# OpenDrift/opendrift

Measured on AMD Instinct MI355X. Metric: particle-steps/sec (RK4, 3D interp), higher is better.
Workload: dtype f64; 1 GPU; C3: OceanDrift 3D, synthetic ROMS-shaped z-level grid 1024x1024x12 (u,v,w,K), RK4 + vertical_mixing(60 s) + vertical_advection; particles_per_gpu=10000000, particles_total=10000000, stage_math=fast, spin_up_steps=200, block_every=0, inputs=resident in HBM, parallelism=particle-sharded x1, field block broadcast once per time level

## Files before the change

include/odrift.h:

```cpp
#ifndef ODRIFT_H
#define ODRIFT_H
#include <stdint.h>

#ifdef __cplusplus
extern "C" {
#endif

typedef struct odr_ctx odr_ctx;
typedef struct odr_particles odr_particles;

typedef enum {
  ODR_OK = 0,
  ODR_ERR_INVALID = -1,
  ODR_ERR_HIP = -2,
  ODR_ERR_CAPACITY = -3,
  ODR_ERR_STATE = -4
} odr_status;

enum {
  ODR_VAR_X_SEA_WATER_VELOCITY = 0,
  ODR_VAR_Y_SEA_WATER_VELOCITY = 1,
  ODR_VAR_X_WIND = 2,
  ODR_VAR_Y_WIND = 3,
  ODR_VAR_UPWARD_SEA_WATER_VELOCITY = 4,
// ... 61 lines not shown
                                       double *z, int32_t *id, int32_t *status);
int odr_particles_upload(odr_ctx *ctx, odr_particles *p, const double *lon, const double *lat,
                         const double *z, const int32_t *moving, const float *wind_drift_factor,
                         const float *current_drift_factor, const float *terminal_velocity);
int odr_particles_download_f32(odr_ctx *ctx, odr_particles *p, const char *name, float *host);
int odr_particles_device_ptr(odr_ctx *ctx, odr_particles *p, const char *name, void **dptr);

int odr_source_constant(odr_ctx *ctx, int nvars, const int32_t *var_ids, const double *values,
                        int32_t *source_id);
int odr_source_analytic(odr_ctx *ctx, int kind, const double *params, int nparams,
                        int32_t *source_id);
int odr_source_landmask(odr_ctx *ctx, int32_t nx, int32_t ny, double lon0, double lat0, double dlon, double dlat,
                        const uint8_t *cells, int32_t *source_id);
int odr_source_grid(odr_ctx *ctx, const odr_proj_desc *proj, const double *domain6,
                    int lon_mode, int mod360_x, int nz, const double *z, int32_t *source_id);
int odr_source_grid_curvilinear(odr_ctx *ctx, const double *lon, const double *lat, int ny, int nx,
                                const double *domain6, int lon_mode, int nz, const double *z,
                                int32_t *source_id);
int odr_source_lonlat2xy(odr_ctx *ctx, int32_t source_id, int64_t n, const double *lon, const double *lat,
                         double *x, double *y);
int odr_block_upload(odr_ctx *ctx, int32_t source_id, int32_t slot, double t_epoch, int nvars,
                     const int32_t *var_ids, const float *const *data, const int32_t *var_nz,
                     int ny, int nx, const double *xy8);
int odr_block_upload_device(odr_ctx *ctx, int32_t source_id, int32_t slot, double t_epoch,
                            int nvars, const int32_t *var_ids, const void *const *dev_data,
                            const int32_t *var_nz, int ny, int nx, const double *xy8);
int odr_block_upload_async(odr_ctx *ctx, int32_t source_id, int32_t slot, double t_epoch, int nvars,
                           const int32_t *var_ids, const void *const *data, const int32_t *var_nz,
                           int ny, int nx, const double *xy8);
int odr_block_commit(odr_ctx *ctx, int32_t source_id, int32_t slot);
int odr_block_set_content_ids(odr_ctx *ctx, int32_t source_id, int32_t slot, int nvars, const int32_t *var_ids,
                              const uint64_t *ids);
int odr_host_register(odr_ctx *ctx, void *ptr, uint64_t bytes);
int odr_host_unregister(odr_ctx *ctx, void *ptr);
int odr_block_drop(odr_ctx *ctx, int32_t source_id, int32_t slot);
int odr_particles_truncate_z(odr_ctx *ctx, odr_particles *p, double truncate_depth);
int odr_particles_restore_z(odr_ctx *ctx, odr_particles *p);
int odr_source_release(odr_ctx *ctx, int32_t source_id);
int odr_source_time_coverage(odr_ctx *ctx, int32_t source_id, double t_start_epoch, double t_end_epoch,
                             int always_valid);
int odr_source_set_members(odr_ctx *ctx, int32_t source_id, int32_t var, int32_t members);
int odr_particles_set_rank_offset(odr_ctx *ctx, odr_particles *p, int64_t offset);
int odr_env_bind(odr_ctx *ctx, int32_t var_id, int nsources, const int32_t *source_ids,
                 float fallback);

int odr_env_sample(odr_ctx *ctx, odr_particles *p, int nvars, const int32_t *var_ids,
                   double t_epoch, float *const *out_host);
int odr_env_download(odr_ctx *ctx, odr_particles *p, int32_t var_id, float *out_host);
int odr_env_upload(odr_ctx *ctx, odr_particles *p, int32_t var_id, const float *host);
enum { ODR_NOISE_NORMAL = 0, ODR_NOISE_UNIFORM = 1 };
int odr_env_add_noise(odr_ctx *ctx, odr_particles *p, int32_t var_x, int32_t var_y, double std, int distribution,
                      int rng_mode, const double *host_nx, const double *host_ny, uint64_t step);
int odr_advect_set_noise(odr_ctx *ctx, odr_particles *p, double std_normal, double std_uniform, int rng_mode,
                         const double *host_main, const double *host_stage, int nstage, uint64_t step);
enum { ODR_STAGE_EXACT = 0, ODR_STAGE_FAST = 1 };
int odr_ctx_set_stage_math(odr_ctx *ctx, int mode);
int odr_advect(odr_ctx *ctx, odr_particles *p, int scheme, double t_epoch, double dt, double factor);
typedef struct {
  int32_t seafloor_action;
  int32_t retired_code;
  double age_dt;
  double max_age_seconds;
  int32_t missing_code;
  int32_t main_noise;
  int32_t vmix;
  int32_t vmix_at_surface;
  int32_t vmix_vadv;
  int32_t pad;
  double vmix_dt_mix;
  uint64_t vmix_step;
} odr_step_extras;
int odr_env_coast_advect(odr_ctx *ctx, odr_particles *p, int nvars, const int32_t *var_ids, double t_epoch,
                         int coastline_action, int stranded_code, int seeded_on_land_code,
                         int store_previous, int scheme, double dt, double factor,
                         const odr_step_extras *extras , int64_t *n_on_land);
int odr_update_positions(odr_ctx *ctx, odr_particles *p, const double *x_vel, const double *y_vel,
                         int velocities_are_float32, double dt);

enum { ODR_FACTOR_SCALAR = 0, ODR_FACTOR_ICE_CURRENT = 1, ODR_FACTOR_ICE_STOKES = 2, ODR_FACTOR_ICE_DRIFT = 3 };
int odr_set_element_factor(odr_ctx *ctx, odr_particles *p, int kind);
int odr_advect_sea_ice(odr_ctx *ctx, odr_particles *p, double dt, double factor);
int odr_advect_wind(odr_ctx *ctx, odr_particles *p, double dt, double wind_drift_depth,
                    int relative_wind, double factor);
int odr_stokes_drift(odr_ctx *ctx, odr_particles *p, double dt, int profile, int hs_mode,
                     int tp_mode, double factor);
int odr_particles_set_property(odr_ctx *ctx, odr_particles *p, int slot, int64_t offset, int64_t count,
                               const float *host);
int odr_particles_get_property(odr_ctx *ctx, odr_particles *p, int slot, float *host);
int odr_particles_snapshot_property(odr_ctx *ctx, odr_particles *p, int slot);
enum { ODR_SPLIT_LANE = 1 };
int odr_leeway_set_missing_code(odr_ctx *ctx, int32_t code);
int odr_env_coast_leeway(odr_ctx *ctx, odr_particles *p, int nvars, const int32_t *var_ids, double t_epoch, int coast_action,
                         int stranded_code, int seeded_on_land_code, int store_previous, double dt, double capsize_fraction,
                         double std_current, double std_wind, uint64_t step, int64_t *n_on_land);
int odr_leeway_capsize(odr_ctx *ctx, odr_particles *p, double dt, double wind_threshold, double wind_threshold_sigma,
                       int rng_mode, const double *host_uniforms, uint64_t step);
int odr_leeway(odr_ctx *ctx, odr_particles *p, double dt, double capsize_leeway_fraction, int rng_mode,
               const double *host_uniforms, uint64_t step);
int odr_hdiffusion(odr_ctx *ctx, odr_particles *p, double dt, int rng_mode,
                   const double *host_nx, const double *host_ny, uint64_t step);
int odr_movers(odr_ctx *ctx, odr_particles *p, double dt, int which, double wind_drift_depth, int relative_wind,
               double wind_factor, int stokes_profile, int hs_mode, int tp_mode, double stokes_factor, int rng_mode,
               const double *host_nx, const double *host_ny, uint64_t step);
int odr_vmix(odr_ctx *ctx, odr_particles *p, double t_epoch, double dt, double dt_mix,
             int mix_at_surface, int rng_mode, const double *host_uniforms, uint64_t step);
enum { ODR_DIFFUSIVITY_LARGE1994 = 1, ODR_DIFFUSIVITY_SUNDBY1983 = 2 };
int odr_vmix_set_profile_levels(odr_ctx *ctx, int32_t n);
int odr_vmix_wind_profile(odr_ctx *ctx, odr_particles *p, int model, double background_diffusivity, double dt,
                          double dt_mix, int mix_at_surface, int rng_mode, const double *host_uniforms,
                          uint64_t step);
enum { ODR_OIL_DIAMETER = 0, ODR_OIL_DENSITY = 1, ODR_OIL_VISCOSITY = 2, ODR_OIL_FILM_THICKNESS = 3,
       ODR_OIL_DIAMETER_IF_ENTRAINED = 4  };
enum { ODR_DROPLETS_JOHANSEN2015 = 1, ODR_DROPLETS_LI2017 = 2 };
int odr_oil_prepare_mixing(odr_ctx *ctx, odr_particles *p, double dt, double dt_mix, double interfacial_tension,
                           double sea_water_density, int droplet_distribution, int keep_droplet_diameter, int hs_mode,
                           int tp_mode, int temperature_to_kelvin, int rng_mode, const double *host_u_diameter,
                           const double *host_u_entrain, const double *host_u_intrusion, uint64_t step);
int odr_oil_mixing_stats(odr_ctx *ctx, double *mean_zb, double *dv50);
int odr_oil_local_sums(odr_ctx *ctx, odr_particles *p, double interfacial_tension, double sea_water_density,
                       int droplet_distribution, int hs_mode, double *sum_dv50, double *sum_zb);
int odr_oil_set_mixing_stats(odr_ctx *ctx, double mean_zb, double dv50);
int odr_vmix_fuse_vertical_advection(odr_ctx *ctx, int at_surface);
int odr_vertical_advection(odr_ctx *ctx, odr_particles *p, double dt, int at_surface);
int odr_vertical_buoyancy(odr_ctx *ctx, odr_particles *p, double dt);
int odr_store_previous(odr_ctx *ctx, odr_particles *p);
int odr_coastline(odr_ctx *ctx, odr_particles *p, int action, int stranded_code,
                  int seeded_on_land_code ,
                  int64_t *n_on_land);
int odr_coastline_crossing(odr_ctx *ctx, odr_particles *p, int action, int stranded_code, int seeded_on_land_code,
                           double precision_deg, int32_t landmask_source, int64_t *n_on_land);
int odr_deactivate_missing(odr_ctx *ctx, odr_particles *p, int nvars, const int32_t *var_ids,
                           int32_t status_code, int64_t *n_missing);
int odr_increase_age(odr_ctx *ctx, odr_particles *p, double dt, double max_age_seconds, int retired_code);
int odr_seafloor(odr_ctx *ctx, odr_particles *p, int64_t *n_below);
enum { ODR_SEAFLOOR_LIFT = 1, ODR_SEAFLOOR_DEACTIVATE = 2, ODR_SEAFLOOR_PREVIOUS = 3 };
int odr_seafloor_action(odr_ctx *ctx, odr_particles *p, int action, int32_t status_code, int64_t *n_below);
int odr_set_seafloor_action(odr_ctx *ctx, int action, int32_t status_code);
int odr_particles_count_status(odr_ctx *ctx, odr_particles *p, int32_t status_code, int64_t *n);
int odr_particles_remap_status(odr_ctx *ctx, odr_particles *p, int32_t from_code, int32_t to_code);
int odr_deactivate(odr_ctx *ctx, odr_particles *p, const uint8_t *mask_host, int32_t status_code);
int odr_deactivate_outside(odr_ctx *ctx, odr_particles *p, double west, double east, double south, double north,
                           int32_t status_code);
int odr_compact(odr_ctx *ctx, odr_particles *p, int64_t *n_active);
int odr_scan_status(odr_ctx *ctx, odr_particles *p, int64_t *n_kept, uint64_t *status_flags);
int odr_scan_status_begin(odr_ctx *ctx, odr_particles *p);
int odr_scan_status_end(odr_ctx *ctx, odr_particles *p, int64_t *n_kept, uint64_t *status_flags);
int odr_ctx_guard_next_vmix(odr_ctx *ctx, int on);
int odr_compact_apply(odr_ctx *ctx, odr_particles *p, int64_t *n_active);
int odr_sort_particles(odr_ctx *ctx, odr_particles *p, int32_t source_id);
int odr_sort_particles_ex(odr_ctx *ctx, odr_particles *p, int32_t source_id, int keep_environment);
int odr_particles_tile_stats(odr_ctx *ctx, odr_particles *p, uint64_t *out4);
int odr_particles_step_layout_stats(odr_ctx *ctx, odr_particles *p, uint64_t *out2);
int odr_particles_step_onlevel_stats(odr_ctx *ctx, odr_particles *p, uint64_t *out1);
int odr_particles_vmix_layout_stats(odr_ctx *ctx, odr_particles *p, uint64_t *out3);
int odr_reduce_scalars(odr_ctx *ctx, odr_particles *p, double wind_drift_depth, double *out16);
int odr_ctx_set_step_reduce(odr_ctx *ctx, int on, double wind_drift_depth, int relative_wind);
int odr_reduce_local(odr_ctx *ctx, odr_particles *p, double wind_drift_depth, int relative_wind, double *out16);
int odr_reduce_install(odr_ctx *ctx, odr_particles *p, const double *in16);
int odr_reduce_unpin(odr_ctx *ctx);

int odr_ctx_set_position_class(odr_ctx *ctx, int f32);
int odr_source_set_coordinate_dtype(odr_ctx *ctx, int32_t source_id, int x_is_float32, int y_is_float32);

#define ODR_COMM_ID_BYTES 256
int odr_device_count(int32_t *n);
int odr_comm_unique_id(uint8_t *id );
int odr_comm_init(odr_ctx *ctx, const uint8_t *id, int32_t rank, int32_t nranks);
int odr_comm_info(int32_t *rank, int32_t *nranks, uint64_t *id_hash, int32_t *rccl_version, uint64_t *collectives);
int odr_comm_destroy(void);
int odr_allreduce_scalars(odr_ctx *ctx, double *values, int32_t n, int32_t op);
int odr_comm_allgather_begin(odr_ctx *ctx, const double *row, int32_t n, int32_t from_scan);
int odr_comm_allgather_end(odr_ctx *ctx, double *rows );
int odr_comm_broadcast_bytes(odr_ctx *ctx, void *buf, int64_t nbytes, int32_t root);
int odr_comm_barrier(odr_ctx *ctx);
int odr_block_broadcast(odr_ctx *ctx, int32_t source_id, int32_t slot, double t_epoch, int nvars, const int32_t *var_ids,
                        const void *const *data, const int32_t *var_nz, int ny, int nx, const double *xy8, int32_t root);

int odr_timer_begin(odr_ctx *ctx);
int odr_timer_end(odr_ctx *ctx, float *ms);

enum {
  ODR_HIST_LON = 1000, ODR_HIST_LAT, ODR_HIST_Z, ODR_HIST_STATUS, ODR_HIST_MOVING, ODR_HIST_AGE_SECONDS,
  ODR_HIST_WIND_DRIFT_FACTOR, ODR_HIST_CURRENT_DRIFT_FACTOR, ODR_HIST_TERMINAL_VELOCITY,
  ODR_HIST_PROPERTY0 = 2000
};
typedef struct odr_history odr_history;
int odr_history_create(odr_ctx *ctx, int64_t n_trajectories, int32_t n_times, int32_t nvars,
                       const int32_t *var_codes, odr_history **out);
int odr_history_set_id_base(odr_ctx *ctx, odr_history *h, int64_t id_base);
int odr_history_destroy(odr_ctx *ctx, odr_history *h);
enum { ODR_HIST_PROPERTIES_FROM_SNAPSHOT = 2 };
int odr_history_record(odr_ctx *ctx, odr_particles *p, odr_history *h, int32_t time_index, int only_deactivated,
                       int position_from_previous);
int odr_history_flush(odr_ctx *ctx, odr_history *h, int32_t t0, int32_t nt);
int odr_history_wait(odr_ctx *ctx, odr_history *h);
int odr_history_host_ptr(odr_ctx *ctx, odr_history *h, int32_t var_index, float **ptr, int32_t *nt);
int odr_history_reset(odr_ctx *ctx, odr_history *h);
int odr_history_minmax(odr_ctx *ctx, odr_history *h, int32_t var_index, double *minval, double *maxval);

typedef struct odr_sgrid odr_sgrid;
int odr_sgrid_create(odr_ctx *ctx, int32_t ny, int32_t nx, int32_t N, const double *H, const double *zeta_or_null,
                     double Hc, const double *Cs_r, const double *S_or_null, int32_t Vtransform, odr_sgrid **out);
int odr_sgrid_destroy(odr_ctx *ctx, odr_sgrid *g);
int odr_sgrid_download_zrho(odr_ctx *ctx, odr_sgrid *g, double *out );
int odr_sgrid_zslice(odr_ctx *ctx, odr_sgrid *g, const void *field, int is_f64, int on_device, int32_t kmax,
                     const double *Z, int32_t out_slot, void **out_dev32, double *out_host64);

#ifdef __cplusplus
}
#endif
#endif
```

opendrift_amd/_abi.py:

```python
import ctypes as C
import os

HERE = os.path.dirname(os.path.abspath(__file__))
LIB_PATH = os.environ.get('ODR_LIB') or os.path.join(HERE, 'libodrift_hip.so')

NVAR = 26
VARIABLES = {
    'x_sea_water_velocity': 0, 'y_sea_water_velocity': 1, 'x_wind': 2, 'y_wind': 3,
    'upward_sea_water_velocity': 4, 'ocean_vertical_diffusivity': 5,
    'sea_surface_wave_stokes_drift_x_velocity': 6, 'sea_surface_wave_stokes_drift_y_velocity': 7,
    'land_binary_mask': 8, 'sea_floor_depth_below_sea_level': 9, 'sea_surface_height': 10,
    'horizontal_diffusivity': 11, 'sea_surface_wave_significant_height': 12,
    'sea_surface_wave_period_at_variance_spectral_density_maximum': 13,
    'ocean_mixed_layer_thickness': 14,
    'sea_water_temperature': 15, 'sea_water_salinity': 16,
    'sea_ice_area_fraction': 17, 'sea_ice_x_velocity': 18, 'sea_ice_y_velocity': 19,
    'sea_surface_swell_wave_to_direction': 20,
    'sea_surface_swell_wave_peak_period_from_variance_spectral_density': 21,
    'sea_surface_swell_wave_significant_height': 22, 'sea_surface_wind_wave_to_direction': 23,
    'sea_surface_wind_wave_mean_period': 24, 'sea_surface_wind_wave_significant_height': 25,
}
VARIABLE_NAMES = {v: k for k, v in VARIABLES.items()}
PROJ_LATLONG, PROJ_STERE_EQUIT_SPHERE, PROJ_STERE_POLAR = 0, 1, 2
PROJ_MERC, PROJ_LCC = 4, 5
PROJ_TMERC, PROJ_LAEA, PROJ_STERE_OBLIQUE, PROJ_OB_TRAN = 6, 7, 8, 9
SCHEME = {'euler': 0, 'runge-kutta': 1, 'runge-kutta4': 2}
RNG_DEVICE, RNG_HOST = 0, 1
STAGE_MATH = {'exact': 0, 'fast': 1}
COAST = {'none': 0, 'stranding': 1, 'previous': 2}
HIST = {'lon': 1000, 'lat': 1001, 'z': 1002, 'status': 1003, 'moving': 1004, 'age_seconds': 1005,
        'wind_drift_factor': 1006, 'current_drift_factor': 1007, 'terminal_velocity': 1008}
HIST_PROPERTY0 = 2000
COMM_ID_BYTES = 256


class StepExtras(C.Structure):
    _fields_ = [('seafloor_action', C.c_int32), ('retired_code', C.c_int32), ('age_dt', C.c_double),
                ('max_age_seconds', C.c_double), ('missing_code', C.c_int32), ('main_noise', C.c_int32),
                ('vmix', C.c_int32), ('vmix_at_surface', C.c_int32), ('vmix_vadv', C.c_int32), ('pad', C.c_int32),
                ('vmix_dt_mix', C.c_double), ('vmix_step', C.c_uint64)]
ANALYTIC_DOUBLE_GYRE, ANALYTIC_OSCILLATING = 1, 2


class ProjDesc(C.Structure):
    _fields_ = [('kind', C.c_int32), ('a', C.c_double), ('es', C.c_double), ('lat0_deg', C.c_double),
                ('lon0_deg', C.c_double), ('lat_ts_deg', C.c_double), ('k0', C.c_double),
                ('x0', C.c_double), ('y0', C.c_double), ('lat1_deg', C.c_double), ('lat2_deg', C.c_double)]


class OdrError(RuntimeError):
    code = 0


_P = C.POINTER
_dp, _fp, _ip, _i64p = _P(C.c_double), _P(C.c_float), _P(C.c_int32), _P(C.c_int64)
_vp = C.c_void_p

_SIGNATURES = {
    'odr_ctx_create': [C.c_int, C.c_uint64, _P(_vp)],
    'odr_ctx_destroy': [_vp],
    'odr_sync': [_vp],
    'odr_set_stream': [_vp, _vp],
    'odr_particles_create': [_vp, C.c_int64, _P(_vp)],
    'odr_particles_destroy': [_vp, _vp],
    'odr_particles_append': [_vp, _vp, C.c_int64, _dp, _dp, _dp, _ip, _ip, _fp, _fp, _fp],
    'odr_particles_count': [_vp, _vp, _i64p, _i64p],
    'odr_particles_download': [_vp, _vp, _dp, _dp, _dp, _ip, _ip, _ip],
    'odr_particles_download_deactivated': [_vp, _vp, _dp, _dp, _dp, _ip, _ip],
    'odr_particles_upload': [_vp, _vp, _dp, _dp, _dp, _ip, _fp, _fp, _fp],
    'odr_particles_device_ptr': [_vp, _vp, C.c_char_p, _P(_vp)],
    'odr_particles_download_f32': [_vp, _vp, C.c_char_p, _fp],
    'odr_source_constant': [_vp, C.c_int, _ip, _dp, _ip],
    'odr_source_analytic': [_vp, C.c_int, _dp, C.c_int, _ip],
    'odr_source_grid': [_vp, _P(ProjDesc), _dp, C.c_int, C.c_int, C.c_int, _dp, _ip],
    'odr_source_grid_curvilinear': [_vp, _dp, _dp, C.c_int, C.c_int, _dp, C.c_int, C.c_int, _dp, _ip],
    'odr_source_landmask': [_vp, C.c_int32, C.c_int32, C.c_double, C.c_double, C.c_double, C.c_double, _P(C.c_uint8), _ip],
    'odr_source_lonlat2xy': [_vp, C.c_int32, C.c_int64, _dp, _dp, _dp, _dp],
    'odr_block_upload': [_vp, C.c_int32, C.c_int32, C.c_double, C.c_int, _ip, _P(_fp), _ip, C.c_int,
                         C.c_int, _dp],
    'odr_block_upload_device': [_vp, C.c_int32, C.c_int32, C.c_double, C.c_int, _ip, _P(_vp), _ip,
                                C.c_int, C.c_int, _dp],
    'odr_block_upload_async': [_vp, C.c_int32, C.c_int32, C.c_double, C.c_int, _ip, _P(_vp), _ip, C.c_int, C.c_int, _dp],
    'odr_block_commit': [_vp, C.c_int32, C.c_int32],
    'odr_host_register': [_vp, _vp, C.c_uint64],
    'odr_host_unregister': [_vp, _vp],
    'odr_block_drop': [_vp, C.c_int32, C.c_int32],
    'odr_env_bind': [_vp, C.c_int32, C.c_int, _ip, C.c_float],
    'odr_env_sample': [_vp, _vp, C.c_int, _ip, C.c_double, _P(_fp)],
    'odr_env_download': [_vp, _vp, C.c_int32, _fp],
    'odr_env_upload': [_vp, _vp, C.c_int32, _fp],
    'odr_env_add_noise': [_vp, _vp, C.c_int32, C.c_int32, C.c_double, C.c_int, C.c_int, _dp, _dp, C.c_uint64],
    'odr_advect_set_noise': [_vp, _vp, C.c_double, C.c_double, C.c_int, _dp, _dp, C.c_int, C.c_uint64],
    'odr_ctx_set_stage_math': [_vp, C.c_int],
    'odr_advect': [_vp, _vp, C.c_int, C.c_double, C.c_double, C.c_double],
    'odr_env_coast_advect': [_vp, _vp, C.c_int, _ip, C.c_double, C.c_int, C.c_int, C.c_int, C.c_int, C.c_int,
                             C.c_double, C.c_double, _vp, _P(C.c_int64)],
    'odr_update_positions': [_vp, _vp, _dp, _dp, C.c_int, C.c_double],
    'odr_source_set_members': [_vp, C.c_int32, C.c_int32, C.c_int32],
    'odr_particles_set_rank_offset': [_vp, _vp, C.c_int64],
    'odr_block_set_content_ids': [_vp, C.c_int32, C.c_int32, C.c_int, _P(C.c_int32), _P(C.c_uint64)],
    'odr_set_element_factor': [_vp, _vp, C.c_int],
    'odr_advect_sea_ice': [_vp, _vp, C.c_double, C.c_double],
    'odr_advect_wind': [_vp, _vp, C.c_double, C.c_double, C.c_int, C.c_double],
    'odr_stokes_drift': [_vp, _vp, C.c_double, C.c_int, C.c_int, C.c_int, C.c_double],
    'odr_particles_set_property': [_vp, _vp, C.c_int, C.c_int64, C.c_int64, _fp],
    'odr_particles_get_property': [_vp, _vp, C.c_int, _fp],
    'odr_particles_snapshot_property': [_vp, _vp, C.c_int],
    'odr_env_coast_leeway': [_vp, _vp, C.c_int, _ip, C.c_double, C.c_int, C.c_int, C.c_int, C.c_int, C.c_double, C.c_double,
                             C.c_double, C.c_double, C.c_uint64, _i64p],
    'odr_leeway_set_missing_code': [_vp, C.c_int32],
    'odr_leeway_capsize': [_vp, _vp, C.c_double, C.c_double, C.c_double, C.c_int, _dp, C.c_uint64],
    'odr_leeway': [_vp, _vp, C.c_double, C.c_double, C.c_int, _dp, C.c_uint64],
    'odr_hdiffusion': [_vp, _vp, C.c_double, C.c_int, _dp, _dp, C.c_uint64],
    'odr_movers': [_vp, _vp, C.c_double, C.c_int, C.c_double, C.c_int, C.c_double, C.c_int, C.c_int, C.c_int, C.c_double, C.c_int, _dp, _dp,
                   C.c_uint64],
    'odr_vmix': [_vp, _vp, C.c_double, C.c_double, C.c_double, C.c_int, C.c_int, _dp, C.c_uint64],
    'odr_vmix_wind_profile': [_vp, _vp, C.c_int, C.c_double, C.c_double, C.c_double, C.c_int, C.c_int, _dp, C.c_uint64],
    'odr_vmix_fuse_vertical_advection': [_vp, C.c_int],
    'odr_oil_prepare_mixing': [_vp, _vp, C.c_double, C.c_double, C.c_double, C.c_double, C.c_int, C.c_int, C.c_int, C.c_int,
                               C.c_int, C.c_int, _dp, _dp, _dp, C.c_uint64],
    'odr_oil_mixing_stats': [_vp, _dp, _dp],
    'odr_oil_local_sums': [_vp, _vp, C.c_double, C.c_double, C.c_int, C.c_int, _dp, _dp],
    'odr_oil_set_mixing_stats': [_vp, C.c_double, C.c_double],
    'odr_vertical_advection': [_vp, _vp, C.c_double, C.c_int],
    'odr_vertical_buoyancy': [_vp, _vp, C.c_double],
    'odr_store_previous': [_vp, _vp],
    'odr_coastline': [_vp, _vp, C.c_int, C.c_int, C.c_int, _i64p],
    'odr_coastline_crossing': [_vp, _vp, C.c_int, C.c_int, C.c_int, C.c_double, C.c_int32, _i64p],
    'odr_increase_age': [_vp, _vp, C.c_double, C.c_double, C.c_int],
    'odr_source_time_coverage': [_vp, C.c_int32, C.c_double, C.c_double, C.c_int],
    'odr_source_release': [_vp, C.c_int32],
    'odr_particles_truncate_z': [_vp, _vp, C.c_double],
    'odr_particles_restore_z': [_vp, _vp],
    'odr_seafloor': [_vp, _vp, _i64p],
    'odr_seafloor_action': [_vp, _vp, C.c_int, C.c_int32, _i64p],
    'odr_set_seafloor_action': [_vp, C.c_int, C.c_int32],
    'odr_deactivate_missing': [_vp, _vp, C.c_int, _ip, C.c_int32, _i64p],
    'odr_particles_count_status': [_vp, _vp, C.c_int32, _i64p],
    'odr_particles_remap_status': [_vp, _vp, C.c_int32, C.c_int32],
    'odr_deactivate': [_vp, _vp, _P(C.c_uint8), C.c_int32],
    'odr_deactivate_outside': [_vp, _vp, C.c_double, C.c_double, C.c_double, C.c_double, C.c_int32],
    'odr_compact': [_vp, _vp, _i64p],
    'odr_vmix_set_profile_levels': [_vp, C.c_int32],
    'odr_ctx_set_position_class': [_vp, C.c_int],
    'odr_source_set_coordinate_dtype': [_vp, C.c_int32, C.c_int, C.c_int],
    'odr_device_count': [_P(C.c_int32)],
    'odr_comm_unique_id': [_P(C.c_uint8)],
    'odr_comm_init': [_vp, _P(C.c_uint8), C.c_int32, C.c_int32],
    'odr_comm_info': [_P(C.c_int32), _P(C.c_int32), _P(C.c_uint64), _P(C.c_int32), _P(C.c_uint64)],
    'odr_comm_destroy': [],
    'odr_allreduce_scalars': [_vp, _dp, C.c_int32, C.c_int32],
    'odr_comm_allgather_begin': [_vp, _dp, C.c_int32, C.c_int32],
    'odr_comm_allgather_end': [_vp, _dp],
    'odr_comm_broadcast_bytes': [_vp, _vp, C.c_int64, C.c_int32],
    'odr_comm_barrier': [_vp],
    'odr_block_broadcast': [_vp, C.c_int32, C.c_int32, C.c_double, C.c_int, _ip, _P(_vp), _ip, C.c_int, C.c_int, _dp, C.c_int32],
    'odr_scan_status': [_vp, _vp, _i64p, _P(C.c_uint64)],
    'odr_scan_status_begin': [_vp, _vp],
    'odr_scan_status_end': [_vp, _vp, _i64p, _P(C.c_uint64)],
    'odr_ctx_guard_next_vmix': [_vp, C.c_int],
    'odr_compact_apply': [_vp, _vp, _i64p],
    'odr_sort_particles': [_vp, _vp, C.c_int32],
    'odr_sort_particles_ex': [_vp, _vp, C.c_int32, C.c_int],
    'odr_particles_tile_stats': [_vp, _vp, _P(C.c_uint64)],
    'odr_particles_step_layout_stats': [_vp, _vp, _P(C.c_uint64)],
    'odr_particles_step_onlevel_stats': [_vp, _vp, _P(C.c_uint64)],
    'odr_particles_vmix_layout_stats': [_vp, _vp, _P(C.c_uint64)],
    'odr_reduce_scalars': [_vp, _vp, C.c_double, _dp],
    'odr_ctx_set_step_reduce': [_vp, C.c_int, C.c_double, C.c_int],
    'odr_reduce_local': [_vp, _vp, C.c_double, C.c_int, _dp],
    'odr_reduce_install': [_vp, _vp, _dp],
    'odr_reduce_unpin': [_vp],
    'odr_timer_begin': [_vp],
    'odr_timer_end': [_vp, _fp],
    'odr_sgrid_create': [_vp, C.c_int32, C.c_int32, C.c_int32, _dp, _dp, C.c_double, _dp, _dp, C.c_int32, _P(_vp)],
    'odr_sgrid_destroy': [_vp, _vp],
    'odr_sgrid_download_zrho': [_vp, _vp, _dp],
    'odr_sgrid_zslice': [_vp, _vp, _vp, C.c_int, C.c_int, C.c_int32, _dp, C.c_int32, _P(_vp), _dp],
    'odr_history_create': [_vp, C.c_int64, C.c_int32, C.c_int32, _ip, _P(_vp)],
    'odr_history_destroy': [_vp, _vp],
    'odr_history_set_id_base': [_vp, _vp, C.c_int64],
    'odr_history_record': [_vp, _vp, _vp, C.c_int32, C.c_int, C.c_int],
    'odr_history_flush': [_vp, _vp, C.c_int32, C.c_int32],
    'odr_history_wait': [_vp, _vp],
    'odr_history_host_ptr': [_vp, _vp, C.c_int32, _P(_fp), _P(C.c_int32)],
    'odr_history_reset': [_vp, _vp],
    'odr_history_minmax': [_vp, _vp, C.c_int32, _dp, _dp],
}
EXPORTS = sorted(list(_SIGNATURES) + ['odr_last_error', 'odr_version'])

_lib = None


def load():
    global _lib
    if _lib is not None:
        return _lib
    if not os.path.exists(LIB_PATH):
        raise OdrError('libodrift_hip.so is missing: run `python -c "import __graft_entry__ as g; '
                       'g.build()"` (hipcc --offload-arch=gfx950).  There is no CPU fallback.')
    lib = C.CDLL(LIB_PATH)
    for name, args in _SIGNATURES.items():
        fn = getattr(lib, name)
        fn.argtypes = args
        fn.restype = C.c_int
    lib.odr_last_error.restype = C.c_char_p
    lib.odr_last_error.argtypes = []
    lib.odr_version.restype = C.c_char_p
    lib.odr_version.argtypes = []
    _lib = lib
    return lib


NOISE_NORMAL, NOISE_UNIFORM = 0, 1
DIFFUSIVITY = {'windspeed_Large1994': 1, 'windspeed_Sundby1983': 2}
DROPLETS = {'Johansen et al. (2015)': 1, 'Li et al. (2017)': 2}
OIL_PROPERTIES = ['diameter', 'density', 'viscosity', 'oil_film_thickness', 'diameter_if_entrained']


def check(rc):
    if rc != 0:
        msg = load().odr_last_error().decode()
        if rc == -1:
            raise ValueError(msg)
        e = OdrError('odrift error %d: %s' % (rc, msg))
        e.code = rc
        raise e
```

opendrift_amd/csrc/odr_host.h:

```cpp
#pragma once
#include <hip/hip_runtime.h>

#include <algorithm>
#include <cmath>
#include <cstdarg>
#include <cstdio>
#include <cstdlib>
#include <cstring>
#include <string>
#include <vector>

#include "../../include/odrift.h"
#include "odr_kernels.hip.h"

using namespace odr;

#include <chrono>
struct SlowSpan {
  const char *what;
  std::chrono::steady_clock::time_point t0;
  static double limit() { static const double v = getenv("ODR_SLOW_CALLS") ? atof(getenv("ODR_SLOW_CALLS")) : 0.0; return v; }
  explicit SlowSpan(const char *w) : what(w) { if (limit() > 0) t0 = std::chrono::steady_clock::now(); }
  ~SlowSpan() {
    if (limit() > 0) {
      const double ms = std::chrono::duration<double, std::milli>(std::chrono::steady_clock::now() - t0).count();
      if (ms > limit()) fprintf(stderr, "[odr slow] %s: %.3f ms\n", what, ms);
    }
  }
};

int odr_i_fail(int code, const char *fmt, ...);
#define fail odr_i_fail
#define HIPCHK(x)                                                                          \
  do {                                                                                     \
    hipError_t e_ = (x);                                                                   \
    if (e_ != hipSuccess) return fail(ODR_ERR_HIP, "%s: %s", #x, hipGetErrorString(e_));   \
  } while (0)
#define REQUIRE(c, ...) do { if (!(c)) return fail(ODR_ERR_INVALID, __VA_ARGS__); } while (0)

struct Staged { DevBlock blk; float *base; size_t bytes; unsigned long long cid[NVAR]; };
struct Retired { void *ptr; size_t bytes; hipEvent_t ev; };

struct odr_ctx {
  int device;
  unsigned long long seed;
  hipStream_t stream, own_stream;
  DevWorld hw;
  DevWorld *dw;
  unsigned src_gen[MAXSRC] = {0};
  hipEvent_t scan_ev = nullptr;
  bool scan_open = false;
  int guard_next_vmix = 0;
  const odr_particles *guarded_vmix = nullptr;
  int guarded_vadv = -1;
  int vmix_levels = 0;
  unsigned long long *scan_host = nullptr;
  DevWorld *hw_pin[3] = {nullptr, nullptr, nullptr};
  hipEvent_t hw_ev[3] = {nullptr, nullptr, nullptr};
  int hw_turn = 0;
  bool dirty;
  std::vector<void *> block_bufs[MAXSRC][MAXLEVELS];
  size_t block_bytes[MAXSRC][MAXLEVELS];
  unsigned long long block_cid[MAXSRC][MAXLEVELS][NVAR];
  hipStream_t up_stream;
  hipEvent_t up_done, up_dep;
  float *prep[2];
  size_t prep_floats;
  int *dilate_flags;
  int *tile_flags = nullptr;
  size_t tile_flags_n = 0;
  void *bounce[2];
  Staged staged[MAXSRC][MAXLEVELS];
  std::vector<Retired> graveyard;
  std::vector<void *> source_bufs;
  std::vector<void *> registered;
  double *red;
  const odr_particles *noise_owner;
  StageNoise noise;
  double *noise_buf;
  size_t noise_buf_n;
  const odr_particles *oil_owner;
  OilArgs oil;
  double *oil_stat, *oil_cdf, *oil_chunk, *oil_part, *oil_u;
  int *oil_guide;
  int oil_override;
  double oil_stat_host[2];
  size_t oil_part_n, oil_u_n;
  unsigned long long *counter;
  hipEvent_t ev0, ev1;
  int nsrc;
  bool src_free[MAXSRC];
  int stage_math;
  int fuse_vadv;
  int leeway_missing_code;
  int seafloor;
  const odr_particles *red_owner;
  unsigned long long red_epoch;
  double red_wdd;
  int red_rel;
  bool red_extents = true;
  int red_pinned;
  double *red_rec = nullptr; long long red_rec_cap = 0;
  bool red_partial = false;
  int step_reduce_on = 0, step_reduce_rel = 0;
  double step_reduce_wdd = 0.1;
};

struct odr_particles {
  long long cap, n, ndead, dead_cap;
  int ice_kind;
  int *rank;
  unsigned *rank_words, *rank_before, *rank_bsum;
  long long rank_words_n, id_max;
  int rank_on;
  int rank_sharded = 0;
  long long rank_offset = 0;
  double *d64[7];
  double *alt64[7];
  int *i32[3];
  int *alti32[3];
  float *f32[4];
  float *altf32[4];
  float *env[NVAR];
  float *altenv[NVAR];
  float *aux[9];
  float *altaux[9];
  bool profiles_f32 = false;
  unsigned aux_user = 0;
  bool kmember_on = false;
  float *aux_snap[9];
  long long aux_snap_cap[9];
  double *dead64[3];
  int *deadi32[2];
  unsigned *bcount;
  unsigned *wcount;
  unsigned long long wcount_epoch;
  long long wcount_n;
  void *scratch;
  size_t scratch_bytes;
  unsigned long long epoch;
  unsigned long long status_epoch, scan_epoch;
  long long scan_kept;
  float env_cval[NVAR];
  long long env_cn[NVAR];
  bool env_cok[NVAR];
  bool external;
  unsigned *wg_tab, *wg_list;
  unsigned long long *wg_total, *wg_stats;
  long long wg_cap, wg_grid, wg_n, wg_list_cap;
  unsigned long long wg_launches;
  unsigned long long step_launches[3];
  unsigned long long vmix_launches[3];
  double *z_keep;
  long long z_keep_n;
  bool z_truncated;
  int wg_sid;
  bool wg_valid;
  unsigned wg_src_gen;
};

static inline unsigned nblk(long long n) { return (unsigned)((n + BLOCK - 1) / BLOCK); }

static inline PView view(const odr_particles *p) {
  PView v;
  v.n = p->n;
  v.lon = p->d64[0]; v.lat = p->d64[1]; v.z = p->d64[2]; v.plon = p->d64[3]; v.plat = p->d64[4];
  v.slon = p->d64[5]; v.slat = p->d64[6];
  v.id = p->i32[0]; v.status = p->i32[1]; v.moving = p->i32[2];
  v.wdf = p->f32[0]; v.cdf = p->f32[1]; v.tv = p->f32[2]; v.age = p->f32[3];
  for (int k = 0; k < NVAR; ++k) v.env[k] = p->env[k];
  for (int k = 0; k < 9; ++k) v.aux[k] = p->aux[k];
  v.ice = p->ice_kind; v.pad = 0;
  v.rank = p->rank_on && p->rank ? p->rank : nullptr;
  return v;
}

static inline EnvGroupDesc env_bind_out(const EnvGroupDesc &G0, const PView &v) {
  EnvGroupDesc G = G0;
  for (int k = 0; k < MAXG; ++k) G.out_ptr[k] = k < G.nv ? v.env[G.var[k]] : nullptr;
  return G;
}

int flush_world(odr_ctx *c);
int flush_world_init(odr_ctx *c);

static inline bool env_is_const(const odr_particles *p, int v, float val) {
  return p->env[v] && p->env_cok[v] && p->env_cn[v] >= p->n && p->env_cval[v] == val;
}
static inline int ensure_env(odr_ctx *c, odr_particles *p, int var) {
  if (!p->env[var]) {
    HIPCHK(hipMalloc((void **)&p->env[var], sizeof(float) * (size_t)p->cap));
    HIPCHK(hipMemsetAsync(p->env[var], 0, sizeof(float) * (size_t)p->cap, c->stream));
  }
  return 0;
}

static inline int scratch(odr_ctx *c, odr_particles *p, size_t bytes, void **out) {
  if (p->scratch_bytes < bytes) {
    SlowSpan sp("scratch: synchronize + hipFree + hipMalloc");
    HIPCHK(hipStreamSynchronize(c->stream));
    if (p->scratch) HIPCHK(hipFree(p->scratch));
    HIPCHK(hipMalloc(&p->scratch, bytes));
    p->scratch_bytes = bytes;
  }
  *out = p->scratch;
  return 0;
}

static inline void host_bracket(const DevSource &s, double t, int &ib, int &ia) {
  int b = 0;
  for (int k = 0; k < s.nlevels; ++k) if (s.slot[s.level_slot[k]].t <= t) b = k;
  ib = s.level_slot[b];
  ia = (b + 1 < s.nlevels && s.slot[ib].t != t) ? s.level_slot[b + 1] : -1;
}

static inline UVTime uv_time(const DevSource &s, double t) {
  int ib, ia;
  host_bracket(s, t, ib, ia);
  UVTime tm;
  tm.b = s.slot[ib].data[VAR_U];
  tm.a = (ia >= 0 && !s.always_valid) ? s.slot[ia].data[VAR_U] : nullptr;
  tm.w = ia >= 0 ? (t - s.slot[ib].t) / (s.slot[ia].t - s.slot[ib].t) : 0.0;
  return tm;
}


static inline bool build_vmix_desc(const odr_ctx *c, double t, VMixDesc &D) {
  memset(&D, 0, sizeof D);
  int ksid = -1, nzp = 1;
  for (int k = 0; k < c->hw.nlist[VAR_KZ]; ++k)
    if (c->hw.src[c->hw.list[VAR_KZ][k]].kind == SRC_GRID) { ksid = c->hw.list[VAR_KZ][k]; break; }
  if (ksid < 0) return false;
  const DevSource &s = c->hw.src[ksid];
  nzp = s.nz > 1 ? s.nz : 1;
  if (nzp <= 1 || s.nlevels < 1) return false;
  const DevBlock &g0 = s.slot[s.level_slot[0]];
  for (int k = 0; k < s.nlevels; ++k) {
    const DevBlock &bk = s.slot[s.level_slot[k]];
    if (s.members[VAR_KZ] > 1 || !bk.small || !bk.data[VAR_KZ] || bk.es[VAR_KZ] != 1 || bk.var_nz[VAR_KZ] != nzp || bk.rec != g0.rec || bk.ny != g0.ny || bk.nx != g0.nx ||
        bk.x0 != g0.x0 || bk.xspan != g0.xspan || bk.y0 != g0.y0 || bk.yspan != g0.yspan)
      return false;
  }
  int ib, ia;
  host_bracket(s, t, ib, ia);
  D.sid = ksid; D.nzp = nzp; D.geo_slot = ib;
  D.kb = s.slot[ib].data[VAR_KZ];
  D.ka = ia >= 0 ? s.slot[ia].data[VAR_KZ] : nullptr;
  D.wgt = ia >= 0 ? (t - s.slot[ib].t) / (s.slot[ia].t - s.slot[ib].t) : 0.0;
  D.Kfb = c->hw.fallback[VAR_KZ];
  return true;
}

constexpr size_t ODR_BOUNCE_BYTES = 8u << 20;
static inline int odr_i_bounce(odr_ctx *c, int which, void **buf) {
  if (!c->bounce[which]) HIPCHK(hipHostMalloc(&c->bounce[which], ODR_BOUNCE_BYTES, hipHostMallocDefault));
  *buf = c->bounce[which];
  return 0;
}
static inline int odr_i_h2d(odr_ctx *c, void *dst, const void *src, size_t bytes, hipStream_t st, int which = 0) {
  void *b;
  int rc = odr_i_bounce(c, which, &b);
  if (rc) return rc;
  for (size_t o = 0; o < bytes; o += ODR_BOUNCE_BYTES) {
    const size_t m = std::min(ODR_BOUNCE_BYTES, bytes - o);
    memcpy(b, (const char *)src + o, m);
    HIPCHK(hipMemcpyAsync((char *)dst + o, b, m, hipMemcpyHostToDevice, st));
    HIPCHK(hipStreamSynchronize(st));
  }
  return 0;
}
static inline int odr_i_d2h(odr_ctx *c, void *dst, const void *src, size_t bytes, hipStream_t st, int which = 0) {
  void *b;
  int rc = odr_i_bounce(c, which, &b);
  if (rc) return rc;
  for (size_t o = 0; o < bytes; o += ODR_BOUNCE_BYTES) {
    const size_t m = std::min(ODR_BOUNCE_BYTES, bytes - o);
    HIPCHK(hipMemcpyAsync(b, (const char *)src + o, m, hipMemcpyDeviceToHost, st));
    HIPCHK(hipStreamSynchronize(st));
    memcpy((char *)dst + o, b, m);
  }
  return 0;
}
#define H2D(dst, src, bytes) do { int rc_ = odr_i_h2d(c, (dst), (src), (bytes), c->stream); if (rc_) return rc_; } while (0)
#define D2H(dst, src, bytes) do { int rc_ = odr_i_d2h(c, (dst), (src), (bytes), c->stream); if (rc_) return rc_; } while (0)

static inline bool source_has_members(const DevSource &s) {
  for (int v = 0; v < NVAR; ++v) if (s.members[v] > 1) return true;
  return false;
}
static inline bool any_members(const odr_ctx *c) {
  for (int k = 0; k < c->nsrc; ++k) if (c->hw.src[k].kind == SRC_GRID && source_has_members(c->hw.src[k])) return true;
  return false;
}
static inline int odr_proj_template(const odr::DevProj &p) {
  if (p.kind == odr::PROJ_STERE_POLAR) return p.es != 0 ? odr::PROJ_STERE_POLAR : odr::PROJ_STERE_EQUIT_SPHERE;
  if (p.kind >= odr::PROJ_TMERC) return odr::PROJ_EXT;
  return p.kind;
}
int odr_i_ensure_ranks(odr_ctx *c, odr_particles *p);

bool odr_i_build_env_group(const odr_ctx *c, const int *grp, int ng, double t, EnvGroupDesc &G);
bool odr_i_comm_on();
int odr_i_comm_rank();
int odr_i_comm_bcast_floats(float *dev, size_t count, int root, hipStream_t st);
void odr_i_phase_dump();
bool odr_i_uv_fast_source(const odr_ctx *c, int &sid, double t_lo, double t_hi);

bool odr_i_gyre_source(const odr_ctx *c, int var, int &sid);
int odr_i_env_sample(odr_ctx *c, odr_particles *p, int nvars, const int32_t *var_ids, double t, float *const *out_host,
                     bool record_positions);
int odr_i_red_finish(odr_ctx *c, odr_particles *p);
int odr_i_red_records(odr_ctx *c, odr_particles *p, double **rec);
int odr_i_reduce(odr_ctx *c, odr_particles *p, double wdd, int relwind, bool wind_args_matter = true, bool extents = true, bool partial_ok = false);
int odr_i_read_counter(odr_ctx *c, int64_t *out);
int odr_i_env_noise(odr_ctx *c, odr_particles *p, int vx, int vy, double std, int distribution, int rng_mode,
                    const double *dev_nx, const double *dev_ny, unsigned long long step);
#define build_env_group odr_i_build_env_group
#define uv_fast_source odr_i_uv_fast_source
#define gyre_source odr_i_gyre_source
#define env_sample_impl odr_i_env_sample
#define reduce odr_i_reduce
#define read_counter odr_i_read_counter
```

opendrift_amd/csrc/odr_kernels.hip.h:

```cpp
#pragma once
#include <hip/hip_runtime.h>
#include <rocrand/rocrand_kernel.h>
#include "odr_field.hip.h"

namespace odr {

#ifndef ODR_BLOCK
#define ODR_BLOCK 256
#endif
constexpr int BLOCK = ODR_BLOCK;
#ifndef ODR_POLAR_WAVES
#define ODR_POLAR_WAVES 3
#endif
#ifndef ODR_POLAR_STEP_WAVES
#define ODR_POLAR_STEP_WAVES 2
#endif
#define ODR_STEP_WAVES(PROJ) ((PROJ) == PROJ_LATLONG ? ODR_LATLONG_WAVES : ((PROJ) == PROJ_EXT ? 1 : ODR_POLAR_STEP_WAVES))
#ifndef ODR_LATLONG_WAVES
#define ODR_LATLONG_WAVES 1
#endif
#define ODR_WAVES(PROJ) ((PROJ) == PROJ_LATLONG ? ODR_LATLONG_WAVES : ((PROJ) == PROJ_EXT ? 1 : ODR_POLAR_WAVES))

__device__ __forceinline__ long long pid() {
  const unsigned nb = gridDim.x, b = blockIdx.x, per = nb >> 3, rem = nb & 7u, x = b & 7u, j = b >> 3;
// ... 397 lines not shown
    if (TL) {
      a00 = ld_off<F4>(ka, o00 + 16u * q); a01 = ld_off<F4>(ka, o01 + 16u * q);
      a10 = ld_off<F4>(ka, o10 + 16u * q); a11 = ld_off<F4>(ka, o11 + 16u * q);
    }
    if (VM::STATIC && q > 0) __builtin_amdgcn_sched_barrier(0);
    if (q == 0) hook();
    double v[4];
    v[0] = (double)bilw(b00.x, b01.x, b10.x, b11.x, w00, w01, w10, w11);
    v[1] = (double)bilw(b00.y, b01.y, b10.y, b11.y, w00, w01, w10, w11);
    v[2] = (double)bilw(b00.z, b01.z, b10.z, b11.z, w00, w01, w10, w11);
    v[3] = (double)bilw(b00.w, b01.w, b10.w, b11.w, w00, w01, w10, w11);
    if (TL) {
      double w[4];
      w[0] = (double)bilw(a00.x, a01.x, a10.x, a11.x, w00, w01, w10, w11);
      w[1] = (double)bilw(a00.y, a01.y, a10.y, a11.y, w00, w01, w10, w11);
      w[2] = (double)bilw(a00.z, a01.z, a10.z, a11.z, w00, w01, w10, w11);
      w[3] = (double)bilw(a00.w, a01.w, a10.w, a11.w, w00, w01, w10, w11);
#pragma unroll
      for (int j = 0; j < 4; ++j) v[j] = __dadd_rn(__dmul_rn(v[j], 1 - wgt), __dmul_rn(w[j], wgt));
    }
#pragma unroll
    for (int j = 0; j < 4; ++j) Kp[(4 * q + j) * BLOCK + tid] = (cov && isfinite(v[j])) ? v[j] : Kfb;
  }
}

struct VMixArgs {
  double dt, dt_mix_cfg;
  int mix_at_surface, rng_mode, sfl, pad;
  const double *huni;
  unsigned long long seed, step;
};
struct MixRng { MixKey key; uint4 q; bool primed; };
template <class VM = VMixRT>
__device__ __forceinline__ MixRng mix_rng_begin(const VMixArgs &A, int id) {
  MixRng R;
  R.key = mix_key(A.seed, A.step, id);
  R.q = make_uint4(0u, 0u, 0u, 0u);
  R.primed = false;
  if (VM::rng_mode(A.rng_mode) == 0) {
    R.q = mix_block(R.key, 0u);
    R.primed = true;
  }
  return R;
}
template <int NQ, class VM = VMixRT>
__device__ __forceinline__ double vmix_col_walk(const DevSource &s, int nzp, const double *Kp, const double *gsh, int tid,
                                                const VMixArgs &A, long long i, long long n, int id, double z, int &moving,
                                                float Zmin, float tv, int &sf_flags, const MixRng *pre) {
  constexpr int NL = 4 * NQ;
  static_assert(!VM::STATIC || NL >= 3, "a static configuration has the three-level window inside the profile");
  const double dt = A.dt;
  const int mix_at_surface = VM::mix_at_surface(A.mix_at_surface), rng_mode = VM::rng_mode(A.rng_mode), sfl = A.sfl;
  double zm[NL - 1];
#pragma unroll
  for (int k = 0; k < NL - 1; ++k) zm[k] = k < nzp - 1 ? s.zmid[k] : __builtin_inf();
  const bool uniform_z = VM::uniform_z(s.vg_uniform != 0);
  const double gd0 = s.vg_d[0], gi0 = s.vg_id[0], gd1 = s.vg_d[1], gi1 = s.vg_id[1], gd2 = s.vg_d[2], gi2 = s.vg_id[2];
  const double sgn = dt > 0 ? 1.0 : (dt < 0 ? -1.0 : 0.0);
  const double dt_mix = A.dt_mix_cfg * sgn;
  const int ntimes = VM::ntimes(abs((int)(dt / dt_mix)));
  const double r = 1.0 / 3, ir = 1.0 / r;
  double wstep = __dmul_rn(__dmul_rn((double)tv, dt_mix), (double)moving);
  const MixKey st = mix_key(A.seed, A.step, id);
  uint4 u4 = make_uint4(0u, 0u, 0u, 0u);
  bool primed = false;
  if (pre) { u4 = pre->q; primed = pre->primed; }
  auto level_terms = [&](auto edges, int zl, double &dk_dt, double &sg) {
    constexpr int E = decltype(edges)::value;
    const double Kz = Kp[zl * BLOCK + tid];
    double gK;
    if ((E & 1) && zl == 0) gK = div_cr(Kp[BLOCK + tid] - Kz, gd0, gi0);
    else if ((E & 2) && zl == nzp - 1) gK = div_cr(Kz - Kp[(nzp - 2) * BLOCK + tid], gd1, gi1);
    else if (uniform_z) gK = div_cr(Kp[(zl + 1) * BLOCK + tid] - Kp[(zl - 1) * BLOCK + tid], gd2, gi2);
    else
      gK = __dadd_rn(__dadd_rn(__dmul_rn(gsh[zl], Kp[(zl - 1) * BLOCK + tid]), __dmul_rn(gsh[NL + zl], Kz)),
                     __dmul_rn(gsh[2 * NL + zl], Kp[(zl + 1) * BLOCK + tid]));
    double dK = -gK;
    if (fabs(dK) < 1e-10) dK = 0;
    dk_dt = __dmul_rn(dK, dt_mix);
    sg = sqrt(div_cr(__dmul_rn(__dmul_rn(Kz, fabs(dt_mix)), 2.0), r, ir));
  };
  using AnyLevel = std::integral_constant<int, 3>;
  int lv0;
  {
    const double d0 = -z;
    int zs = 0;
#pragma unroll
    for (int k = 0; k < NL - 1; ++k) zs += ((k & 1) ? d0 >= zm[k] : d0 > zm[k]) ? 1 : 0;
    lv0 = zs < 1 ? 1 : (zs > nzp - 2 ? nzp - 2 : zs);
    if (nzp < 3) lv0 = 1;
  }
  double c_dk[3], c_sg[3];
#pragma unroll
  for (int q = 0; q < 3; ++q) {
    const int zl = lv0 - 1 + q;
    c_dk[q] = 0; c_sg[q] = 0;
    if constexpr (VM::STATIC) {
      if (q == 0) level_terms(std::integral_constant<int, 1>(), zl, c_dk[q], c_sg[q]);
      else if (q == 1) level_terms(std::integral_constant<int, 0>(), zl, c_dk[q], c_sg[q]);
      else level_terms(std::integral_constant<int, 2>(), zl, c_dk[q], c_sg[q]);
    } else if (zl >= 0 && zl < nzp) level_terms(AnyLevel(), zl, c_dk[q], c_sg[q]);
  }
  double wb[4];
#pragma unroll
  for (int j = 0; j < 4; ++j) {
    const int k = lv0 - 2 + j;
    double b = k < 0 ? -1.0 : __builtin_inf();
    if (k >= 0 && k < nzp - 1) {
      b = gsh[3 * NL + k];
      if ((k & 1) && b > 0) b = __longlong_as_double(__double_as_longlong(b) - 1);
    }
    wb[j] = b;
  }
  for (int it0 = 0; it0 < ntimes; it0 += 5) {
  if (rng_mode == 0 && !(primed && it0 == 0)) u4 = mix_block(st, (unsigned)it0 / 5u);
#pragma unroll
  for (int k5 = 0; k5 < 5; ++k5) {
    const int it = it0 + k5;
    if (it >= ntimes) break;
    const bool surface = z == 0;
    const double d = -z;
    int q = (d > wb[1] ? 1 : 0) + (d > wb[2] ? 1 : 0);
    int zi = lv0 - 1 + q;
    if (!(d > wb[0]) || d > wb[3]) {
      zi = 0;
#pragma unroll
      for (int k = 0; k < NL - 1; ++k) zi += ((k & 1) ? d >= zm[k] : d > zm[k]) ? 1 : 0;
      q = zi - lv0 + 1;
    }
    double dKdt = q == 0 ? c_dk[0] : (q == 1 ? c_dk[1] : c_dk[2]);
    double sig = q == 0 ? c_sg[0] : (q == 1 ? c_sg[1] : c_sg[2]);
    if (q < 0 || q > 2) level_terms(AnyLevel(), zi, dKdt, sig);
    double R;
    if (rng_mode == 1) R = __dsub_rn(__dmul_rn(2.0, A.huni[(size_t)it * n + i]), 1.0);
    else R = mix_R_of(mix_word(u4, (unsigned)k5));
    z = __dsub_rn(z, __dmul_rn((double)moving, __dsub_rn(dKdt, __dmul_rn(R, sig))));
    if (z >= 0) z = -z;
    if (z < (double)Zmin && moving == 1) z = __dsub_rn((double)__fmul_rn(2.f, Zmin), z);
    z = __dadd_rn(z, wstep);
    if (!mix_at_surface && surface) z = 0.0;
    if (z > 0) z = 0.0;
    if (z < (double)Zmin) {
      const int act = VM::sf_action(sfl & 255);
      if (act == 3) sf_flags |= 2;
      else if (act) {
        z = (double)Zmin;
        if (act == 2) { sf_flags |= 1; moving = 0; wstep = 0.0; }
      }
    }
  }
  }
  return z;
}

__device__ __forceinline__ float pick_slot(const float (&a)[MAXG], int j) {
  float r = a[0];
#pragma unroll
  for (int k = 1; k < MAXG; ++k) {
    float v = a[k];
    asm volatile("" : "+v"(v));
    r = j == k ? v : r;
  }
  return r;
}

#ifdef ODR_TU_MISC
template <int NV>
struct GroupVars { int v[NV]; };

template <int NV>
__global__ __launch_bounds__(BLOCK) void k_env_group(const DevWorld *__restrict__ W, PView p,
                                                     GroupVars<NV> gv, double t, int record_prev) {
  long long i = (long long)blockIdx.x * BLOCK + threadIdx.x;
  if (i >= p.n) return;
  int vars[NV];
#pragma unroll
  for (int k = 0; k < NV; ++k) vars[k] = gv.v[k];
  double lon = p.lon[i], lat = p.lat[i], z = p.z[i];
  float out[NV];
  env_group<NV>(*W, vars, lon, lat, z, t, out, p.rank ? p.rank[i] : 0, W->f32pos & 1);
#pragma unroll
  for (int k = 0; k < NV; ++k) p.env[vars[k]][i] = out[k];
  if (record_prev) { p.slon[i] = lon; p.slat[i] = lat; }
}

template <int PROJ>
__global__ __launch_bounds__(BLOCK, ODR_WAVES(PROJ)) void k_env_grid(const DevWorld *__restrict__ W, PView p, EnvGroupDesc G,
                                                    int record_prev) {
  long long i = pid();
  if (i >= p.n) return;
  double lon = p.lon[i], lat = p.lat[i], z = p.z[i];
  int f32idx = 0;
  if (W->f32pos & 1) {
    lon = lon_f32class(W->src[G.sid].lon_mode, lon);
    if (PROJ == PROJ_LATLONG) f32idx = W->src[G.sid].xy_f32;
  }
  float out[MAXG];
  env_group_fast<PROJ>(*W, G, lon, lat, z, out, f32idx);
#pragma unroll
  for (int k = 0; k < MAXG; ++k)
    if (k < G.nv) G.out_ptr[k][i] = out[k];
  if (record_prev) { p.slon[i] = lon; p.slat[i] = lat; }
}

__global__ __launch_bounds__(BLOCK) void k_fill_f32(float *a, long long n, float v) {
  long long i = (long long)blockIdx.x * BLOCK + threadIdx.x;
  if (i < n) a[i] = v;
}

__global__ __launch_bounds__(BLOCK) void k_record_prev(PView p, int which) {
  long long i = (long long)blockIdx.x * BLOCK + threadIdx.x;
  if (i >= p.n) return;
  if (which == 0) { p.slon[i] = p.lon[i]; p.slat[i] = p.lat[i]; }
  else { p.plon[i] = p.lon[i]; p.plat[i] = p.lat[i]; }
}

#endif
#ifdef ODR_TU_STEP
__device__ __forceinline__ float rk4_mix(float k1, float k2, float k3, float k4) {
  float s = __fadd_rn(k1, __fmul_rn(2.0f, k2));
  s = __fadd_rn(s, __fmul_rn(2.0f, k3));
  s = __fadd_rn(s, k4);
  return div_cr_f32(s, 6.0f, 1.0f / 6.0f);
}

template <int SCHEME, bool NOISE>
__global__ __launch_bounds__(BLOCK) void k_advect(const DevWorld *__restrict__ W, PView p, double t,
                                                  double dt, float factor, StageNoise N) {
  long long i = (long long)blockIdx.x * BLOCK + threadIdx.x;
  if (i >= p.n) return;
  const int uv[2] = {VAR_U, VAR_V};
  double lon = p.lon[i], lat = p.lat[i], z = p.z[i];
  float u1 = p.env[VAR_U][i], v1 = p.env[VAR_V][i];
  float f = __fmul_rn(current_factor(p, i, factor), p.cdf[i]);
  int moving = p.moving[i];
  const int rk = p.rank ? p.rank[i] : 0;
  float fu, fv;
  GeodStart o = geod_start(lat, lon);
  if (SCHEME == 0) {
    fu = __fmul_rn(f, u1);
    fv = __fmul_rn(f, v1);
  } else {
    float dtf = (float)dt;
    double lon2, lat2;
    float k2[2];
    stage_pos_rt(N.sm, o, u1, v1, dtf, lon2, lat2);
    env_group<2>(*W, uv, lon2, lat2, z, t + dt / 2, k2, rk);
    const int id = NOISE ? p.id[i] : 0;
    if (NOISE) add_current_noise(N, 1, i, p.n, id, k2[0], k2[1]);
    if (SCHEME == 1) {
      fu = __fmul_rn(f, k2[0]);
      fv = __fmul_rn(f, k2[1]);
    } else {
      float k3[2], k4[2];
      stage_pos_rt(N.sm, o, k2[0], k2[1], dtf, lon2, lat2);
      env_group<2>(*W, uv, lon2, lat2, z, t + dt / 2, k3, rk);
      if (NOISE) add_current_noise(N, 2, i, p.n, id, k3[0], k3[1]);
      stage_pos_rt(N.sm, o, k3[0], k3[1], dtf, lon2, lat2);
      env_group<2>(*W, uv, lon2, lat2, z, t + dt, k4, rk);
      if (NOISE) add_current_noise(N, 3, i, p.n, id, k4[0], k4[1]);
      fu = __fmul_rn(rk4_mix(u1, k2[0], k3[0], k4[0]), f);
      fv = __fmul_rn(rk4_mix(v1, k2[1], k3[1], k4[1]), f);
    }
  }
  move_f32_from(o, lon, lat, fu, fv, moving, dt);
  p.lon[i] = lon;
  p.lat[i] = lat;
}

template <int PROJ, bool IS3D, int SM, class LD>
__device__ __forceinline__ void uv_stage_or_global(const DevSource &s, const DevBlock &geo, const UVTime &tm, const LD &ld, double lon,
                                                   double lat, double z, const ZBracket &zb, float fbu, float fbv, float &uo,
                                                   float &vo, const ProjStart &ps, UVKeep<IS3D> &K, bool keep) {
  if (!uv_stage<PROJ, IS3D, SM>(s, geo, tm, ld, lon, lat, z, zb, fbu, fbv, uo, vo, ps, K, keep)) {
    if constexpr (sizeof(LD) != sizeof(LdGlobal)) uv_stage<PROJ, IS3D, SM>(s, geo, tm, uv_global(tm), lon, lat, z, zb, fbu, fbv, uo, vo, ps, K, keep);
  }
}
template <int SCHEME, int PROJ, bool IS3D, bool NOISE, int SM = 0, bool PARK = false, class LD = LdGlobal>
__device__ __forceinline__ void advect_grid_body(const DevSource &s, const DevBlock &geo, double &lon, double &lat,
                                                 double z, float u1, float v1, float f, int moving, double dt,
                                                 const UVTime &th, const UVTime &tf, const LD &lh, const LD &lf, float fbu, float fbv,
                                                 const StageNoise &N, long long i, long long n, int id, UVKeep<IS3D> &K,
                                                 ZBracket zb_pre = ZBracket(), bool have_pre = false,
                                                 double *park = nullptr ODR_PT_PARAM, const ProjStart ps_pre = ProjStart()) {
  float fu, fv;
  const bool keep_f = tf.b == th.b && tf.a == th.a;
  GeodStart o0 = geod_start(lat, lon);
  lds_f64 *slot = (lds_f64 *)park;
  if constexpr (PARK) { geod_park(o0, slot); if (SM == 1 && SCHEME == 2) slot[14 * BLOCK] = (double)f; }
  auto O = [&]() { if constexpr (PARK) return geod_unpark(slot[12 * BLOCK], slot[13 * BLOCK], slot); else return o0; };
#define ODR_O O()
#define ODR_STAGE_POS(U_, V_) do { if constexpr (PARK && SM == 1) stage_pos_parked(slot, U_, V_, dtf, lon2, lat2); \
                                   else stage_pos<SM>(ODR_O, U_, V_, dtf, lon2, lat2); } while (0)
  if (SCHEME == 0) {
    fu = __fmul_rn(f, u1);
    fv = __fmul_rn(f, v1);
  } else {
    ZBracket zb;
    zb.iz0 = 0; zb.same = 0; zb.wa = 1;
    if (IS3D) { if (have_pre) zb = zb_pre; else zb = zbracket(s, z); }
    float dtf = (float)dt;
    double lon2, lat2;
    float u2, v2;
    ProjStart ps;
    if (PROJ == PROJ_STERE_POLAR || (ODR_PROJ_ROTATES(PROJ) && s.proj.kind == PROJ_STERE_POLAR && s.proj.es != 0)) {
      if (ps_pre.ok) ps = ps_pre;
      else {
        double lw = lon;
        if (s.lon_mode == 1) lw = np_mod(lw + 180.0, 360.0) - 180.0;
        else if (s.lon_mode == 2) lw = np_mod(lw, 360.0);
        ps = proj_start(s.proj, lw, lat);
      }
    }
    ODR_STAGE_POS(u1, v1);
    ODR_PT_USE(lon2); ODR_PT_USE(lat2); ODR_PT(4);
    uv_stage_or_global<PROJ, IS3D, SM>(s, geo, th, lh, lon2, lat2, z, zb, fbu, fbv, u2, v2, ps, K, true);
    if (NOISE) add_current_noise(N, 1, i, n, id, u2, v2);
    ODR_PT_USE(u2); ODR_PT_USE(v2); ODR_PT(5);
    if (SCHEME == 1) {
      fu = __fmul_rn(f, u2);
      fv = __fmul_rn(f, v2);
    } else {
      float u3, v3, u4, v4;
      ODR_STAGE_POS(u2, v2);
      uv_stage_or_global<PROJ, IS3D, SM>(s, geo, th, lh, lon2, lat2, z, zb, fbu, fbv, u3, v3, ps, K, true);
      if (NOISE) add_current_noise(N, 2, i, n, id, u3, v3);
      ODR_PT_USE(u3); ODR_PT_USE(v3); ODR_PT(6);
      ODR_STAGE_POS(u3, v3);
      uv_stage_or_global<PROJ, IS3D, SM>(s, geo, tf, lf, lon2, lat2, z, zb, fbu, fbv, u4, v4, ps, K, keep_f);
      if (NOISE) add_current_noise(N, 3, i, n, id, u4, v4);
      ODR_PT_USE(u4); ODR_PT_USE(v4); ODR_PT(7);
      float fl = f;
      if constexpr (PARK && SM == 1) fl = (float)slot[14 * BLOCK];
      fu = __fmul_rn(rk4_mix(u1, u2, u3, u4), fl);
      fv = __fmul_rn(rk4_mix(v1, v2, v3, v4), fl);
    }
  }
  move_f32_from(ODR_O, lon, lat, fu, fv, moving, dt);
#undef ODR_O
#undef ODR_STAGE_POS
}

template <int SCHEME, int PROJ, bool IS3D, bool NOISE, int SM = 0>
__global__ __launch_bounds__(BLOCK, ODR_STEP_WAVES(PROJ)) void k_advect_grid(const DevWorld *__restrict__ W, int sid, int geo_slot,
                                                       PView p, double dt, float factor, UVTime th,
                                                       UVTime tf, StageNoise N) {
  long long i = pid();
  if (i >= p.n) return;
  const DevSource &s = W->src[sid];
  const DevBlock &geo = s.slot[geo_slot];
  double lon = p.lon[i], lat = p.lat[i];
  UVKeep<IS3D> K;
  K.valid = false; K.n00 = K.n11 = K.kb = 0;
  advect_grid_body<SCHEME, PROJ, IS3D, NOISE, SM>(s, geo, lon, lat, p.z[i], p.env[VAR_U][i], p.env[VAR_V][i],
                                              __fmul_rn(current_factor(p, i, factor), p.cdf[i]), p.moving[i], dt, th, tf, uv_global(th), uv_global(tf),
                                              W->fallback[VAR_U], W->fallback[VAR_V], N, i, p.n, NOISE ? p.id[i] : 0, K);
  p.lon[i] = lon;
  p.lat[i] = lat;
}

#endif
enum { R_NACT = 0, R_LONMIN, R_LONMAX, R_LATMIN, R_LATMAX, R_ZMIN, R_ZMAX, R_DMAX, R_STOKESMAX,
       R_WSPEEDMAX, R_WDFMAX, R_NSURF, R_HSMAX, R_TPMAX, R_RELWSPEEDMAX, R_MLDMAX, R_N };

__device__ __forceinline__ void atomic_max_d(double *addr, double v) {
  unsigned long long *a = (unsigned long long *)addr, old = *a, assumed;
  do {
    assumed = old;
    if (__longlong_as_double((long long)assumed) >= v) break;
    old = atomicCAS(a, assumed, (unsigned long long)__double_as_longlong(v));
  } while (assumed != old);
}

__device__ __forceinline__ double wave_max(double v) {
#pragma unroll
  for (int o = 32; o > 0; o >>= 1) v = fmax(v, __shfl_xor(v, o, 64));
  return v;
}
__device__ __forceinline__ double wave_sum(double v) {
#pragma unroll
  for (int o = 32; o > 0; o >>= 1) v += __shfl_xor(v, o, 64);
  return v;
}
#ifdef ODR_TU_STEP
struct StepDesc {
  int coast_action, stranded_code, seeded_code, land_slot;
  int store_previous, geo_slot_uv;
  int seafloor, depth_slot;
  float age_dt, max_age;
  int retired_code, missing_code;
  int nmiss_grp, nmiss_rest;
  int miss_grp[4], miss_rest[4];
  int main_noise;
  int ssh_slot;
  int red_on, red_rel;
  int red_hd, red_sx, red_xw, red_pad;
  double red_wdd, red_iwdd;
  double *red;
  unsigned *wcount;
  unsigned long long *sflags;
};

#ifndef ODR_PARK_WAVES
#define ODR_PARK_WAVES 4
#endif
#ifndef ODR_PARK_WAVES_FAST3D
#define ODR_PARK_WAVES_FAST3D 5
#endif
#define ODR_PARK_WAVES_OF(PROJ, IS3D, SM) (((PROJ) == PROJ_LATLONG && (IS3D) && (SM) == 1) ? ODR_PARK_WAVES_FAST3D : ODR_PARK_WAVES)
#define ODR_STEP_PARKS(SCHEME, PROJ) ((SCHEME) > 0 && ((PROJ) == PROJ_LATLONG || (PROJ) == PROJ_CURVILINEAR))
template <int SCHEME, int PROJ, bool IS3D, bool NOISE, int SM = 0, class LY = LayoutRT>
__global__ __launch_bounds__(BLOCK, ODR_STEP_PARKS(SCHEME, PROJ) ? ODR_PARK_WAVES_OF(PROJ, IS3D, SM) : ODR_STEP_WAVES(PROJ)) void k_step_grid(const DevWorld *__restrict__ W, PView p, EnvGroupDesc G,
                                                     StepDesc S, double dt, float factor, UVTime th, UVTime tf,
                                                     unsigned long long *n_hit, StageNoise N) {
  long long i = pid();
  bool hit = false;
  ODR_PT_DECL;
  ODR_PT(0);
  constexpr bool PARK = ODR_STEP_PARKS(SCHEME, PROJ);
  __shared__ double s_park[PARK ? GEOD_PARK * BLOCK : 1];
  __shared__ double s_zt[IS3D ? 3 * ZT_STRIDE : 1];
  const double *zt = nullptr;
  double lon_e = 0, lat_e = 0, z_e = 0;
  if (i < p.n) { lon_e = p.lon[i]; lat_e = p.lat[i]; z_e = p.z[i]; }
  if (IS3D) { zt_stage(W->src[G.sid], s_zt); zt = s_zt; }
  unsigned r_bits = 0;
  if (i < p.n) {
    double lon = lon_e, lat = lat_e;
    const double z = z_e;
    constexpr bool STATE_LATE = ODR_STEP_PARKS(SCHEME, PROJ) && IS3D;
    int moving = 0, st = 0;
    float age0 = 0.f, cdf0 = 0.f, ssh0 = 0.f;
    auto load_state = [&]() {
      moving = p.moving[i];
      st = p.status[i];
      age0 = p.age[i]; cdf0 = p.cdf[i];
      ssh0 = S.seafloor && p.env[VAR_SSH] ? p.env[VAR_SSH][i] : 0.f;
    };
    if constexpr (!STATE_LATE) load_state();
    constexpr bool RED = !IS3D;
    const float wdf0 = (RED && S.red_on && S.red_xw > -2) ? p.wdf[i] : 0.f;
    ODR_PT_USE(lon); ODR_PT_USE(lat); ODR_PT_USE(z); ODR_PT(1);
    float out[MAXG];
    ZBracket zb_env;
    zb_env.iz0 = 0; zb_env.same = 0; zb_env.wa = 1;
    EnvExport X;
    X.valid = false; X.n00 = X.n11 = 0; X.iz0 = 0;
    X.combine = IS3D && SM == 1;
    ProjStart ps0;
    if constexpr (PROJ == PROJ_STERE_POLAR && SCHEME != 0) {
      const DevSource &s0 = W->src[G.sid];
      double lw = lon;
      if (s0.lon_mode == 1) lw = np_mod(lw + 180.0, 360.0) - 180.0;
      else if (s0.lon_mode == 2) lw = np_mod(lw, 360.0);
      ps0 = proj_start(s0.proj, lw, lat);
    }
    env_group_fast<PROJ, true, IS3D, LY>(*W, G, lon, lat, z, out, zt, zb_env, &X ODR_PT_ARG, 0, ps0, th.a);
    UVKeep<IS3D> K = uv_keep_from_sm<IS3D, SM, LY>(G, X, th, zb_env, W->src[G.sid].nz, true);
    if constexpr (STATE_LATE) load_state();
    ODR_PT_USE(out[0]); ODR_PT_USE(out[1]); ODR_PT_USE(out[2]); ODR_PT_USE(out[3]); ODR_PT_USE(out[4]); ODR_PT(2);
    const int id = NOISE ? p.id[i] : 0;
    if (NOISE && S.main_noise) add_current_noise(N, 0, i, p.n, id, out[0], out[1]);
#pragma unroll
    for (int k = 0; k < MAXG; ++k)
      if (k < LY::nv_of(G)) G.out_ptr[k][i] = out[k];
    p.slon[i] = lon;
    p.slat[i] = lat;
    float l_hd = 0.f, l_sx = 0.f, l_sy = 0.f, l_xw = 0.f, l_yw = 0.f;
    if (RED && S.red_on) {
      if (S.red_hd > -2) l_hd = p.env[VAR_HDIFF][i];
      if (S.red_sx > -2) { l_sx = p.env[VAR_SX][i]; l_sy = p.env[VAR_SY][i]; }
      if (S.red_xw > -2) { l_xw = p.env[VAR_XWIND][i]; l_yw = p.env[VAR_YWIND][i]; }
    }
    double zz = z;
    if (S.missing_code) {
      bool miss = false;
#pragma unroll
      for (int k = 0; k < 4; ++k) {
        if (k < S.nmiss_grp) { const float e = pick_slot(out, S.miss_grp[k]); miss |= e != e; }
        if (k < S.nmiss_rest) { const float e = p.env[S.miss_rest[k]][i]; miss |= e != e; }
      }
      if (miss) {
        if (st == 0) p.status[i] = st = S.missing_code;
        p.moving[i] = moving = 0;
      }
    }
    if (S.coast_action) {
      float land;
      if constexpr (LY::STATIC) land = out[LY::land_slot];
      else land = S.land_slot == 2 ? out[2] : p.env[VAR_LAND][i];
      if (land == 1.0f) {
        hit = true;
        if (S.coast_action == 1) {
          if (z <= 0) {
            if (st == 0) p.status[i] = st = S.stranded_code;
            p.moving[i] = moving = 0;
          }
        } else {
          if (S.seeded_code > 0 && age0 == 0.0f) {
            if (st == 0) p.status[i] = st = S.seeded_code;
            p.moving[i] = moving = 0;
          }
          lon = p.plon[i];
          lat = p.plat[i];
          ps0.ok = 0;
          p.env[VAR_LAND][i] = 0.0f;
        }
      }
    }
    if (S.seafloor) {
      float floorz;
      if constexpr (LY::STATIC) {
        static_assert(LY::depth_slot >= 0 && LY::ssh_slot < 0, "a static layout holds the depth and not the ssh");
        floorz = -__fadd_rn(out[LY::depth_slot], ssh0);
      } else {
        const float dep = S.depth_slot == 2 ? out[2] : (S.depth_slot == 3 ? out[3] : p.env[VAR_DEPTH][i]);
        floorz = -__fadd_rn(dep, S.ssh_slot >= 0 ? pick_slot(out, S.ssh_slot) : ssh0);
      }
      if (zz < (double)floorz) { zz = (double)floorz; p.z[i] = zz; }
    }
    if (S.age_dt != 0.0f) {
      const float a = __fadd_rn(age0, S.age_dt);
      p.age[i] = a;
      if (S.max_age > 0 && a >= S.max_age) {
        if (st == 0) p.status[i] = st = S.retired_code;
        p.moving[i] = moving = 0;
      }
    }
    const bool skip = st != 0;
    if constexpr (IS3D && SM == 1) { if (zz != z) K.valid = false; }
    if (S.store_previous) { p.plon[i] = lon; p.plat[i] = lat; }
    ODR_PT(3);
    if (!skip) {
      const DevSource &s = W->src[G.sid];
      advect_grid_body<SCHEME, PROJ, IS3D, NOISE, SM, PARK>(s, s.slot[S.geo_slot_uv], lon, lat, zz, out[0], out[1],
                                                        __fmul_rn(current_factor(p, i, factor), cdf0), moving, dt, th, tf, uv_global(th), uv_global(tf),
                                                        W->fallback[VAR_U], W->fallback[VAR_V], N, i, p.n, id, K, zb_env, IS3D && zz == z, PARK ? s_park + threadIdx.x : nullptr ODR_PT_ARG, ps0);
    }
    ODR_PT_USE(lon); ODR_PT_USE(lat); ODR_PT(8);
    if (RED && S.red_on && !skip) {
      if (S.red_hd > -2) r_bits |= (l_hd > 0.f ? 1u : 0u) | (l_hd == 0.f ? 2u : 0u);
      if (S.red_sx > -2) { const float st_sum = __fadd_rn(l_sx, l_sy); r_bits |= (st_sum > 0.f ? 4u : 0u) | (st_sum == 0.f ? 8u : 0u); }
      if (S.red_xw > -2) {
        const double wdd = fabs(S.red_wdd);
        if (zz >= -wdd) {
          double wdf = wdf0;
          if (S.red_wdd != 0) {
            wdf = div_cr(wdf * (wdd + zz), wdd, S.red_iwdd);
            if (zz > 0) wdf = wdf0;
          }
          float xa = l_xw, ya = l_yw;
          if (S.red_rel) { xa = __fsub_rn(xa, out[0]); ya = __fsub_rn(ya, out[1]); }
          const float rws = speed_f32(xa, ya);
          r_bits |= 16u | (wdf > 0 ? 32u : 0u) | (wdf == 0 ? 64u : 0u) | (rws > 0.f ? 128u : 0u) | (rws == 0.f ? 256u : 0u);
        }
      }
    }
    {
      long long i2 = i;
      asm volatile("" : "+v"(i2));
      p.lon[i2] = lon;
      p.lat[i2] = lat;
    }
#ifdef ODR_PHASE_TIMING
    pt_[9] = __builtin_readcyclecounter();
    if ((threadIdx.x & 63) == 0 && (blockIdx.x & 127) == 5) {
      for (int k = 0; k < 9; ++k) atomicAdd(&g_phase[k], pt_[k + 1] > pt_[k] && pt_[k] ? pt_[k + 1] - pt_[k] : 0ull);
      for (int k = 10; k < 17; ++k) atomicAdd(&g_phase[k], pt_[k + 1] > pt_[k] && pt_[k] ? pt_[k + 1] - pt_[k] : 0ull);
      atomicAdd(&g_phase[31], 1ull);
    }
#endif
  }
  if (S.coast_action) {
    unsigned long long b = __ballot(hit);
    if ((threadIdx.x & 63) == 0 && b) atomicAdd(n_hit, (unsigned long long)__popcll(b));
  }
  if (!IS3D && S.red_on) {
    const unsigned long long b1 = __ballot(r_bits & 1u), b2 = __ballot(r_bits & 2u), b4 = __ballot(r_bits & 4u), b8 = __ballot(r_bits & 8u);
    const unsigned long long bs = __ballot(r_bits & 16u), b32 = __ballot(r_bits & 32u), b64 = __ballot(r_bits & 64u);
    const unsigned long long b128 = __ballot(r_bits & 128u), b256 = __ballot(r_bits & 256u);
    const unsigned lane = threadIdx.x & 63u;
    if (lane < 6u) {
      const double ninf = -__builtin_inf();
      auto sgn = [&](unsigned long long pos, unsigned long long zero) { return pos ? 1.0 : (zero ? 0.0 : ninf); };
      const double v = lane == 0 ? sgn(b1, b2) : lane == 1 ? sgn(b4, b8) : lane == 2 ? ninf
                     : lane == 3 ? sgn(b128, b256) : lane == 4 ? sgn(b32, b64) : (double)__popcll(bs);
      S.red[((size_t)blockIdx.x * (BLOCK / 64) + (threadIdx.x >> 6)) * 6 + lane] = v;
    }
  }
  if (S.wcount) {
    int s2 = 1;
    long long i3 = i;
    asm volatile("" : "+v"(i3));
    if (i3 < p.n) s2 = p.status[i3];
    const unsigned long long kb = __ballot(s2 == 0);
    if (__ballot(s2 >= 100 && s2 < 164)) {
      if (s2 >= 100 && s2 < 164) atomicOr(S.sflags, 1ull << (s2 - 100));
    }
    if ((threadIdx.x & 63) == 0 && i3 < p.n) S.wcount[i3 >> 6] = (unsigned)__popcll(kb);
  }
}

#endif
#ifdef ODR_TU_MISC
__global__ __launch_bounds__(BLOCK) void k_env_gyre(const DevWorld *__restrict__ W, int sid, PView p, double snw,
                                                    int with_land, int record_prev) {
  long long i = (long long)blockIdx.x * BLOCK + threadIdx.x;
  if (i >= p.n) return;
  const DevSource &s = W->src[sid];
  const double lon = (W->f32pos & 1) ? lon_f32class(s.lon_mode, p.lon[i]) : p.lon[i], lat = p.lat[i];
  float u, v;
  const bool covered = gyre_sample(s, lon, lat, p.z[i], snw, W->fallback[VAR_U], W->fallback[VAR_V], u, v);
  p.env[VAR_U][i] = u;
  p.env[VAR_V][i] = v;
  if (with_land) p.env[VAR_LAND][i] = covered ? 0.0f : W->fallback[VAR_LAND];
  if (record_prev) { p.slon[i] = lon; p.slat[i] = lat; }
}

#endif
#ifdef ODR_TU_STEP
template <int SCHEME, bool NOISE>
__global__ __launch_bounds__(BLOCK) void k_advect_gyre(const DevWorld *__restrict__ W, int sid, PView p, double dt,
                                                       float factor, double snw_half, double snw_full, StageNoise N) {
  long long i = (long long)blockIdx.x * BLOCK + threadIdx.x;
  if (i >= p.n) return;
  const DevSource &s = W->src[sid];
  const float fbu = W->fallback[VAR_U], fbv = W->fallback[VAR_V];
  double lon = p.lon[i], lat = p.lat[i];
  const double z = p.z[i];
  const float u1 = p.env[VAR_U][i], v1 = p.env[VAR_V][i];
  const float f = __fmul_rn(current_factor(p, i, factor), p.cdf[i]);
  float fu, fv;
  GeodStart o = geod_start(lat, lon);
  if (SCHEME == 0) {
    fu = __fmul_rn(f, u1);
    fv = __fmul_rn(f, v1);
  } else {
    const float dtf = (float)dt;
    double lon2, lat2;
    float u2, v2;
    stage_pos_rt(N.sm, o, u1, v1, dtf, lon2, lat2);
    gyre_sample(s, lon2, lat2, z, snw_half, fbu, fbv, u2, v2);
    const int id = NOISE ? p.id[i] : 0;
    if (NOISE) add_current_noise(N, 1, i, p.n, id, u2, v2);
    if (SCHEME == 1) {
      fu = __fmul_rn(f, u2);
      fv = __fmul_rn(f, v2);
    } else {
      float u3, v3, u4, v4;
      stage_pos_rt(N.sm, o, u2, v2, dtf, lon2, lat2);
      gyre_sample(s, lon2, lat2, z, snw_half, fbu, fbv, u3, v3);
      if (NOISE) add_current_noise(N, 2, i, p.n, id, u3, v3);
      stage_pos_rt(N.sm, o, u3, v3, dtf, lon2, lat2);
      gyre_sample(s, lon2, lat2, z, snw_full, fbu, fbv, u4, v4);
      if (NOISE) add_current_noise(N, 3, i, p.n, id, u4, v4);
      fu = __fmul_rn(rk4_mix(u1, u2, u3, u4), f);
      fv = __fmul_rn(rk4_mix(v1, v2, v3, v4), f);
    }
  }
  move_f32_from(o, lon, lat, fu, fv, p.moving[i], dt);
  p.lon[i] = lon;
  p.lat[i] = lat;
}

#endif
#ifdef ODR_TU_MISC
__global__ __launch_bounds__(BLOCK) void k_update_positions(PView p, const double *u, const double *v,
                                                            int is_f32, double dt) {
  long long i = (long long)blockIdx.x * BLOCK + threadIdx.x;
  if (i >= p.n) return;
  double lon = p.lon[i], lat = p.lat[i];
  if (is_f32) move_f32(lon, lat, (float)u[i], (float)v[i], p.moving[i], dt);
  else move_f64(lon, lat, u[i], v[i], p.moving[i], dt);
  p.lon[i] = lon;
  p.lat[i] = lat;
}

#endif
#ifdef ODR_TU_MISC
template <bool EXT>
__global__ __launch_bounds__(BLOCK) void k_reduce(PView p, double wind_drift_depth, int relative_wind,
                                                  double *red) {
  const double ninf = -__builtin_inf();
  double v[R_N];
#pragma unroll
  for (int k = 0; k < R_N; ++k) v[k] = ninf;
  v[R_NACT] = 0;
  v[R_NSURF] = 0;
  const double wdd = fabs(wind_drift_depth);
  const bool has_hd = p.env[VAR_HDIFF] != nullptr, has_st = p.env[VAR_SX] && p.env[VAR_SY], has_hs = p.env[VAR_HS] != nullptr;
  const bool has_tp = p.env[VAR_TP] != nullptr, has_mld = p.env[VAR_MLD] != nullptr, has_w = p.env[VAR_XWIND] && p.env[VAR_YWIND];
  const bool rel = relative_wind && p.env[VAR_U] && p.env[VAR_V];
  const long long stride = (long long)gridDim.x * BLOCK;
  for (long long i0 = (long long)blockIdx.x * BLOCK + threadIdx.x; i0 < p.n; i0 += 2 * stride) {
    int st[2]; double z[2], lo[2], la[2]; float hd[2], sx[2], sy[2], hs[2], tp[2], mld[2], xw[2], yw[2], wdf0[2], cu[2], cv[2];
#pragma unroll
    for (int u = 0; u < 2; ++u) {
      const long long i = i0 + u * stride;
      const bool in = i < p.n;
      const long long j = in ? i : i0;
      st[u] = in ? p.status[j] : 1;
      z[u] = p.z[j];
      if (EXT) { lo[u] = p.lon[j]; la[u] = p.lat[j]; }
      hd[u] = has_hd ? p.env[VAR_HDIFF][j] : 0.f;
      sx[u] = has_st ? p.env[VAR_SX][j] : 0.f; sy[u] = has_st ? p.env[VAR_SY][j] : 0.f;
      hs[u] = has_hs ? p.env[VAR_HS][j] : 0.f; tp[u] = has_tp ? p.env[VAR_TP][j] : 0.f; mld[u] = has_mld ? p.env[VAR_MLD][j] : 0.f;
      xw[u] = has_w ? p.env[VAR_XWIND][j] : 0.f; yw[u] = has_w ? p.env[VAR_YWIND][j] : 0.f; wdf0[u] = has_w ? p.wdf[j] : 0.f;
      cu[u] = rel ? p.env[VAR_U][j] : 0.f; cv[u] = rel ? p.env[VAR_V][j] : 0.f;
    }
#pragma unroll
    for (int u = 0; u < 2; ++u) {
      if (st[u] != 0) continue;
      v[R_NACT] += 1;
      if (EXT) {
        v[R_LONMIN] = fmax(v[R_LONMIN], -lo[u]); v[R_LONMAX] = fmax(v[R_LONMAX], lo[u]);
        v[R_LATMIN] = fmax(v[R_LATMIN], -la[u]); v[R_LATMAX] = fmax(v[R_LATMAX], la[u]);
        v[R_ZMIN] = fmax(v[R_ZMIN], -z[u]); v[R_ZMAX] = fmax(v[R_ZMAX], z[u]);
      }
      if (has_hd) v[R_DMAX] = fmax(v[R_DMAX], (double)hd[u]);
      if (has_st) v[R_STOKESMAX] = fmax(v[R_STOKESMAX], (double)__fadd_rn(sx[u], sy[u]));
      if (has_hs) v[R_HSMAX] = fmax(v[R_HSMAX], (double)hs[u]);
      if (has_tp) v[R_TPMAX] = fmax(v[R_TPMAX], (double)tp[u]);
      if (has_mld) v[R_MLDMAX] = fmax(v[R_MLDMAX], (double)mld[u]);
      if (has_w) {
// ... 334 lines not shown
  {
    bool cov = false;
    double xi = 0, yi = 0, wgt = 0;
    int ib = 0, ia = -1;
    const size_t moff = (kmembers > 1 && p.aux[AUX_KMEMBER]) ? (size_t)((int)p.aux[AUX_KMEMBER][i]) * (size_t)nz_full : 0;
    if (src) {
      double lon = p.slon[i], lat = p.slat[i], x, y;
      if (src->lon_mode == 1) lon = np_mod(lon + 180.0, 360.0) - 180.0;
      else if (src->lon_mode == 2) lon = np_mod(lon, 360.0);
      proj_fwd_rt(src->proj, lon, lat, x, y);
      cov = x >= src->xmin && x <= src->xmax && y >= src->ymin && y <= src->ymax;
      if (src->mod360_x) x = np_mod(x, 360.0);
      bracket(*src, t, ib, ia);
      const DevBlock &bb = src->slot[ib];
      const int f32idx = ((W->f32pos & 2) && src->proj.kind == PROJ_LATLONG) ? src->xy_f32 : 0;
      xi = (f32idx & 1) ? index_f32(x, bb.x0, bb.xspan, bb.nx - 1) : __dmul_rn(div_cr(x - bb.x0, bb.xspan, bb.ixspan), (double)(bb.nx - 1));
      yi = (f32idx & 2) ? index_f32(y, bb.y0, bb.yspan, bb.ny - 1) : __dmul_rn(div_cr(y - bb.y0, bb.yspan, bb.iyspan), (double)(bb.ny - 1));
      if (ia >= 0) wgt = __ddiv_rn(t - bb.t, src->slot[ia].t - bb.t);
    }
    if (src && cov && src->slot[ib].es[VAR_KZ] == 1 && NZMAX > 1) {
      const DevBlock &bb = src->slot[ib];
      const int ny = bb.ny, nx = bb.nx;
      const Axis ay = axis_fp(yi, ny), ax = axis_fp(xi, nx);
      const int y0 = ay.i0, y1 = ay.i1, x0 = ax.i0, x1 = ax.i1;
      const double ty = ay.t, tx = ax.t, wy0 = 1 - ty, wx0 = 1 - tx;
      const size_t rec = (size_t)bb.rec;
      size_t o00 = ((size_t)y0 * nx + x0) * rec, o01 = ((size_t)y0 * nx + x1) * rec;
      size_t o10 = ((size_t)y1 * nx + x0) * rec, o11 = ((size_t)y1 * nx + x1) * rec;
      float c00[NZMAX], c01[NZMAX], c10[NZMAX], c11[NZMAX];
      const float *d = bb.data[VAR_KZ] + moff;
      kcolumn(d + o00, nzp, c00); kcolumn(d + o01, nzp, c01);
      kcolumn(d + o10, nzp, c10); kcolumn(d + o11, nzp, c11);
#pragma unroll
      for (int k = 0; k < NZMAX; ++k)
        if (k < nzp) Kp[k * BLOCK + tid] = (double)bil4(c00[k], c01[k], c10[k], c11[k], wy0, ty, wx0, tx);
      if (ia >= 0) {
        const float *da = src->slot[ia].data[VAR_KZ] + moff;
        kcolumn(da + o00, nzp, c00); kcolumn(da + o01, nzp, c01);
        kcolumn(da + o10, nzp, c10); kcolumn(da + o11, nzp, c11);
#pragma unroll
        for (int k = 0; k < NZMAX; ++k)
          if (k < nzp) {
            double v1 = (double)bil4(c00[k], c01[k], c10[k], c11[k], wy0, ty, wx0, tx);
            Kp[k * BLOCK + tid] = __dadd_rn(__dmul_rn(Kp[k * BLOCK + tid], 1 - wgt), __dmul_rn(v1, wgt));
          }
      }
      for (int k = 0; k < nzp; ++k)
        if (!isfinite(Kp[k * BLOCK + tid])) Kp[k * BLOCK + tid] = Kfb;
    } else {
      for (int k = 0; k < nzp; ++k) {
        double val = Kfb;
        if (src && cov) {
          const DevBlock &bb = src->slot[ib];
          const size_t ns = (size_t)bb.rec;
          double v0 = bilinear_f32(bb.data[VAR_KZ] + (moff + (size_t)k) * bb.es[VAR_KZ], bb.ny, bb.nx, ns, yi, xi), vv;
          if (ia >= 0) {
            const DevBlock &ba = src->slot[ia];
            double v1 = bilinear_f32(ba.data[VAR_KZ] + (moff + (size_t)k) * ba.es[VAR_KZ], ba.ny, ba.nx, ns, yi, xi);
            vv = __dadd_rn(__dmul_rn(v0, 1 - wgt), __dmul_rn(v1, wgt));
          } else vv = v0;
          if (isfinite(vv)) val = vv;
        }
        Kp[k * BLOCK + tid] = val;
      }
    }
  }
  const bool uniform_z = src ? src->vg_uniform != 0 : true;
  const double sgn = dt > 0 ? 1.0 : (dt < 0 ? -1.0 : 0.0);
  const double dt_mix = dt_mix_cfg * sgn;
  const int ntimes = abs((int)(dt / dt_mix));
  const double r = 1.0 / 3, ir = 1.0 / r;
  double z = p.z[i];
  int moving = p.moving[i];
  int sf_flags = 0;
  const float Zmin = __fmul_rn(-1.f, __fadd_rn(p.env[VAR_DEPTH][i], p.env[VAR_SSH][i]));
  double wstep = __dmul_rn(__dmul_rn((double)p.tv[i], dt_mix), (double)moving);
  const MixKey st = mix_key(seed, step, rng_mode == 0 ? p.id[i] : 0);
  uint4 u4 = make_uint4(0u, 0u, 0u, 0u);
  OilLane oil;
  if (OIL) oil.init(p, i, oa);
  int zi_cur = -1;
  double sig = 0, dKdt = 0;
  for (int it = 0; it < ntimes; ++it) {
    const bool surface = z == 0;
    if (OIL)
      wstep = __dmul_rn(__dmul_rn(oil.terminal_velocity(), dt_mix), (double)moving);
    const double d = -z;
    int zi = 0;
#pragma unroll
    for (int k = 0; k < (NZMAX > 1 ? NZMAX - 1 : MAXNZ - 1); ++k)
      if (k < nzp - 1) {
        const double mid = src->zmid[k];
        zi += ((k & 1) ? d >= mid : d > mid) ? 1 : 0;
      }
    if (zi != zi_cur) {
      zi_cur = zi;
      const double Kz = Kp[zi * BLOCK + tid];
      double gK = 0;
      if (nzp >= 2) {
        if (zi == 0) gK = div_cr(Kp[BLOCK + tid] - Kz, src->vg_d[0], src->vg_id[0]);
        else if (zi == nzp - 1) {
          if (nzp == nz_full) gK = div_cr(Kz - Kp[(nzp - 2) * BLOCK + tid], src->vg_d[1], src->vg_id[1]);
          else gK = __ddiv_rn(Kz - Kp[(nzp - 2) * BLOCK + tid], src->z[nzp - 1] - src->z[nzp - 2]);
        } else if (uniform_z)
          gK = div_cr(Kp[(zi + 1) * BLOCK + tid] - Kp[(zi - 1) * BLOCK + tid], src->vg_d[2], src->vg_id[2]);
        else
          gK = __dadd_rn(__dadd_rn(__dmul_rn(gsh[zi], Kp[(zi - 1) * BLOCK + tid]), __dmul_rn(gsh[nzp + zi], Kz)),
                         __dmul_rn(gsh[2 * nzp + zi], Kp[(zi + 1) * BLOCK + tid]));
      }
      double dK = -gK;
      if (fabs(dK) < 1e-10) dK = 0;
      dKdt = __dmul_rn(dK, dt_mix);
      sig = sqrt(div_cr(__dmul_rn(__dmul_rn(Kz, fabs(dt_mix)), 2.0), r, ir));
    }
    double u01;
    if (rng_mode == 1) u01 = huni[(size_t)it * p.n + i];
    else u01 = mix_uniform(st, u4, it);
    double R = __dsub_rn(__dmul_rn(2.0, u01), 1.0);
    z = __dsub_rn(z, __dmul_rn((double)moving, __dsub_rn(dKdt, __dmul_rn(R, sig))));
    if (z >= 0) z = -z;
    if (z < (double)Zmin && moving == 1) z = __dsub_rn((double)__fmul_rn(2.f, Zmin), z);
    z = __dadd_rn(z, wstep);
    if (!mix_at_surface && surface) z = 0.0;
    if (z > 0) z = 0.0;
    if (OIL && z >= 0) z = oil.surface_wave_mixing(z, p, i, it, oa, seed, step);
    if (z < (double)Zmin) {
      const int act = sfl & 255;
      if (act == 3) sf_flags |= 2;
      else if (act) {
        z = (double)Zmin;
        if (act == 2) { sf_flags |= 1; moving = 0; wstep = 0.0; }
      }
    }
  }
  if (sf_flags & 1) {
    if (p.status[i] == 0) p.status[i] = sfl >> 8;
    p.moving[i] = 0;
  }
  if (sf_flags & 2) { p.lon[i] = p.plon[i]; p.lat[i] = p.plat[i]; }
  if (vadv >= 0 && (vadv ? z <= 0 : z < 0)) {
    double zz = __dadd_rn(z, __dmul_rn(__dmul_rn((double)moving, (double)p.env[VAR_W][i]), dt));
    z = zz < 0 ? zz : 0.0;
  }
  if (OIL) {
    p.tv[i] = (float)oil.W;
    p.aux[OIL_DIAMETER][i] = oil.d;
  }
  p.z[i] = z;
}

#ifndef ODR_VMIX_WAVES
#define ODR_VMIX_WAVES 6
#endif
struct VMixState { double slon, slat, z0; int moving, id; float dep, ssh, tv; };
__device__ __forceinline__ VMixState vmix_load_state(const PView &p, long long i) {
  VMixState S;
  S.slon = p.slon[i]; S.slat = p.slat[i]; S.z0 = p.z[i];
  S.moving = p.moving[i]; S.id = p.id[i];
  S.dep = p.env[VAR_DEPTH][i]; S.ssh = p.env[VAR_SSH][i]; S.tv = p.tv[i];
  return S;
}
template <int NQ, bool TL, class VM>
__device__ __forceinline__ void vmix_col_particle(const DevSource &s, const PView &p, const VMixDesc &D, const VMixArgs &A,
                                                  int vadv, long long i, double *Kp, const double *gsh, int tid, const VMixState &S) {
  const int nzp = VM::nzp(D.nzp, 4 * NQ), sfl = A.sfl;
  const double dt = A.dt;
  const double slon = S.slon, slat = S.slat, z0 = S.z0;
  int moving = S.moving;
  const float dep0 = S.dep, ssh0 = S.ssh, tv0 = S.tv;
  const int id0 = S.id;
  MixRng R0;
  R0.key = mix_key(A.seed, A.step, id0); R0.q = make_uint4(0u, 0u, 0u, 0u); R0.primed = false;
  vmix_col_fill<NQ, TL, VM>(s, D, slon, slat, Kp, tid, [&]() { R0 = mix_rng_begin<VM>(A, id0); });
  int sf_flags = 0;
  const float Zmin = __fmul_rn(-1.f, __fadd_rn(dep0, ssh0));
  double z = vmix_col_walk<NQ, VM>(s, nzp, Kp, gsh, tid, A, i, p.n, id0, z0, moving, Zmin, tv0, sf_flags, &R0);
  if (sf_flags & 1) {
    if (p.status[i] == 0) p.status[i] = sfl >> 8;
    p.moving[i] = 0;
  }
  if (sf_flags & 2) { p.lon[i] = p.plon[i]; p.lat[i] = p.plat[i]; }
  vadv = VM::vadv(vadv);
  if (vadv >= 0 && (vadv ? z <= 0 : z < 0)) {
    const float w0 = p.env[VAR_W][i];
    double zz = __dadd_rn(z, __dmul_rn(__dmul_rn((double)moving, (double)w0), dt));
    z = zz < 0 ? zz : 0.0;
  }
  p.z[i] = z;
}
template <int NQ, bool TL, class VM = VMixRT>
__global__ __launch_bounds__(BLOCK, ODR_VMIX_WAVES) void k_vmix_col(const DevWorld *__restrict__ W, PView p, VMixDesc D,
                                                    double dt, double dt_mix_cfg, int mix_at_surface,
                                                    int rng_mode, const double *__restrict__ huni,
                                                    unsigned long long seed, unsigned long long step,
                                                    int vadv, int sfl) {
  constexpr int NL = 4 * NQ;
  extern __shared__ __attribute__((aligned(16))) char smem[];
  const int tid = threadIdx.x;
  const DevSource &s = W->src[D.sid];
  const int nzp = VM::nzp(D.nzp, NL);
  double *Kp = (double *)smem;
  double *gsh = Kp + (size_t)NL * BLOCK;
  if (D.guard && *D.guard == 0ull) return;
  const long long i = pid();
  const bool valid = i < p.n;
  const VMixState S = vmix_load_state(p, valid ? i : 0);
  if (tid < nzp) {
    gsh[tid] = s.vg_a[tid]; gsh[NL + tid] = s.vg_b[tid]; gsh[2 * NL + tid] = s.vg_c[tid];
    gsh[3 * NL + tid] = s.zmid[tid];
  }
  __syncthreads();
  if (!valid) return;
  VMixArgs A;
  A.dt = dt; A.dt_mix_cfg = dt_mix_cfg; A.mix_at_surface = mix_at_surface; A.rng_mode = rng_mode; A.sfl = sfl; A.pad = 0;
  A.huni = huni; A.seed = seed; A.step = step;
  vmix_col_particle<NQ, TL, VM>(s, p, D, A, vadv, i, Kp, gsh, tid, S);
}

#ifndef ODR_VWIN_WAVES
#define ODR_VWIN_WAVES 5
#endif
template <bool TL>
__device__ __forceinline__ double vmix_layer(float b00, float b01, float b10, float b11, float a00, float a01, float a10, float a11,
                                             double w00, double w01, double w10, double w11, double wgt, bool cov, double Kfb) {
  double v = (double)bilw(b00, b01, b10, b11, w00, w01, w10, w11);
  if (TL) {
    const double w = (double)bilw(a00, a01, a10, a11, w00, w01, w10, w11);
    v = __dadd_rn(__dmul_rn(v, 1 - wgt), __dmul_rn(w, wgt));
  }
  return (cov && isfinite(v)) ? v : Kfb;
}
struct VMixGrad { double gd0, gi0, gd1, gi1, gd2, gi2, dt_mix; bool uniform_z; };
__device__ __forceinline__ void vmix_terms(const VMixGrad &G, const double *gsh, int nzp, int zl, double Kl, double Kz, double Kh,
                                           double &dk_dt, double &sg) {
  const double r = 1.0 / 3, ir = 1.0 / r;
  double gK;
  if (zl == 0) gK = div_cr(Kh - Kz, G.gd0, G.gi0);
  else if (zl == nzp - 1) gK = div_cr(Kz - Kl, G.gd1, G.gi1);
  else if (G.uniform_z) gK = div_cr(Kh - Kl, G.gd2, G.gi2);
  else gK = __dadd_rn(__dadd_rn(__dmul_rn(gsh[zl], Kl), __dmul_rn(gsh[nzp + zl], Kz)), __dmul_rn(gsh[2 * nzp + zl], Kh));
  double dK = -gK;
  if (fabs(dK) < 1e-10) dK = 0;
  dk_dt = __dmul_rn(dK, G.dt_mix);
  sg = sqrt(div_cr(__dmul_rn(__dmul_rn(Kz, fabs(G.dt_mix)), 2.0), r, ir));
}
template <bool TL>
__global__ __launch_bounds__(BLOCK, ODR_VWIN_WAVES) void k_vmix_win(const DevWorld *__restrict__ W, PView p, VMixDesc D,
                                                    double dt, double dt_mix_cfg, int mix_at_surface,
                                                    int rng_mode, const double *__restrict__ huni,
                                                    unsigned long long seed, unsigned long long step,
                                                    int vadv, int sfl) {
  extern __shared__ __attribute__((aligned(16))) char smem[];
  if (D.guard && *D.guard == 0ull) return;
  const int tid = threadIdx.x;
  const DevSource &s = W->src[D.sid];
  const int nzp = D.nzp;
  double *fw = (double *)smem;
  unsigned *fo = (unsigned *)(fw + 4 * BLOCK);
  double *gsh = (double *)(fo + 4 * BLOCK);
  if (tid < nzp) {
    gsh[tid] = s.vg_a[tid]; gsh[nzp + tid] = s.vg_b[tid]; gsh[2 * nzp + tid] = s.vg_c[tid];
    gsh[3 * nzp + tid] = tid < nzp - 1 ? s.zmid[tid] : __builtin_inf();
  }
  __syncthreads();
  const long long i = pid();
  if (i >= p.n) return;
  const double slon = p.slon[i], slat = p.slat[i], z0 = p.z[i];
  int moving = p.moving[i];
  const float dep0 = p.env[VAR_DEPTH][i], ssh0 = p.env[VAR_SSH][i], tv0 = p.tv[i];
  const int id0 = rng_mode == 0 ? p.id[i] : 0;
  const float w0 = vadv >= 0 ? p.env[VAR_W][i] : 0.f;
  const MixKey key = mix_key(seed, step, id0);
  uint4 u4 = make_uint4(0u, 0u, 0u, 0u);
  const bool primed = rng_mode == 0;
  VMixGrad G;
  G.uniform_z = s.vg_uniform != 0;
  G.gd0 = s.vg_d[0]; G.gi0 = s.vg_id[0]; G.gd1 = s.vg_d[1]; G.gi1 = s.vg_id[1]; G.gd2 = s.vg_d[2]; G.gi2 = s.vg_id[2];
  const double sgn = dt > 0 ? 1.0 : (dt < 0 ? -1.0 : 0.0);
  const double dt_mix = dt_mix_cfg * sgn;
  G.dt_mix = dt_mix;
  const int ntimes = abs((int)(dt / dt_mix));
  double wstep = __dmul_rn(__dmul_rn((double)tv0, dt_mix), (double)moving);
  const float Zmin = __fmul_rn(-1.f, __fadd_rn(dep0, ssh0));
  const double Kfb = (double)D.Kfb, wgt = D.wgt;
  const float *kb = D.kb, *ka = TL ? D.ka : D.kb;
  auto level_of = [&](double d) {
    int zs = 0;
    for (int k = 0; k < nzp - 1; ++k) {
      const double b = gsh[3 * nzp + k];
      zs += ((k & 1) ? d >= b : d > b) ? 1 : 0;
    }
    return zs;
  };
  auto centre_of = [&](int zs) { return zs < 1 ? 1 : (zs > nzp - 2 ? nzp - 2 : zs); };
  double c_dk[3], c_sg[3], wb[4];
  auto load_window = [&](int lv0, unsigned o00, unsigned o01, unsigned o10, unsigned o11, double w00, double w01, double w10,
                         double w11, bool cov, bool first) {
    const unsigned lq = (unsigned)(lv0 - 1) * 4u, l1 = (unsigned)(lv0 >= 2 ? lv0 - 2 : 0) * 4u;
    const F4 b00 = ld_off<F4>(kb, o00 + lq), b01 = ld_off<F4>(kb, o01 + lq), b10 = ld_off<F4>(kb, o10 + lq), b11 = ld_off<F4>(kb, o11 + lq);
    const float c00 = ld_off<float>(kb, o00 + l1), c01 = ld_off<float>(kb, o01 + l1), c10 = ld_off<float>(kb, o10 + l1), c11 = ld_off<float>(kb, o11 + l1);
    const F4 a00 = ld_off<F4>(ka, o00 + lq), a01 = ld_off<F4>(ka, o01 + lq), a10 = ld_off<F4>(ka, o10 + lq), a11 = ld_off<F4>(ka, o11 + lq);
    const float e00 = ld_off<float>(ka, o00 + l1), e01 = ld_off<float>(ka, o01 + l1), e10 = ld_off<float>(ka, o10 + l1), e11 = ld_off<float>(ka, o11 + l1);
    if (first && primed) u4 = mix_block(key, 0u);
    double Kw[5];
    Kw[0] = vmix_layer<TL>(c00, c01, c10, c11, e00, e01, e10, e11, w00, w01, w10, w11, wgt, cov, Kfb);
    Kw[1] = vmix_layer<TL>(b00.x, b01.x, b10.x, b11.x, a00.x, a01.x, a10.x, a11.x, w00, w01, w10, w11, wgt, cov, Kfb);
    Kw[2] = vmix_layer<TL>(b00.y, b01.y, b10.y, b11.y, a00.y, a01.y, a10.y, a11.y, w00, w01, w10, w11, wgt, cov, Kfb);
    Kw[3] = vmix_layer<TL>(b00.z, b01.z, b10.z, b11.z, a00.z, a01.z, a10.z, a11.z, w00, w01, w10, w11, wgt, cov, Kfb);
    Kw[4] = vmix_layer<TL>(b00.w, b01.w, b10.w, b11.w, a00.w, a01.w, a10.w, a11.w, w00, w01, w10, w11, wgt, cov, Kfb);
#pragma unroll
    for (int q = 0; q < 3; ++q) {
      const int zl = lv0 - 1 + q;
      c_dk[q] = 0; c_sg[q] = 0;
      if (zl >= 0 && zl < nzp) vmix_terms(G, gsh, nzp, zl, Kw[q], Kw[q + 1], Kw[q + 2], c_dk[q], c_sg[q]);
    }
#pragma unroll
    for (int j = 0; j < 4; ++j) {
      const int k = lv0 - 2 + j;
      double b = k < 0 ? -1.0 : __builtin_inf();
      if (k >= 0 && k < nzp - 1) {
        b = gsh[3 * nzp + k];
        if ((k & 1) && b > 0) b = __longlong_as_double(__double_as_longlong(b) - 1);
      }
      wb[j] = b;
    }
  };
  double z = z0;
  int sf_flags = 0, it = 0;
  auto substep = [&](int lv0, unsigned x) -> bool {
    const bool surface = z == 0;
    const double d = -z;
    int q = (d > wb[1] ? 1 : 0) + (d > wb[2] ? 1 : 0);
    if (!(d > wb[0]) || d > wb[3]) {
      if (d != d && lv0 == 1) q = 0;
      else return false;
    }
    const double dKdt = q == 0 ? c_dk[0] : (q == 1 ? c_dk[1] : c_dk[2]);
    const double sig = q == 0 ? c_sg[0] : (q == 1 ? c_sg[1] : c_sg[2]);
    double R;
    if (rng_mode == 1) R = __dsub_rn(__dmul_rn(2.0, huni[(size_t)it * p.n + i]), 1.0);
    else R = mix_R_of(x);
    z = __dsub_rn(z, __dmul_rn((double)moving, __dsub_rn(dKdt, __dmul_rn(R, sig))));
    if (z >= 0) z = -z;
    if (z < (double)Zmin && moving == 1) z = __dsub_rn((double)__fmul_rn(2.f, Zmin), z);
    z = __dadd_rn(z, wstep);
    if (!mix_at_surface && surface) z = 0.0;
    if (z > 0) z = 0.0;
    if (z < (double)Zmin) {
      const int act = sfl & 255;
      if (act == 3) sf_flags |= 2;
      else if (act) {
        z = (double)Zmin;
        if (act == 2) { sf_flags |= 1; moving = 0; wstep = 0.0; }
      }
    }
    return true;
  };
  bool cov;
  {
    double lon = slon, x, y;
    if (s.lon_mode == 1) lon = np_mod(lon + 180.0, 360.0) - 180.0;
    else if (s.lon_mode == 2) lon = np_mod(lon, 360.0);
    proj_fwd_rt(s.proj, lon, slat, x, y);
// ... 1301 lines not shown
```

opendrift_amd/csrc/odr_mix.hip:

```cpp
#define ODR_TU_MIX 1
#include "odr_host.h"

template <class VM>
static bool vmix_layout_matches(const DevSource &s, const VMixDesc &D, int nq, double dt, double dt_mix, int mix_at_surface,
                                int rng_mode, int sfl, int vadv) {
  const bool uz = s.vg_uniform != 0;
  const int ntimes = abs((int)(dt / (dt_mix * (dt > 0 ? 1.0 : (dt < 0 ? -1.0 : 0.0)))));
  return VM::proj_kind(s.proj.kind) == s.proj.kind && VM::lon_mode(s.lon_mode) == s.lon_mode &&
         VM::mod360_x(s.mod360_x) == s.mod360_x && VM::nzp(D.nzp, 4 * nq) == D.nzp && VM::uniform_z(uz) == uz &&
         VM::rng_mode(rng_mode) == rng_mode && VM::mix_at_surface(mix_at_surface) == mix_at_surface &&
         VM::sf_action(sfl & 255) == (sfl & 255) && VM::vadv(vadv) == vadv && VM::ntimes(ntimes) == ntimes;
}

int odr_vmix(odr_ctx *c, odr_particles *p, double t, double dt, double dt_mix, int mix_at_surface, int rng_mode,
             const double *huni, uint64_t step) {
  const bool guarded = c->guard_next_vmix != 0;
  c->guard_next_vmix = 0;
  const bool oil = c->oil_owner == p;
  const bool f32prof = p->profiles_f32;
  const int cut = c->vmix_levels;
  VMixDesc D;
  const bool fast = !oil && !f32prof && cut <= 0 && !getenv("ODR_NO_FAST_PATH") && build_vmix_desc(c, t, D);
  if (guarded && (rng_mode == ODR_RNG_HOST || !fast)) return 1;
  const int vadv = c->fuse_vadv;
  c->fuse_vadv = -1;
  c->oil_owner = nullptr;
  c->vmix_levels = 0;
  c->guarded_vmix = nullptr;
  p->status_epoch++;
  p->epoch++;
  REQUIRE(dt_mix > 0 && dt != 0, "bad time steps");
  if (!p->env[VAR_DEPTH]) return fail(ODR_ERR_STATE, "sea_floor_depth_below_sea_level has not been sampled");
  int rc = ensure_env(c, p, VAR_SSH);
  if (rc) return rc;
  if ((rc = flush_world(c))) return rc;
  if (p->n == 0) return 0;
  int nzp = 1;
  for (int k = 0; k < c->hw.nlist[VAR_KZ]; ++k) {
    const DevSource &s = c->hw.src[c->hw.list[VAR_KZ][k]];
    if (s.kind == SRC_GRID) { nzp = s.nz > 1 ? s.nz : 1; break; }
  }
  double *du = nullptr;
  if (rng_mode == ODR_RNG_HOST) {
    REQUIRE(huni, "host uniforms required in ODR_RNG_HOST mode");
    int ntimes = abs((int)(dt / (dt_mix * (dt > 0 ? 1 : -1))));
    void *s;
    size_t n = (size_t)ntimes * (size_t)p->n;
    if ((rc = scratch(c, p, sizeof(double) * n, &s))) return rc;
    du = (double *)s;
    H2D(du, huni, sizeof(double) * n);
    HIPCHK(hipStreamSynchronize(c->stream));
  }
  size_t lds = sizeof(double) * ((size_t)nzp * BLOCK + 3 * (size_t)nzp);
  dim3 g(nblk(p->n)), b(BLOCK);
  PView v = view(p);
  unsigned long long st = (unsigned long long)step;
  if (vadv >= 0 && !p->env[VAR_W]) return fail(ODR_ERR_STATE, "upward_sea_water_velocity has not been sampled");
  struct F32ProfileClass {
    odr_ctx *c;
    bool on;
    ~F32ProfileClass() { if (on) { c->hw.f32pos &= ~2; c->dirty = true; } }
  } f32bit{c, false};
  if (f32prof) { c->hw.f32pos |= 2; c->dirty = true; f32bit.on = true; if ((rc = flush_world(c))) return rc; }
  if (cut > 0) {
    REQUIRE(cut >= 2 && cut <= 255, "odr_vmix_set_profile_levels: 2 .. 255 levels");
    if (cut < nzp) nzp = cut;
  }
  const int sfl_cut = c->seafloor | ((cut > 0 ? nzp : 0) << 16);
  if (fast) {
    if (guarded) { D.guard = c->counter + 4; c->guarded_vmix = p; c->guarded_vadv = vadv; }
    const int nq = (nzp + 3) / 4;
    const bool tl = D.ka != nullptr;
    const char *wenv = getenv("ODR_VMIX_WINDOW");
    const bool win = nzp >= 3 && nzp <= BLOCK && (wenv ? atoi(wenv) != 0 : nzp > 12);
    const bool spec = !win && (nq == 2 || nq == 3) &&
                      vmix_layout_matches<VMixC3>(c->hw.src[D.sid], D, nq, dt, dt_mix, mix_at_surface, rng_mode, c->seafloor, vadv) &&
                      !getenv("ODR_NO_VMIX_SPEC");
    p->vmix_launches[win ? 2 : spec ? 1 : 0]++;
#define VMIX_COL(NQ, VM)                                                                                          \
  do {                                                                                                            \
    size_t l2 = sizeof(double) * ((size_t)(4 * NQ) * BLOCK + 4 * (size_t)(4 * NQ));                               \
    if (tl) hipLaunchKernelGGL((k_vmix_col<NQ, true, VM>), g, b, l2, c->stream, c->dw, v, D, dt, dt_mix,          \
                               mix_at_surface, rng_mode, du, c->seed, st, vadv, c->seafloor);                                  \
    else hipLaunchKernelGGL((k_vmix_col<NQ, false, VM>), g, b, l2, c->stream, c->dw, v, D, dt, dt_mix,            \
                            mix_at_surface, rng_mode, du, c->seed, st, vadv, c->seafloor);                                     \
  } while (0)
    if (win) {
      const size_t lw = (sizeof(double) + sizeof(unsigned)) * 4 * BLOCK + sizeof(double) * 4 * (size_t)nzp;
      if (tl) hipLaunchKernelGGL((k_vmix_win<true>), g, b, lw, c->stream, c->dw, v, D, dt, dt_mix, mix_at_surface, rng_mode, du,
                                 c->seed, st, vadv, c->seafloor);
      else hipLaunchKernelGGL((k_vmix_win<false>), g, b, lw, c->stream, c->dw, v, D, dt, dt_mix, mix_at_surface, rng_mode, du,
                              c->seed, st, vadv, c->seafloor);
    }
    else if (spec && nq == 2) VMIX_COL(2, VMixC3);
    else if (spec) VMIX_COL(3, VMixC3);
    else if (nq <= 1) VMIX_COL(1, VMixRT);
    else if (nq == 2) VMIX_COL(2, VMixRT);
    else if (nq == 3) VMIX_COL(3, VMixRT);
    else if (nq == 4) VMIX_COL(4, VMixRT);
    else if (nq <= 6) VMIX_COL(6, VMixRT);
    else if (nq <= 8) VMIX_COL(8, VMixRT);
    else if (nq <= 12) VMIX_COL(12, VMixRT);
    else VMIX_COL(16, VMixRT);
#undef VMIX_COL
  } else if (oil) {
    if (nzp <= 16) hipLaunchKernelGGL((k_vmix<16, true>), g, b, lds, c->stream, c->dw, v, t, dt, dt_mix, mix_at_surface, rng_mode, du, c->seed, st, vadv, sfl_cut, c->oil);
    else if (nzp <= 32) hipLaunchKernelGGL((k_vmix<32, true>), g, b, lds, c->stream, c->dw, v, t, dt, dt_mix, mix_at_surface, rng_mode, du, c->seed, st, vadv, sfl_cut, c->oil);
    else hipLaunchKernelGGL((k_vmix<1, true>), g, b, lds, c->stream, c->dw, v, t, dt, dt_mix, mix_at_surface, rng_mode, du, c->seed, st, vadv, sfl_cut, c->oil);
  } else if (nzp <= 16) hipLaunchKernelGGL(k_vmix<16>, g, b, lds, c->stream, c->dw, v, t, dt, dt_mix, mix_at_surface, rng_mode, du, c->seed, st, vadv, sfl_cut);
  else if (nzp <= 32) hipLaunchKernelGGL(k_vmix<32>, g, b, lds, c->stream, c->dw, v, t, dt, dt_mix, mix_at_surface, rng_mode, du, c->seed, st, vadv, sfl_cut);
  else hipLaunchKernelGGL(k_vmix<1>, g, b, lds, c->stream, c->dw, v, t, dt, dt_mix, mix_at_surface, rng_mode, du, c->seed, st, vadv, sfl_cut);
  if (!fast) p->vmix_launches[2]++;
  HIPCHK(hipGetLastError());
  return 0;
}

int odr_particles_vmix_layout_stats(odr_ctx *c, odr_particles *p, uint64_t *out3) {
  REQUIRE(c && p && out3, "NULL argument");
  for (int k = 0; k < 3; ++k) out3[k] = p->vmix_launches[k];
  return 0;
}

int odr_vmix_set_profile_levels(odr_ctx *c, int32_t n) {
  REQUIRE(n == 0 || (n >= 2 && n <= 255), "bad level count %d", n);
  c->vmix_levels = n;
  return 0;
}

int odr_vmix_wind_profile(odr_ctx *c, odr_particles *p, int model, double background_diffusivity, double dt,
                          double dt_mix, int mix_at_surface, int rng_mode, const double *huni, uint64_t step) {
  c->guard_next_vmix = 0;
  p->status_epoch++;
  p->epoch++;
  REQUIRE(model == ODR_DIFFUSIVITY_LARGE1994 || model == ODR_DIFFUSIVITY_SUNDBY1983, "Unknown diffusivity model: %d", model);
  REQUIRE(dt_mix > 0 && dt != 0, "bad time steps");
  if (!p->env[VAR_DEPTH]) return fail(ODR_ERR_STATE, "sea_floor_depth_below_sea_level has not been sampled");
  int rc;
  for (int v : {VAR_SSH, VAR_XWIND, VAR_YWIND, VAR_MLD})
    if ((rc = ensure_env(c, p, v))) return rc;
  if ((rc = flush_world(c))) return rc;
  if (p->n == 0) return 0;
  p->epoch++;
  if ((rc = reduce(c, p, 0.0, 0, false, false))) return rc;
  double *du = nullptr;
  if (rng_mode == ODR_RNG_HOST) {
    REQUIRE(huni, "host uniforms required in ODR_RNG_HOST mode");
    int ntimes = abs((int)(dt / (dt_mix * (dt > 0 ? 1 : -1))));
    void *s;
    size_t n = (size_t)ntimes * (size_t)p->n;
    if ((rc = scratch(c, p, sizeof(double) * n, &s))) return rc;
    du = (double *)s;
    H2D(du, huni, sizeof(double) * n);
    HIPCHK(hipStreamSynchronize(c->stream));
  }
  int vadv = c->fuse_vadv;
  c->fuse_vadv = -1;
  if (vadv >= 0 && !p->env[VAR_W]) return fail(ODR_ERR_STATE, "upward_sea_water_velocity has not been sampled");
  dim3 g(nblk(p->n)), b(BLOCK);
  const bool oil = c->oil_owner == p;
  c->oil_owner = nullptr;
  if (oil && model == ODR_DIFFUSIVITY_LARGE1994)
    hipLaunchKernelGGL((k_vmix_wind<DIFF_LARGE1994, true>), g, b, 0, c->stream, view(p), c->red, background_diffusivity, dt, dt_mix,
                       mix_at_surface, rng_mode, du, c->seed, (unsigned long long)step, vadv, c->seafloor, c->oil);
  else if (oil)
    hipLaunchKernelGGL((k_vmix_wind<DIFF_SUNDBY1983, true>), g, b, 0, c->stream, view(p), c->red, background_diffusivity, dt, dt_mix,
                       mix_at_surface, rng_mode, du, c->seed, (unsigned long long)step, vadv, c->seafloor, c->oil);
  else if (model == ODR_DIFFUSIVITY_LARGE1994)
    hipLaunchKernelGGL(k_vmix_wind<DIFF_LARGE1994>, g, b, 0, c->stream, view(p), c->red, background_diffusivity, dt, dt_mix,
                       mix_at_surface, rng_mode, du, c->seed, (unsigned long long)step, vadv, c->seafloor);
  else
    hipLaunchKernelGGL(k_vmix_wind<DIFF_SUNDBY1983>, g, b, 0, c->stream, view(p), c->red, background_diffusivity, dt, dt_mix,
                       mix_at_surface, rng_mode, du, c->seed, (unsigned long long)step, vadv, c->seafloor);
  HIPCHK(hipGetLastError());
  p->epoch++;
  return 0;
}

int odr_oil_prepare_mixing(odr_ctx *c, odr_particles *p, double dt, double dt_mix, double interfacial_tension,
                           double sea_water_density, int droplet_distribution, int keep_droplet_diameter, int hs_mode,
                           int tp_mode, int temperature_to_kelvin, int rng_mode, const double *host_u_diameter,
                           const double *host_u_entrain, const double *host_u_intrusion, uint64_t step) {
  c->oil_owner = nullptr;
  REQUIRE(dt_mix > 0 && dt != 0, "bad time steps");
  REQUIRE(droplet_distribution == ODR_DROPLETS_JOHANSEN2015 || droplet_distribution == ODR_DROPLETS_LI2017,
          "no wave entrainment droplet size distribution specified");
  REQUIRE(interfacial_tension > 0 && sea_water_density > 0, "bad oil / water constants");
  REQUIRE(hs_mode >= 0 && hs_mode <= 2 && tp_mode >= 0 && tp_mode <= 3, "bad wave options");
  for (int k : {OIL_DIAMETER, OIL_DENSITY, OIL_VISCOSITY, OIL_FILM})
    if (!p->aux[k]) return fail(ODR_ERR_STATE, "oil property slot %d has not been set", k);
  for (int v : {VAR_XWIND, VAR_YWIND, VAR_TEMP, VAR_SALT})
    if (!p->env[v]) return fail(ODR_ERR_STATE, "wind, sea_water_temperature and sea_water_salinity must have been sampled");
  if ((hs_mode == 0 && !p->env[VAR_HS]) || (tp_mode == 0 && !p->env[VAR_TP])) return fail(ODR_ERR_STATE, "Hs/Tp not sampled");
  if (!p->aux[OIL_DIAMETER_IF_ENTRAINED]) {
    HIPCHK(hipMalloc((void **)&p->aux[OIL_DIAMETER_IF_ENTRAINED], sizeof(float) * (size_t)p->cap));
    HIPCHK(hipMemsetAsync(p->aux[OIL_DIAMETER_IF_ENTRAINED], 0, sizeof(float) * (size_t)p->cap, c->stream));
  }
  if (!c->oil_stat) {
    HIPCHK(hipMalloc((void **)&c->oil_stat, sizeof(double) * OIL_STAT_N));
    HIPCHK(hipMalloc((void **)&c->oil_cdf, sizeof(double) * OIL_NSPEC));
    HIPCHK(hipMalloc((void **)&c->oil_chunk, sizeof(double) * OIL_SPEC_BLOCKS));
    HIPCHK(hipMalloc((void **)&c->oil_guide, sizeof(int) * (OIL_GUIDE + 1)));
  }
  if (p->n == 0) return 0;
  const int ntimes = abs((int)(dt / (dt_mix * (dt > 0 ? 1 : -1))));
  REQUIRE(rng_mode == ODR_RNG_HOST || ntimes <= OIL_MAX_SUBSTEPS_DEVICE_RNG, "more than %d mixing sub-steps per step", OIL_MAX_SUBSTEPS_DEVICE_RNG);
  const unsigned nb = nblk(p->n);
  if (c->oil_part_n < 2 * (size_t)nb) {
    HIPCHK(hipStreamSynchronize(c->stream));
    if (c->oil_part) HIPCHK(hipFree(c->oil_part));
    HIPCHK(hipMalloc((void **)&c->oil_part, sizeof(double) * 2 * (size_t)nb));
    c->oil_part_n = 2 * (size_t)nb;
  }
  OilArgs &a = c->oil;
  memset(&a, 0, sizeof a);
  a.keep_diameter = keep_droplet_diameter ? 1 : 0;
  a.hs_mode = hs_mode; a.tp_mode = tp_mode; a.to_kelvin = temperature_to_kelvin ? 1 : 0;
  a.droplets = droplet_distribution; a.rng_mode = rng_mode;
  a.sigma_ow = interfacial_tension; a.rho_w = sea_water_density; a.dt_mix_cfg = dt_mix;
  a.stat = c->oil_stat;
  const double *du_d = nullptr;
  if (rng_mode == ODR_RNG_HOST) {
    REQUIRE(host_u_diameter && host_u_entrain && host_u_intrusion, "host uniforms required in ODR_RNG_HOST mode");
    const size_t per = (size_t)ntimes * (size_t)p->n, need = 2 * per + (size_t)p->n;
    if (c->oil_u_n < need) {
      HIPCHK(hipStreamSynchronize(c->stream));
      if (c->oil_u) HIPCHK(hipFree(c->oil_u));
      HIPCHK(hipMalloc((void **)&c->oil_u, sizeof(double) * need));
      c->oil_u_n = need;
    }
    H2D(c->oil_u, host_u_entrain, sizeof(double) * per);
// ... 73 lines not shown
```

opendrift_amd/csrc/odr_step.hip:

```cpp
#define ODR_TU_STEP 1
#include <chrono>
#include "odr_step_launch.h"

int odr_advect_set_noise(odr_ctx *c, odr_particles *p, double std_normal, double std_uniform, int rng_mode,
                         const double *host_main, const double *host_stage, int nstage, uint64_t step) {
  c->noise_owner = nullptr;
  REQUIRE(std_normal >= 0 && std_uniform >= 0, "uncertainties must not be negative");
  REQUIRE(rng_mode == ODR_RNG_DEVICE || rng_mode == ODR_RNG_HOST, "bad rng mode");
  if (!(std_normal > 0) && !(std_uniform > 0)) return 0;
  StageNoise &N = c->noise;
  memset(&N, 0, sizeof N);
  N.on = 1; N.rng_mode = rng_mode; N.std_n = std_normal; N.std_u = std_uniform;
  N.ncomp = 2 * ((std_normal > 0) + (std_uniform > 0));
  N.seed = c->seed; N.step = (unsigned long long)step;
  if (rng_mode == ODR_RNG_HOST && p->n > 0) {
    REQUIRE(nstage >= 0 && nstage <= 3 && (nstage == 0 || host_stage), "host draws of the stage calls required in ODR_RNG_HOST mode");
    const size_t per = (size_t)N.ncomp * (size_t)p->n, need = per * (size_t)(nstage + (host_main ? 1 : 0));
    if (c->noise_buf_n < need) {
      HIPCHK(hipStreamSynchronize(c->stream));
      if (c->noise_buf) HIPCHK(hipFree(c->noise_buf));
      HIPCHK(hipMalloc((void **)&c->noise_buf, sizeof(double) * need));
      c->noise_buf_n = need;
    }
    double *d = c->noise_buf;
// ... 50 lines not shown

int odr_advect(odr_ctx *c, odr_particles *p, int scheme, double t, double dt, double factor) {
  const StageNoise N = take_noise(c, p);
  return advect_impl(c, p, scheme, t, dt, factor, N);
}

static int mix_after(odr_ctx *c, odr_particles *p, double t, double dt, const odr_step_extras *ex) {
  c->fuse_vadv = ex->vmix_vadv;
  return odr_vmix(c, p, t, dt, ex->vmix_dt_mix, ex->vmix_at_surface, ODR_RNG_DEVICE, nullptr, ex->vmix_step);
}

int odr_env_coast_advect(odr_ctx *c, odr_particles *p, int nvars, const int32_t *var_ids, double t,
                         int coast_action, int stranded_code, int seeded_on_land_code, int store_previous,
                         int scheme, double dt, double factor, const odr_step_extras *extras, int64_t *n_on_land) {
  p->status_epoch++;
  p->epoch++;
  const StageNoise N = take_noise(c, p);
  const bool main_noise = N.on && extras && extras->main_noise;
  REQUIRE(nvars > 0 && nvars <= NVAR && var_ids, "bad variable list");
  REQUIRE(scheme >= 0 && scheme <= 2, "Drift scheme not recognised: %d", scheme);
  REQUIRE(coast_action >= 0 && coast_action <= 2, "bad coastline action");
  HIPCHK(hipSetDevice(c->device));
  if (n_on_land) *n_on_land = 0;
  int rc;
  bool has_u = false, has_v = false, has_land = false;
  for (int k = 0; k < nvars; ++k) {
    REQUIRE(var_ids[k] >= 0 && var_ids[k] < NVAR, "bad variable id %d", var_ids[k]);
    has_u |= var_ids[k] == VAR_U; has_v |= var_ids[k] == VAR_V; has_land |= var_ids[k] == VAR_LAND;
  }
  REQUIRE(has_u && has_v, "the variable list must hold x/y_sea_water_velocity");
  if (coast_action && !has_land && !p->env[VAR_LAND]) return fail(ODR_ERR_STATE, "land_binary_mask has not been sampled");
  static const double slow_ms = getenv("ODR_SLOW_CALLS") ? atof(getenv("ODR_SLOW_CALLS")) : 0.0;
  const auto t_call = std::chrono::steady_clock::now();
  double t_mark[4] = {0, 0, 0, 0};
  auto mark = [&](int k) { if (slow_ms > 0) t_mark[k] = std::chrono::duration<double, std::milli>(std::chrono::steady_clock::now() - t_call).count(); };
  struct SlowReport {
    const double &lim; const double *m;
    ~SlowReport() { if (lim > 0 && (m[3] > lim || m[2] > lim)) fprintf(stderr, "odr_env_coast_advect: world flushed at %.3f ms, group built at %.3f, other variables sampled at %.3f, launched at %.3f\n", m[0], m[1], m[2], m[3]); }
  } slow_report{slow_ms, t_mark};
  if ((rc = flush_world(c))) return rc;
  mark(0);
  int grp[NVAR], ng = 0, rest[NVAR], nrest = 0;
  auto same_list = [&](int a, int b) {
    if (c->hw.nlist[a] != c->hw.nlist[b]) return false;
    for (int k = 0; k < c->hw.nlist[a]; ++k) if (c->hw.list[a][k] != c->hw.list[b][k]) return false;
    return true;
  };
  bool land_in_group = has_land && same_list(VAR_LAND, VAR_U);
  bool has_depth = false;
  for (int k = 0; k < nvars; ++k) has_depth |= var_ids[k] == VAR_DEPTH;
  const bool want_floor = extras && extras->seafloor_action == 1;
  const bool want_mix = extras && extras->vmix;
  if (want_mix) REQUIRE(extras->vmix_dt_mix > 0 && dt != 0, "bad mixing time step");
  if (want_floor && !has_depth && !p->env[VAR_DEPTH]) return fail(ODR_ERR_STATE, "sea_floor_depth_below_sea_level has not been sampled");
  const bool depth_in_group = (want_floor || want_mix) && has_depth && same_list(VAR_DEPTH, VAR_U);
  grp[ng++] = VAR_U; grp[ng++] = VAR_V;
  if (land_in_group) grp[ng++] = VAR_LAND;
  const int depth_slot = depth_in_group ? ng : -1;
  if (depth_in_group) grp[ng++] = VAR_DEPTH;
  bool seen[NVAR] = {false};
  seen[VAR_U] = seen[VAR_V] = true;
  if (land_in_group) seen[VAR_LAND] = true;
  if (depth_in_group) seen[VAR_DEPTH] = true;
  for (int k = 0; k < nvars; ++k) {
    int v = var_ids[k];
    if (seen[v]) continue;
    seen[v] = true;
    if (same_list(v, VAR_U)) grp[ng++] = v; else rest[nrest++] = v;
  }
  int miss_grp[NVAR], nmg = 0, miss_rest[NVAR], nmr = 0;
  if (extras && extras->missing_code) {
    for (int k = 0; k < ng; ++k) if (std::isnan(c->hw.fallback[grp[k]])) miss_grp[nmg++] = k;
    for (int k = 0; k < nrest; ++k) if (std::isnan(c->hw.fallback[rest[k]])) miss_rest[nmr++] = rest[k];
  }
  EnvGroupDesc G;
  int sid = -1;
  bool fuse = p->n > 0 && !c->hw.f32pos && !getenv("ODR_NO_FAST_PATH") && same_list(VAR_V, VAR_U) && ng <= MAXG && nmg <= 4 && nmr <= 4 &&
              uv_fast_source(c, sid, t < t + dt ? t : t + dt, t < t + dt ? t + dt : t) &&
              build_env_group(c, grp, ng, t, G) && G.sid == sid && G.burst;
  mark(1);
  if (main_noise && N.rng_mode == ODR_RNG_HOST && !N.main) return fail(ODR_ERR_INVALID, "no host draws for the main sample");
  if (!fuse) {
    if ((rc = odr_env_sample(c, p, nvars, var_ids, t, nullptr))) return rc;
    if (main_noise) {
      const size_t n = (size_t)p->n;
      if (N.std_n > 0 && (rc = odr_i_env_noise(c, p, VAR_U, VAR_V, N.std_n, ODR_NOISE_NORMAL, N.rng_mode, N.main, N.main ? N.main + n : nullptr, N.step)))
        return rc;
      const double *um = N.main ? N.main + (N.std_n > 0 ? 2 * n : 0) : nullptr;
      if (N.std_u > 0 && (rc = odr_i_env_noise(c, p, VAR_U, VAR_V, N.std_u, ODR_NOISE_UNIFORM, N.rng_mode, um, um ? um + n : nullptr, N.step)))
        return rc;
    }
    if (extras && extras->missing_code && (rc = odr_deactivate_missing(c, p, nvars, var_ids, extras->missing_code, nullptr)))
      return rc;
    if ((rc = odr_coastline(c, p, coast_action, stranded_code, seeded_on_land_code, n_on_land))) return rc;
    if (want_floor && (rc = odr_seafloor(c, p, nullptr))) return rc;
    if (extras && extras->age_dt != 0 &&
        (rc = odr_increase_age(c, p, extras->age_dt, extras->max_age_seconds, extras->retired_code)))
      return rc;
    if (store_previous && (rc = odr_store_previous(c, p))) return rc;
    if ((rc = advect_impl(c, p, scheme, t, dt, factor, N))) return rc;
    return want_mix ? mix_after(c, p, t, dt, extras) : 0;
  }
  p->profiles_f32 = false;
  for (int k = 0; k < ng; ++k) { if ((rc = ensure_env(c, p, grp[k]))) return rc; p->env_cok[grp[k]] = false; }
  if (coast_action == 2) p->env_cok[VAR_LAND] = false;
  if (nrest && (rc = env_sample_impl(c, p, nrest, rest, t, nullptr, false))) return rc;
  mark(2);
  StepDesc S;
  memset(&S, 0, sizeof S);
  S.coast_action = coast_action; S.stranded_code = stranded_code; S.seeded_code = seeded_on_land_code;
  S.land_slot = land_in_group ? 2 : -1;
  S.store_previous = store_previous;
  S.seafloor = want_floor ? 1 : 0;
  S.depth_slot = depth_slot;
  S.age_dt = extras ? (float)extras->age_dt : 0.0f;
  S.max_age = extras ? (float)extras->max_age_seconds : 0.0f;
  S.retired_code = extras ? extras->retired_code : 0;
  S.missing_code = extras ? extras->missing_code : 0;
  S.nmiss_grp = nmg; S.nmiss_rest = nmr;
  for (int k = 0; k < nmg && k < 4; ++k) S.miss_grp[k] = miss_grp[k];
  for (int k = 0; k < nmr && k < 4; ++k) S.miss_rest[k] = miss_rest[k];
  if (want_floor && (rc = ensure_env(c, p, VAR_SSH))) return rc;
  const bool count_in_launch = p->wcount && !p->external && !getenv("ODR_NO_STEP_COUNT");
  if (coast_action || count_in_launch)
    HIPCHK(hipMemsetAsync(c->counter, 0, sizeof(unsigned long long) * (count_in_launch ? 4 : 1), c->stream));
  S.main_noise = main_noise ? 1 : 0;
  S.ssh_slot = -1;
  for (int k = 0; k < G.nv; ++k) if (G.var[k] == VAR_SSH) S.ssh_slot = k;
  if (odr_i_step_tile(c, p, G, S, scheme, t, dt, factor, N)) {
    HIPCHK(hipGetLastError());
    if ((rc = coast_action ? read_counter(c, n_on_land) : 0)) return rc;
    return want_mix ? mix_after(c, p, t, dt, extras) : 0;
  }
  bool red_in_launch = c->step_reduce_on && !p->external && !(c->red_pinned && c->red_owner == p) && !getenv("ODR_NO_STEP_REDUCE") &&
                       !(c->hw.src[G.sid].slot[c->hw.src[G.sid].level_slot[0]].var_nz[VAR_U] > 1);
  if (red_in_launch) {
    auto slot_of = [&](int var) { for (int k = 0; k < G.nv; ++k) if (G.var[k] == var) return k; return p->env[var] ? -1 : -2; };
    auto pair_of = [&](int vx, int vy, int &out) {
      const int a = slot_of(vx), b = slot_of(vy);
      if (a >= 0 && b == a + 1) { out = a; return true; }
      if (a == -1 && b == -1) { out = -1; return true; }
      if (a == -2 || b == -2) { out = -2; return a < 0 && b < 0; }
      return false;
    };
    S.red_hd = slot_of(VAR_HDIFF);
    red_in_launch = pair_of(VAR_SX, VAR_SY, S.red_sx) && pair_of(VAR_XWIND, VAR_YWIND, S.red_xw) && (S.red_xw == -2 || p->f32[0]);
    if (red_in_launch) {
      S.red_on = 1; S.red_rel = c->step_reduce_rel; S.red_wdd = c->step_reduce_wdd;
      S.red_iwdd = c->step_reduce_wdd != 0 ? 1.0 / fabs(c->step_reduce_wdd) : 0.0;
      if ((rc = odr_i_red_records(c, p, &S.red))) return rc;
    }
  }
  if (count_in_launch) { S.wcount = p->wcount; S.sflags = c->counter + 2; }
  if (N.on && (scheme > 0 || main_noise)) {
    if (scheme > 0 && N.rng_mode == ODR_RNG_HOST && !N.stage) return fail(ODR_ERR_INVALID, "no host draws for the Runge-Kutta stage calls");
    if (N.sm == ODR_STAGE_FAST && scheme > 0) odr_i_step_fast_noise(c, p, G, S, scheme, t, dt, factor, N);
    else odr_i_step_noise(c, p, G, S, scheme, t, dt, factor, N);
  } else if (N.sm == ODR_STAGE_FAST && scheme > 0) odr_i_step_fast(c, p, G, S, scheme, t, dt, factor, N);
  else step_dispatch<false>(c, p, G, S, scheme, t, dt, factor, N);
  HIPCHK(hipGetLastError());
  if (red_in_launch) {
    if ((rc = odr_i_red_finish(c, p))) return rc;
    c->red_owner = p; c->red_epoch = p->epoch; c->red_wdd = c->step_reduce_wdd; c->red_rel = c->step_reduce_rel;
    c->red_extents = false; c->red_partial = true;
  }
  mark(3);
  if (count_in_launch) { p->wcount_epoch = p->status_epoch; p->wcount_n = p->n; }
  if ((rc = coast_action ? read_counter(c, n_on_land) : 0)) return rc;
  return want_mix ? mix_after(c, p, t, dt, extras) : 0;
}

int odr_particles_step_layout_stats(odr_ctx *c, odr_particles *p, uint64_t *out2) {
  REQUIRE(c && p && out2, "NULL argument");
  out2[0] = p->step_launches[0]; out2[1] = p->step_launches[1];
  return 0;
}

int odr_particles_step_onlevel_stats(odr_ctx *c, odr_particles *p, uint64_t *out1) {
  REQUIRE(c && p && out1, "NULL argument");
  out1[0] = p->step_launches[2];
  return 0;
}
```

opendrift_amd/csrc/odr_step_fast.hip:

```cpp
#define ODR_TU_STEP 1
#include "odr_step_launch.h"

bool odr_i_advect_fast(odr_ctx *c, odr_particles *p, int scheme, double t, double dt, double factor, const StageNoise &N) {
  return advect_dispatch<false, 1>(c, p, scheme, t, dt, factor, N);
}
void odr_i_step_fast(odr_ctx *c, odr_particles *p, const EnvGroupDesc &G, const StepDesc &S, int scheme, double t, double dt,
                     double factor, const StageNoise &N) {
  step_dispatch<false, 1>(c, p, G, S, scheme, t, dt, factor, N);
}
ODR_DEFINE_PHASE_DUMP(odr_i_phase_dump_fast, "fast stage math")
```

opendrift_amd/csrc/odr_step_launch.h:

```cpp
#pragma once
#include "odr_host.h"

template <int SCHEME, bool NOISE, int SM = 0>
static void launch_advect_grid(odr_ctx *c, odr_particles *p, int sid, double t, double dt, double factor, const StageNoise &N) {
  const DevSource &s = c->hw.src[sid];
  UVTime th = uv_time(s, t + dt / 2), tf = uv_time(s, t + dt);
  int geo = s.level_slot[0];
  bool is3d = s.slot[geo].var_nz[VAR_U] > 1;
  dim3 g(nblk(p->n)), b(BLOCK);
  PView v = view(p);
  float f = (float)factor;
#define ODR_LAUNCH(PROJ, D3) hipLaunchKernelGGL((k_advect_grid<SCHEME, PROJ, D3, NOISE, SM>), g, b, 0, c->stream, c->dw, sid, geo, v, dt, f, th, tf, N)
  switch (odr_proj_template(s.proj)) {
    case PROJ_LATLONG: if (is3d) ODR_LAUNCH(PROJ_LATLONG, true); else ODR_LAUNCH(PROJ_LATLONG, false); break;
    case PROJ_STERE_POLAR: if (is3d) ODR_LAUNCH(PROJ_STERE_POLAR, true); else ODR_LAUNCH(PROJ_STERE_POLAR, false); break;
    case PROJ_CURVILINEAR: if (is3d) ODR_LAUNCH(PROJ_CURVILINEAR, true); else ODR_LAUNCH(PROJ_CURVILINEAR, false); break;
    case PROJ_EXT: if (is3d) ODR_LAUNCH(PROJ_EXT, true); else ODR_LAUNCH(PROJ_EXT, false); break;
    default: if (is3d) ODR_LAUNCH(PROJ_STERE_EQUIT_SPHERE, true); else ODR_LAUNCH(PROJ_STERE_EQUIT_SPHERE, false); break;
  }
#undef ODR_LAUNCH
}

template <bool NOISE, int SM = 0>
static bool advect_dispatch(odr_ctx *c, odr_particles *p, int scheme, double t, double dt, double factor, const StageNoise &N) {
  dim3 g(nblk(p->n)), b(BLOCK);
  PView v = view(p);
  int sid = -1, gsid = -1;
  const bool gyre = !getenv("ODR_NO_FAST_PATH") && scheme > 0 && gyre_source(c, VAR_U, gsid) && c->hw.nlist[VAR_V] == 1 &&
                    c->hw.list[VAR_V][0] == gsid &&
                    (c->hw.src[gsid].always_valid || (fmin(t, t + dt) >= c->hw.src[gsid].tmin && fmax(t, t + dt) <= c->hw.src[gsid].tmax));
  const bool grid = scheme > 0 && !gyre && uv_fast_source(c, sid, t < t + dt ? t : t + dt, t < t + dt ? t + dt : t) && !getenv("ODR_NO_FAST_PATH");
  if constexpr (SM != 0) {
    if (!grid) return false;
    if (scheme == 1) launch_advect_grid<1, NOISE, SM>(c, p, sid, t, dt, factor, N);
    else launch_advect_grid<2, NOISE, SM>(c, p, sid, t, dt, factor, N);
    return true;
  } else {
    if (scheme == 0) hipLaunchKernelGGL((k_advect<0, false>), g, b, 0, c->stream, c->dw, v, t, dt, (float)factor, N);
    else if (gyre) {
      const DevSource &gs = c->hw.src[gsid];
      const double sh = sin(gs.params[2] * (t + dt / 2 - gs.params[3])), sf = sin(gs.params[2] * (t + dt - gs.params[3]));
      if (scheme == 1) hipLaunchKernelGGL((k_advect_gyre<1, NOISE>), g, b, 0, c->stream, c->dw, gsid, v, dt, (float)factor, sh, sf, N);
      else hipLaunchKernelGGL((k_advect_gyre<2, NOISE>), g, b, 0, c->stream, c->dw, gsid, v, dt, (float)factor, sh, sf, N);
    } else if (grid) {
      if (scheme == 1) launch_advect_grid<1, NOISE, 0>(c, p, sid, t, dt, factor, N);
      else launch_advect_grid<2, NOISE, 0>(c, p, sid, t, dt, factor, N);
    } else if (scheme == 1) hipLaunchKernelGGL((k_advect<1, NOISE>), g, b, 0, c->stream, c->dw, v, t, dt, (float)factor, N);
    else hipLaunchKernelGGL((k_advect<2, NOISE>), g, b, 0, c->stream, c->dw, v, t, dt, (float)factor, N);
    return true;
  }
}

template <class LY>
static bool layout_matches(const EnvGroupDesc &G, const StepDesc &S) {
  return G.burst && G.nv == LY::nv && G.bs[0] == LY::kA && G.bs[1] == LY::kB && G.bs[2] == LY::kC && G.bs[3] == LY::kD &&
         G.bs[4] == LY::kL && G.var[0] == VAR_U && G.var[1] == VAR_V && G.ps_mode[0] == LY::mA && G.ps_mode[1] == LY::mB &&
         G.ps_mode[2] == LY::mC && G.ps_off[0] == LY::offA && G.ps_static == LY::ps_static && G.temp_mask == 0 &&
         S.land_slot == LY::land_slot && S.depth_slot == LY::depth_slot && S.ssh_slot == LY::ssh_slot;
}
static bool layout_matches_onlevel(const DevSource &s, const EnvGroupDesc &G, const StepDesc &S, double t, double dt,
                                   const UVTime &th) {
  typedef LayoutC3L1 LY;
  if (!(layout_matches<LY>(G, S) && G.ba == nullptr && !G.all_static && th.a != nullptr &&
        th.b == (const float *)((const char *)G.bb + LY::offA)))
    return false;
  int ib, ia;
  host_bracket(s, t + dt / 2, ib, ia);
  return ia >= 0 && th.a == (const float *)((const char *)s.slot[ia].base + LY::offA) && s.slot[ia].small &&
         s.slot[ia].rec == s.slot[ib].rec;
}

template <int SCHEME, bool NOISE, int SM = 0>
static void launch_step_grid(odr_ctx *c, odr_particles *p, const EnvGroupDesc &G0, StepDesc S, double t, double dt,
                             double factor, const StageNoise &N) {
  const EnvGroupDesc G = env_bind_out(G0, view(p));
  const DevSource &s = c->hw.src[G.sid];
  UVTime th = uv_time(s, t + dt / 2), tf = uv_time(s, t + dt);
  S.geo_slot_uv = s.level_slot[0];
  bool is3d = s.slot[S.geo_slot_uv].var_nz[VAR_U] > 1;
  dim3 g(nblk(p->n)), b(BLOCK);
  PView v = view(p);
  float f = (float)factor;
  if constexpr (SCHEME == 2 && !NOISE && SM == 1) {
    if (odr_proj_template(s.proj) == PROJ_LATLONG && is3d && !getenv("ODR_NO_LAYOUT_SPEC")) {
      if (layout_matches<LayoutC3>(G, S)) {
        hipLaunchKernelGGL((k_step_grid<SCHEME, PROJ_LATLONG, true, NOISE, SM, LayoutC3>), g, b, 0, c->stream, c->dw, v, G, S,
                           dt, f, th, tf, c->counter, N);
        p->step_launches[1]++;
        return;
      }
      if (layout_matches_onlevel(s, G, S, t, dt, th)) {
        hipLaunchKernelGGL((k_step_grid<SCHEME, PROJ_LATLONG, true, NOISE, SM, LayoutC3L1>), g, b, 0, c->stream, c->dw, v, G, S,
                           dt, f, th, tf, c->counter, N);
        p->step_launches[0]++;
        p->step_launches[2]++;
        return;
      }
    }
  }
  p->step_launches[0]++;
#define ODR_LAUNCH(PROJ, D3) hipLaunchKernelGGL((k_step_grid<SCHEME, PROJ, D3, NOISE, SM>), g, b, 0, c->stream, c->dw, v, G, S, dt, f, th, tf, c->counter, N)
  switch (odr_proj_template(s.proj)) {
    case PROJ_LATLONG: if (is3d) ODR_LAUNCH(PROJ_LATLONG, true); else ODR_LAUNCH(PROJ_LATLONG, false); break;
    case PROJ_STERE_POLAR: if (is3d) ODR_LAUNCH(PROJ_STERE_POLAR, true); else ODR_LAUNCH(PROJ_STERE_POLAR, false); break;
    case PROJ_CURVILINEAR: if (is3d) ODR_LAUNCH(PROJ_CURVILINEAR, true); else ODR_LAUNCH(PROJ_CURVILINEAR, false); break;
    case PROJ_EXT: if (is3d) ODR_LAUNCH(PROJ_EXT, true); else ODR_LAUNCH(PROJ_EXT, false); break;
    default: if (is3d) ODR_LAUNCH(PROJ_STERE_EQUIT_SPHERE, true); else ODR_LAUNCH(PROJ_STERE_EQUIT_SPHERE, false); break;
  }
#undef ODR_LAUNCH
}

template <bool NOISE, int SM = 0>
static void step_dispatch(odr_ctx *c, odr_particles *p, const EnvGroupDesc &G, const StepDesc &S, int scheme, double t, double dt,
                          double factor, const StageNoise &N) {
  if constexpr (SM == 0) { if (scheme == 0) { launch_step_grid<0, NOISE, 0>(c, p, G, S, t, dt, factor, N); return; } }
  if (scheme == 1) launch_step_grid<1, NOISE, SM>(c, p, G, S, t, dt, factor, N);
  else launch_step_grid<2, NOISE, SM>(c, p, G, S, t, dt, factor, N);
}

bool odr_i_step_tile(odr_ctx *c, odr_particles *p, const EnvGroupDesc &G, StepDesc S, int scheme, double t, double dt,
                     double factor, const StageNoise &N);
#ifdef ODR_PHASE_TIMING
#define ODR_DEFINE_PHASE_DUMP(NAME, LABEL)                                                                                      \
  void NAME() {                                                                                                                 \
    unsigned long long h[32];                                                                                                   \
    if (hipMemcpyFromSymbol(h, HIP_SYMBOL(g_phase), sizeof h) != hipSuccess || !h[31]) return;                                  \
    static const char *nm[9] = {"entry->state loaded", "env sample (gathers+math)", "stores+bookkeeping", "geod origin+stage1 pos", \
                                "stage1 sample", "stage2 pos+sample", "stage3 pos+sample", "rk4 mix+final move", "final stores issue"}; \
    static const char *sub[6] = {"env: front door + coverage", "env: xi, yi", "env: zbracket", "env: footprint + nearest",       \
                                 "env: burst 1 (A, land)", "env: burst 2 (B, C, D)"};                                            \
    double tot = 0;                                                                                                             \
    for (int k = 0; k < 9; ++k) tot += (double)h[k] / (double)h[31];                                                             \
    fprintf(stderr, "k_step_grid phases, %s (cycles per wave, %llu waves, total %.0f):\n", LABEL, h[31], tot);                   \
    for (int k = 0; k < 9; ++k) fprintf(stderr, "  %-28s %9.0f  %5.1f %%\n", nm[k], (double)h[k] / (double)h[31], 100.0 * (double)h[k] / (double)h[31] / tot); \
    for (int k = 0; k < 6; ++k) fprintf(stderr, "      %-28s %9.0f\n", sub[k], (double)h[10 + k] / (double)h[31]);               \
  }
#else
#define ODR_DEFINE_PHASE_DUMP(NAME, LABEL) void NAME() {}
#endif
void odr_i_phase_dump_fast();
bool odr_i_advect_fast(odr_ctx *c, odr_particles *p, int scheme, double t, double dt, double factor, const StageNoise &N);
void odr_i_step_fast(odr_ctx *c, odr_particles *p, const EnvGroupDesc &G, const StepDesc &S, int scheme, double t, double dt,
                     double factor, const StageNoise &N);
bool odr_i_advect_fast_noise(odr_ctx *c, odr_particles *p, int scheme, double t, double dt, double factor, const StageNoise &N);
void odr_i_step_fast_noise(odr_ctx *c, odr_particles *p, const EnvGroupDesc &G, const StepDesc &S, int scheme, double t, double dt,
                           double factor, const StageNoise &N);
void odr_i_advect_noise(odr_ctx *c, odr_particles *p, int scheme, double t, double dt, double factor, const StageNoise &N);
void odr_i_step_noise(odr_ctx *c, odr_particles *p, const EnvGroupDesc &G, const StepDesc &S, int scheme, double t, double dt,
                      double factor, const StageNoise &N);
```

opendrift_amd/device.py:

```python
import ctypes as C
import os

import numpy as np

from . import _abi
from ._abi import VARIABLES, check

_dp, _fp, _ip = C.POINTER(C.c_double), C.POINTER(C.c_float), C.POINTER(C.c_int32)


def _vid(v):
    return v if isinstance(v, (int, np.integer)) else VARIABLES[v]


def _d(a, n=None):
    if a is None:
        return None, None
    a = np.ascontiguousarray(np.broadcast_to(np.asarray(a, dtype=np.float64), (n,)) if n is not None
                             else np.asarray(a, dtype=np.float64))
    return a, a.ctypes.data_as(_dp)


def _f(a, n=None):
    if a is None:
# ... 623 lines not shown
        if distribution not in _abi.DROPLETS:
            raise ValueError('no wave entrainment droplet size distribution specified')
        pd = pe = pi = None
        mode = _abi.RNG_DEVICE
        if uniforms is not None:
            d, pd = _d(np.ascontiguousarray(self._host_order(uniforms['diameter'])))
            e, pe = _d(np.ascontiguousarray(self._host_order(uniforms['entrain'])))
            i, pi = _d(np.ascontiguousarray(self._host_order(uniforms['intrusion'])))
            mode = _abi.RNG_HOST
        check(self.lib.odr_oil_prepare_mixing(self.ctx.h, self.h, float(dt), float(dt_mix), float(interfacial_tension),
                                              float(sea_water_density), _abi.DROPLETS[distribution],
                                              int(bool(keep_droplet_diameter)), int(hs_mode), int(tp_mode),
                                              int(bool(temperature_to_kelvin)), mode, pd, pe, pi, step))

    def oil_global_stats(self, allreduce_sum, interfacial_tension, distribution, sea_water_density, hs_mode=1):
        a, b = C.c_double(), C.c_double()
        check(self.lib.odr_oil_local_sums(self.ctx.h, self.h, float(interfacial_tension), float(sea_water_density),
                                          _abi.DROPLETS[distribution], int(hs_mode), C.byref(a), C.byref(b)))
        g = allreduce_sum([a.value, b.value, float(len(self))])
        if g[2] > 0:
            check(self.lib.odr_oil_set_mixing_stats(self.ctx.h, g[1] / g[2], g[0] / g[2]))

    def oil_mixing_stats(self):
        a, b = C.c_double(), C.c_double()
        check(self.lib.odr_oil_mixing_stats(self.ctx.h, C.byref(a), C.byref(b)))
        return dict(mean_zb=a.value, dV_50=b.value)

    def vmix_oil(self, model, background_diffusivity, dt, dt_mix, interfacial_tension, distribution, sea_water_density=None,
                 t_epoch=0.0, uniforms=None, step=0, mix_at_surface=False, profile_levels=0, **kw):
        if sea_water_density is None:
            sea_water_density = sea_water_density_default()
        self.oil_prepare_mixing(dt, dt_mix, interfacial_tension, distribution, sea_water_density, step=step,
                                uniforms=uniforms, **kw)
        mix = None if uniforms is None else uniforms['mix']
        if model in ('environment', 'constant'):
            self.vmix(t_epoch, dt, dt_mix, mix_at_surface=mix_at_surface, step=step, uniforms=mix,
                      profile_levels=profile_levels if model == 'environment' else 0)
        else:
            self.vmix_analytic(model, background_diffusivity, dt, dt_mix, mix_at_surface=mix_at_surface, step=step, uniforms=mix)

    def vertical_advection(self, dt, at_surface=False):
        check(self.lib.odr_vertical_advection(self.ctx.h, self.h, float(dt), int(at_surface)))

    def vertical_buoyancy(self, dt):
        check(self.lib.odr_vertical_buoyancy(self.ctx.h, self.h, float(dt)))

    def store_previous(self):
        check(self.lib.odr_store_previous(self.ctx.h, self.h))

    def coastline(self, action, stranded_code=1, seeded_on_land_code=0):
        a = action if isinstance(action, int) else _abi.COAST[action]
        n = C.c_int64()
        check(self.lib.odr_coastline(self.ctx.h, self.h, a, stranded_code, seeded_on_land_code, C.byref(n)))
        return n.value

    def coastline_crossing(self, action, precision, landmask_source, stranded_code=1, seeded_on_land_code=0):
        a = action if isinstance(action, int) else _abi.COAST[action]
        n = C.c_int64()
        check(self.lib.odr_coastline_crossing(self.ctx.h, self.h, a, stranded_code, seeded_on_land_code, float(precision),
                                              int(landmask_source), C.byref(n)))
        return n.value

    def increase_age(self, dt, max_age_seconds=0.0, retired_code=0):
        check(self.lib.odr_increase_age(self.ctx.h, self.h, float(dt), float(max_age_seconds), retired_code))

    def deactivate_missing(self, variables, status_code):
        ids, pi = _i([_vid(v) for v in variables])
        n = C.c_int64()
        check(self.lib.odr_deactivate_missing(self.ctx.h, self.h, len(ids), pi, int(status_code), C.byref(n)))
        return n.value

    def count_status(self, status_code):
        n = C.c_int64()
        check(self.lib.odr_particles_count_status(self.ctx.h, self.h, int(status_code), C.byref(n)))
        return n.value

    def remap_status(self, from_code, to_code):
        check(self.lib.odr_particles_remap_status(self.ctx.h, self.h, int(from_code), int(to_code)))

    def seafloor(self, action='lift_to_seafloor', status_code=0):
        n = C.c_int64()
        a = {'lift_to_seafloor': 1, 'deactivate': 2, 'previous': 3}[action]
        check(self.lib.odr_seafloor_action(self.ctx.h, self.h, a, int(status_code), C.byref(n)))
        return n.value

    def deactivate(self, mask, status_code):
        m = np.ascontiguousarray(mask, dtype=np.uint8)
        check(self.lib.odr_deactivate(self.ctx.h, self.h, m.ctypes.data_as(C.POINTER(C.c_uint8)), status_code))

    def deactivate_outside(self, west, east, south, north, status_code):
        f = lambda v: np.nan if v is None else float(v)
        check(self.lib.odr_deactivate_outside(self.ctx.h, self.h, f(west), f(east), f(south), f(north), int(status_code)))

    def compact(self):
        n0 = len(self)
        n = C.c_int64()
        check(self.lib.odr_compact(self.ctx.h, self.h, C.byref(n)))
        if n.value != n0:
            self._permuted = True
        return n.value

    def scan_status(self):
        n, f = C.c_int64(), C.c_uint64()
        check(self.lib.odr_scan_status(self.ctx.h, self.h, C.byref(n), C.byref(f)))
        return n.value, f.value

    def scan_status_begin(self):
        rc = self.lib.odr_scan_status_begin(self.ctx.h, self.h)
        if rc < 0:
            check(rc)
        return rc == 0

    def scan_status_end(self):
        n, f = C.c_int64(), C.c_uint64()
        check(self.lib.odr_scan_status_end(self.ctx.h, self.h, C.byref(n), C.byref(f)))
        return n.value, f.value

    def compact_apply(self):
        n0 = len(self)
        n = C.c_int64()
        check(self.lib.odr_compact_apply(self.ctx.h, self.h, C.byref(n)))
        if n.value != n0:
            self._permuted = True
        return n.value

    def sort_by_cell(self, source_id, keep_environment=True):
        check(self.lib.odr_sort_particles_ex(self.ctx.h, self.h, int(source_id), int(bool(keep_environment))))
        self._permuted = True

    def truncate_z(self, depth):
        check(self.lib.odr_particles_truncate_z(self.ctx.h, self.h, float(depth)))

    def restore_z(self):
        check(self.lib.odr_particles_restore_z(self.ctx.h, self.h))

    def tile_stats(self):
        import ctypes as C
        out = (C.c_uint64 * 4)()
        check(self.lib.odr_particles_tile_stats(self.ctx.h, self.h, out))
        return dict(launches=int(out[0]), handed_over=int(out[1]), rectangles_cut=int(out[2]), ranges=int(out[3]))

    def step_layout_stats(self):
        import ctypes as C
        out = (C.c_uint64 * 2)()
        check(self.lib.odr_particles_step_layout_stats(self.ctx.h, self.h, out))
        return dict(runtime=int(out[0]), static=int(out[1]))

    def step_onlevel_stats(self):
        import ctypes as C
        out = (C.c_uint64 * 1)()
        check(self.lib.odr_particles_step_onlevel_stats(self.ctx.h, self.h, out))
        return int(out[0])

    def vmix_layout_stats(self):
        import ctypes as C
        out = (C.c_uint64 * 3)()
        check(self.lib.odr_particles_vmix_layout_stats(self.ctx.h, self.h, out))
        return dict(runtime=int(out[0]), static=int(out[1]), other=int(out[2]))

    def reduce_global(self, combine, wind_drift_depth=0.1, relative_wind=False):
        raw = np.empty(16)
        check(self.lib.odr_reduce_local(self.ctx.h, self.h, float(wind_drift_depth), int(relative_wind), raw.ctypes.data_as(_dp)))
        g = np.ascontiguousarray(combine(raw), dtype=np.float64)
        check(self.lib.odr_reduce_install(self.ctx.h, self.h, g.ctypes.data_as(_dp)))
        return g

    def reduce_local(self, wind_drift_depth=0.1, relative_wind=False):
        raw = np.empty(16)
        check(self.lib.odr_reduce_local(self.ctx.h, self.h, float(wind_drift_depth), int(relative_wind), raw.ctypes.data_as(_dp)))
        return raw

    def reduce_install(self, combined16):
        g = np.ascontiguousarray(combined16, dtype=np.float64)
        check(self.lib.odr_reduce_install(self.ctx.h, self.h, g.ctypes.data_as(_dp)))

    @staticmethod
    def reduction_dict(raw):
        keys = ['n_active', 'lon_min', 'lon_max', 'lat_min', 'lat_max', 'z_min', 'z_max', 'D_max',
                'stokes_sum_max', 'wind_speed_max', 'wdf_surface_max', 'n_surface', 'hs_max', 'tp_max']
        d = dict(zip(keys, raw))
        for k in ('lon_min', 'lat_min', 'z_min'):
            d[k] = -d[k]
        return d

    def reduce_unpin(self):
        check(self.lib.odr_reduce_unpin(self.ctx.h))

    def reduce_scalars(self, wind_drift_depth=0.1):
        out = np.empty(16)
        check(self.lib.odr_reduce_scalars(self.ctx.h, self.h, float(wind_drift_depth), out.ctypes.data_as(_dp)))
        keys = ['n_active', 'lon_min', 'lon_max', 'lat_min', 'lat_max', 'z_min', 'z_max', 'D_max',
                'stokes_sum_max', 'wind_speed_max', 'wdf_surface_max', 'n_surface', 'hs_max', 'tp_max']
        return dict(zip(keys, out))


_SLOW_MS = float(os.environ.get('ODR_SLOW_CALLS', 0) or 0)


def _touching(fn):
    def wrapper(self, *a, **kw):
        v = self.__dict__.get('_view')
        if v is not None:
            self._view = None
            v.flush()
        self._touch = self.__dict__.get('_touch', 0) + 1
        if _SLOW_MS:
            import sys
            import time
            t0 = time.perf_counter()
            r = fn(self, *a, **kw)
            ms = 1e3 * (time.perf_counter() - t0)
            if ms > _SLOW_MS:
                print('%s: %.3f ms' % (fn.__name__, ms), file=sys.stderr)
            return r
        return fn(self, *a, **kw)
    wrapper.__name__, wrapper.__doc__ = fn.__name__, fn.__doc__
    return wrapper


for _name in ('append', 'upload', 'env_sample', 'env_upload', 'env_add_noise', 'advect', 'env_coast_advect',
              'update_positions', 'advect_wind', 'stokes_drift', 'advect_sea_ice', 'set_property', 'leeway_capsize', 'leeway', 'hdiffusion', 'movers',
              'vmix', 'vmix_analytic', 'vmix_oil', 'vertical_advection', 'vertical_buoyancy', 'coastline', 'coastline_crossing',
              'increase_age', 'deactivate_missing', 'remap_status', 'seafloor', 'deactivate', 'deactivate_outside', 'compact',
              'compact_apply', 'sort_by_cell', 'store_previous', 'oil_prepare_mixing', 'env_coast_leeway'):
    setattr(Particles, _name, _touching(getattr(Particles, _name)))


def _reading(fn):
    def wrapper(self, *a, **kw):
        v = self.__dict__.get('_view')
        if v is not None and not getattr(v, '_flushing', False):
            touch = self.__dict__.get('_touch', 0)
            v.flush()
            self._touch = touch
            self._view = v
        return fn(self, *a, **kw)
    wrapper.__name__, wrapper.__doc__ = fn.__name__, fn.__doc__
    return wrapper


for _name in ('download', 'download_f32', 'env_download', 'get_property', 'reduce_scalars', 'reduce_global', 'reduce_local', 'oil_global_stats',
              'scan_status', 'count_status'):
    setattr(Particles, _name, _reading(getattr(Particles, _name)))


class History:

    def __init__(self, ctx, n_trajectories, n_times, variables, id_base=0):
        self.ctx, self.lib = ctx, ctx.lib
        self.variables = list(variables)
        self._id_base = int(id_base)
        self.n_trajectories, self.n_times = int(n_trajectories), int(n_times)
        codes = []
        for v in self.variables:
            if isinstance(v, tuple):
                codes.append(_abi.HIST_PROPERTY0 + int(v[1]))
            elif v in _abi.HIST:
                codes.append(_abi.HIST[v])
            else:
                codes.append(_vid(v))
        a, pa = _i(codes)
        self.h = C.c_void_p()
        check(self.lib.odr_history_create(ctx.h, self.n_trajectories, self.n_times, len(codes), pa, C.byref(self.h)))
        if self._id_base:
            check(self.lib.odr_history_set_id_base(ctx.h, self.h, self._id_base))

    def record(self, particles, time_index, only_deactivated=False, position_from_previous=False):
        check(self.lib.odr_history_record(self.ctx.h, particles.h, self.h, int(time_index), int(bool(only_deactivated)),
                                          int(position_from_previous)))

    def flush(self, t0=0, nt=None):
        check(self.lib.odr_history_flush(self.ctx.h, self.h, int(t0), int(self.n_times - t0 if nt is None else nt)))

    def wait(self):
        check(self.lib.odr_history_wait(self.ctx.h, self.h))

    def array(self, variable):
        k = self.variables.index(variable)
        p, nt = _fp(), C.c_int32()
        check(self.lib.odr_history_host_ptr(self.ctx.h, self.h, k, C.byref(p), C.byref(nt)))
        return np.ctypeslib.as_array(p, shape=(self.n_trajectories, nt.value))

    def minmax(self, variable):
        lo, hi = C.c_double(), C.c_double()
        check(self.lib.odr_history_minmax(self.ctx.h, self.h, self.variables.index(variable), C.byref(lo), C.byref(hi)))
        return lo.value, hi.value

    def reset(self):
        check(self.lib.odr_history_reset(self.ctx.h, self.h))

    def close(self):
        if self.h:
            self.lib.odr_history_destroy(self.ctx.h, self.h)
            self.h = None


class SigmaGrid:

    def __init__(self, ctx, H, Hc, Cs_r, zeta=None, S=None, Vtransform=1):
        self.ctx, self.lib = ctx, ctx.lib
        H = np.ascontiguousarray(H, dtype=np.float64)
        self.ny, self.nx = H.shape
        Cs = np.ascontiguousarray(Cs_r, dtype=np.float64)
        self.N = len(Cs)
        ze = None if zeta is None else np.ascontiguousarray(zeta, dtype=np.float64)
        Sa = None if S is None else np.ascontiguousarray(S, dtype=np.float64)
# ... 32 lines not shown
```

Before: 11.07 billion particle-steps/s.

## Fuse vertical mixing column walk into the RK4 step kernel for C3 layout

Adds a MIX template parameter to the step-grid kernel so that, on the specialised C3 lat-long 3D path, each particle runs the vertical-mixing column walk and vertical advection right after the RK4 step inside the same launch. It reuses the step kernel's shared park buffer for the Kz profile and stages the mixing tables in shared memory. The goal is to drop a separate vmix kernel launch and the extra global reads and writes of particle state. The cost is more register and LDS pressure in the step kernel, which could lower occupancy or slow the fused kernel. Host-side vmix planning is split into plan and take helpers so both paths share it.

```diff
diff --git a/include/odrift.h b/include/odrift.h
--- a/include/odrift.h
+++ b/include/odrift.h
@@ -237,6 +237,7 @@
 int odr_particles_tile_stats(odr_ctx *ctx, odr_particles *p, uint64_t *out4);
 int odr_particles_step_layout_stats(odr_ctx *ctx, odr_particles *p, uint64_t *out2);
 int odr_particles_step_onlevel_stats(odr_ctx *ctx, odr_particles *p, uint64_t *out1);
+int odr_particles_step_mix_stats(odr_ctx *ctx, odr_particles *p, uint64_t *out1);
 int odr_particles_vmix_layout_stats(odr_ctx *ctx, odr_particles *p, uint64_t *out3);
 int odr_reduce_scalars(odr_ctx *ctx, odr_particles *p, double wind_drift_depth, double *out16);
 int odr_ctx_set_step_reduce(odr_ctx *ctx, int on, double wind_drift_depth, int relative_wind);
diff --git a/opendrift_amd/_abi.py b/opendrift_amd/_abi.py
--- a/opendrift_amd/_abi.py
+++ b/opendrift_amd/_abi.py
@@ -165,6 +165,7 @@
     'odr_particles_tile_stats': [_vp, _vp, _P(C.c_uint64)],
     'odr_particles_step_layout_stats': [_vp, _vp, _P(C.c_uint64)],
     'odr_particles_step_onlevel_stats': [_vp, _vp, _P(C.c_uint64)],
+    'odr_particles_step_mix_stats': [_vp, _vp, _P(C.c_uint64)],
     'odr_particles_vmix_layout_stats': [_vp, _vp, _P(C.c_uint64)],
     'odr_reduce_scalars': [_vp, _vp, C.c_double, _dp],
     'odr_ctx_set_step_reduce': [_vp, C.c_int, C.c_double, C.c_int],
diff --git a/opendrift_amd/csrc/odr_host.h b/opendrift_amd/csrc/odr_host.h
--- a/opendrift_amd/csrc/odr_host.h
+++ b/opendrift_amd/csrc/odr_host.h
@@ -151,6 +151,7 @@
   unsigned long long wg_launches;
   unsigned long long step_launches[3];
   unsigned long long vmix_launches[3];
+  unsigned long long step_mix_launches;
   double *z_keep;
   long long z_keep_n;
   bool z_truncated;
@@ -251,6 +252,15 @@
   return true;
 }
 
+struct VMixPlan {
+  bool guarded, oil, f32prof, fast, win, spec, tl;
+  int cut, nzp, nq;
+  StepMixArgs args;
+};
+void odr_i_vmix_plan(const odr_ctx *c, const odr_particles *p, double t, double dt, double dt_mix, int mix_at_surface,
+                     int rng_mode, int vadv, uint64_t step, VMixPlan &P);
+void odr_i_vmix_take(odr_ctx *c, odr_particles *p);
+
 constexpr size_t ODR_BOUNCE_BYTES = 8u << 20;
 static inline int odr_i_bounce(odr_ctx *c, int which, void **buf) {
   if (!c->bounce[which]) HIPCHK(hipHostMalloc(&c->bounce[which], ODR_BOUNCE_BYTES, hipHostMallocDefault));
diff --git a/opendrift_amd/csrc/odr_kernels.hip.h b/opendrift_amd/csrc/odr_kernels.hip.h
--- a/opendrift_amd/csrc/odr_kernels.hip.h
+++ b/opendrift_amd/csrc/odr_kernels.hip.h
@@ -573,6 +573,65 @@
   }
   return z;
 }
+
+struct VMixState { double slon, slat, z0; int moving, id; float dep, ssh, tv; };
+__device__ __forceinline__ VMixState vmix_load_state(const PView &p, long long i) {
+  VMixState S;
+  S.slon = p.slon[i]; S.slat = p.slat[i]; S.z0 = p.z[i];
+  S.moving = p.moving[i]; S.id = p.id[i];
+  S.dep = p.env[VAR_DEPTH][i]; S.ssh = p.env[VAR_SSH][i]; S.tv = p.tv[i];
+  return S;
+}
+template <int NQ, bool TL, class VM>
+__device__ __forceinline__ void vmix_col_particle(const DevSource &s, const PView &p, const VMixDesc &D, const VMixArgs &A,
+                                                  int vadv, long long i, double *Kp, const double *gsh, int tid, const VMixState &S) {
+  const int nzp = VM::nzp(D.nzp, 4 * NQ), sfl = A.sfl;
+  const double dt = A.dt;
+  const double slon = S.slon, slat = S.slat, z0 = S.z0;
+  int moving = S.moving;
+  const float dep0 = S.dep, ssh0 = S.ssh, tv0 = S.tv;
+  const int id0 = S.id;
+  MixRng R0;
+  R0.key = mix_key(A.seed, A.step, id0); R0.q = make_uint4(0u, 0u, 0u, 0u); R0.primed = false;
+  vmix_col_fill<NQ, TL, VM>(s, D, slon, slat, Kp, tid, [&]() { R0 = mix_rng_begin<VM>(A, id0); });
+  int sf_flags = 0;
+  const float Zmin = __fmul_rn(-1.f, __fadd_rn(dep0, ssh0));
+  double z = vmix_col_walk<NQ, VM>(s, nzp, Kp, gsh, tid, A, i, p.n, id0, z0, moving, Zmin, tv0, sf_flags, &R0);
+  if (sf_flags & 1) {
+    if (p.status[i] == 0) p.status[i] = sfl >> 8;
+    p.moving[i] = 0;
+  }
+  if (sf_flags & 2) { p.lon[i] = p.plon[i]; p.lat[i] = p.plat[i]; }
+  vadv = VM::vadv(vadv);
+  if (vadv >= 0 && (vadv ? z <= 0 : z < 0)) {
+    const float w0 = p.env[VAR_W][i];
+    double zz = __dadd_rn(z, __dmul_rn(__dmul_rn((double)moving, (double)w0), dt));
+    z = zz < 0 ? zz : 0.0;
+  }
+  p.z[i] = z;
+}
+template <int NQ, class VM>
+__device__ __forceinline__ void vmix_stage_tables(const DevSource &s, const VMixDesc &D, double *gsh, int tid) {
+  constexpr int NL = 4 * NQ;
+  if (tid < VM::nzp(D.nzp, NL)) {
+    gsh[tid] = s.vg_a[tid]; gsh[NL + tid] = s.vg_b[tid]; gsh[2 * NL + tid] = s.vg_c[tid];
+    gsh[3 * NL + tid] = s.zmid[tid];
+  }
+}
+
+struct StepMixArgs { VMixDesc D; VMixArgs A; int vadv, pad; };
+struct StepMixNone {
+  static constexpr bool ON = false;
+  static constexpr int NL = 1;
+  struct Args {};
+};
+template <int NQ_, bool TL_>
+struct StepMixC3 {
+  static constexpr bool ON = true, TL = TL_;
+  static constexpr int NQ = NQ_, NL = 4 * NQ_;
+  typedef VMixC3 VM;
+  typedef StepMixArgs Args;
+};
 
 __device__ __forceinline__ float pick_slot(const float (&a)[MAXG], int j) {
   float r = a[0];
@@ -830,20 +889,23 @@
 #endif
 #define ODR_PARK_WAVES_OF(PROJ, IS3D, SM) (((PROJ) == PROJ_LATLONG && (IS3D) && (SM) == 1) ? ODR_PARK_WAVES_FAST3D : ODR_PARK_WAVES)
 #define ODR_STEP_PARKS(SCHEME, PROJ) ((SCHEME) > 0 && ((PROJ) == PROJ_LATLONG || (PROJ) == PROJ_CURVILINEAR))
-template <int SCHEME, int PROJ, bool IS3D, bool NOISE, int SM = 0, class LY = LayoutRT>
+template <int SCHEME, int PROJ, bool IS3D, bool NOISE, int SM = 0, class LY = LayoutRT, class MIX = StepMixNone>
 __global__ __launch_bounds__(BLOCK, ODR_STEP_PARKS(SCHEME, PROJ) ? ODR_PARK_WAVES_OF(PROJ, IS3D, SM) : ODR_STEP_WAVES(PROJ)) void k_step_grid(const DevWorld *__restrict__ W, PView p, EnvGroupDesc G,
                                                      StepDesc S, double dt, float factor, UVTime th, UVTime tf,
-                                                     unsigned long long *n_hit, StageNoise N) {
+                                                     unsigned long long *n_hit, StageNoise N, typename MIX::Args M) {
   long long i = pid();
   bool hit = false;
   ODR_PT_DECL;
   ODR_PT(0);
   constexpr bool PARK = ODR_STEP_PARKS(SCHEME, PROJ);
+  static_assert(!MIX::ON || (PARK && IS3D && SM == 1 && MIX::NL <= GEOD_PARK), "the mixing phase needs the park and the z tables");
   __shared__ double s_park[PARK ? GEOD_PARK * BLOCK : 1];
   __shared__ double s_zt[IS3D ? 3 * ZT_STRIDE : 1];
+  __shared__ double s_gsh[MIX::ON ? 4 * MIX::NL : 1];
   const double *zt = nullptr;
   double lon_e = 0, lat_e = 0, z_e = 0;
   if (i < p.n) { lon_e = p.lon[i]; lat_e = p.lat[i]; z_e = p.z[i]; }
+  if constexpr (MIX::ON) vmix_stage_tables<MIX::NQ, typename MIX::VM>(W->src[M.D.sid], M.D, s_gsh, threadIdx.x);
   if (IS3D) { zt_stage(W->src[G.sid], s_zt); zt = s_zt; }
   unsigned r_bits = 0;
   if (i < p.n) {
@@ -991,6 +1053,13 @@
       atomicAdd(&g_phase[31], 1ull);
     }
 #endif
+    if constexpr (MIX::ON) {
+      __builtin_amdgcn_sched_barrier(0);
+      long long i4 = i;
+      asm volatile("" : "+v"(i4));
+      const VMixState V = vmix_load_state(p, i4);
+      vmix_col_particle<MIX::NQ, MIX::TL, typename MIX::VM>(W->src[M.D.sid], p, M.D, M.A, M.vadv, i4, s_park, s_gsh, threadIdx.x, V);
+    }
   }
   if (S.coast_action) {
     unsigned long long b = __ballot(hit);
@@ -1631,42 +1700,6 @@
 #ifndef ODR_VMIX_WAVES
 #define ODR_VMIX_WAVES 6
 #endif
-struct VMixState { double slon, slat, z0; int moving, id; float dep, ssh, tv; };
-__device__ __forceinline__ VMixState vmix_load_state(const PView &p, long long i) {
-  VMixState S;
-  S.slon = p.slon[i]; S.slat = p.slat[i]; S.z0 = p.z[i];
-  S.moving = p.moving[i]; S.id = p.id[i];
-  S.dep = p.env[VAR_DEPTH][i]; S.ssh = p.env[VAR_SSH][i]; S.tv = p.tv[i];
-  return S;
-}
-template <int NQ, bool TL, class VM>
-__device__ __forceinline__ void vmix_col_particle(const DevSource &s, const PView &p, const VMixDesc &D, const VMixArgs &A,
-                                                  int vadv, long long i, double *Kp, const double *gsh, int tid, const VMixState &S) {
-  const int nzp = VM::nzp(D.nzp, 4 * NQ), sfl = A.sfl;
-  const double dt = A.dt;
-  const double slon = S.slon, slat = S.slat, z0 = S.z0;
-  int moving = S.moving;
-  const float dep0 = S.dep, ssh0 = S.ssh, tv0 = S.tv;
-  const int id0 = S.id;
-  MixRng R0;
-  R0.key = mix_key(A.seed, A.step, id0); R0.q = make_uint4(0u, 0u, 0u, 0u); R0.primed = false;
-  vmix_col_fill<NQ, TL, VM>(s, D, slon, slat, Kp, tid, [&]() { R0 = mix_rng_begin<VM>(A, id0); });
-  int sf_flags = 0;
-  const float Zmin = __fmul_rn(-1.f, __fadd_rn(dep0, ssh0));
-  double z = vmix_col_walk<NQ, VM>(s, nzp, Kp, gsh, tid, A, i, p.n, id0, z0, moving, Zmin, tv0, sf_flags, &R0);
-  if (sf_flags & 1) {
-    if (p.status[i] == 0) p.status[i] = sfl >> 8;
-    p.moving[i] = 0;
-  }
-  if (sf_flags & 2) { p.lon[i] = p.plon[i]; p.lat[i] = p.plat[i]; }
-  vadv = VM::vadv(vadv);
-  if (vadv >= 0 && (vadv ? z <= 0 : z < 0)) {
-    const float w0 = p.env[VAR_W][i];
-    double zz = __dadd_rn(z, __dmul_rn(__dmul_rn((double)moving, (double)w0), dt));
-    z = zz < 0 ? zz : 0.0;
-  }
-  p.z[i] = z;
-}
 template <int NQ, bool TL, class VM = VMixRT>
 __global__ __launch_bounds__(BLOCK, ODR_VMIX_WAVES) void k_vmix_col(const DevWorld *__restrict__ W, PView p, VMixDesc D,
                                                     double dt, double dt_mix_cfg, int mix_at_surface,
@@ -1677,17 +1710,13 @@
   extern __shared__ __attribute__((aligned(16))) char smem[];
   const int tid = threadIdx.x;
   const DevSource &s = W->src[D.sid];
-  const int nzp = VM::nzp(D.nzp, NL);
   double *Kp = (double *)smem;
   double *gsh = Kp + (size_t)NL * BLOCK;
   if (D.guard && *D.guard == 0ull) return;
   const long long i = pid();
   const bool valid = i < p.n;
   const VMixState S = vmix_load_state(p, valid ? i : 0);
-  if (tid < nzp) {
-    gsh[tid] = s.vg_a[tid]; gsh[NL + tid] = s.vg_b[tid]; gsh[2 * NL + tid] = s.vg_c[tid];
-    gsh[3 * NL + tid] = s.zmid[tid];
-  }
+  vmix_stage_tables<NQ, VM>(s, D, gsh, tid);
   __syncthreads();
   if (!valid) return;
   VMixArgs A;
diff --git a/opendrift_amd/csrc/odr_mix.hip b/opendrift_amd/csrc/odr_mix.hip
--- a/opendrift_amd/csrc/odr_mix.hip
+++ b/opendrift_amd/csrc/odr_mix.hip
@@ -12,34 +12,62 @@
          VM::sf_action(sfl & 255) == (sfl & 255) && VM::vadv(vadv) == vadv && VM::ntimes(ntimes) == ntimes;
 }
 
-int odr_vmix(odr_ctx *c, odr_particles *p, double t, double dt, double dt_mix, int mix_at_surface, int rng_mode,
-             const double *huni, uint64_t step) {
-  const bool guarded = c->guard_next_vmix != 0;
+void odr_i_vmix_plan(const odr_ctx *c, const odr_particles *p, double t, double dt, double dt_mix, int mix_at_surface,
+                     int rng_mode, int vadv, uint64_t step, VMixPlan &P) {
+  memset(&P, 0, sizeof P);
+  P.guarded = c->guard_next_vmix != 0;
+  P.oil = c->oil_owner == p;
+  P.f32prof = p->profiles_f32;
+  P.cut = c->vmix_levels;
+  VMixDesc &D = P.args.D;
+  P.fast = !P.oil && !P.f32prof && P.cut <= 0 && !getenv("ODR_NO_FAST_PATH") && build_vmix_desc(c, t, D);
+  P.nzp = 1;
+  for (int k = 0; k < c->hw.nlist[VAR_KZ]; ++k) {
+    const DevSource &s = c->hw.src[c->hw.list[VAR_KZ][k]];
+    if (s.kind == SRC_GRID) { P.nzp = s.nz > 1 ? s.nz : 1; break; }
+  }
+  P.nq = (P.nzp + 3) / 4;
+  P.tl = D.ka != nullptr;
+  if (P.fast) {
+    const char *wenv = getenv("ODR_VMIX_WINDOW");
+    P.win = P.nzp >= 3 && P.nzp <= BLOCK && (wenv ? atoi(wenv) != 0 : P.nzp > 12);
+    P.spec = !P.win && (P.nq == 2 || P.nq == 3) &&
+             vmix_layout_matches<VMixC3>(c->hw.src[D.sid], D, P.nq, dt, dt_mix, mix_at_surface, rng_mode, c->seafloor, vadv) &&
+             !getenv("ODR_NO_VMIX_SPEC");
+  }
+  VMixArgs &A = P.args.A;
+  A.dt = dt; A.dt_mix_cfg = dt_mix; A.mix_at_surface = mix_at_surface; A.rng_mode = rng_mode; A.sfl = c->seafloor;
+  A.huni = nullptr; A.seed = c->seed; A.step = (unsigned long long)step;
+  P.args.vadv = vadv;
+}
+
+void odr_i_vmix_take(odr_ctx *c, odr_particles *p) {
   c->guard_next_vmix = 0;
-  const bool oil = c->oil_owner == p;
-  const bool f32prof = p->profiles_f32;
-  const int cut = c->vmix_levels;
-  VMixDesc D;
-  const bool fast = !oil && !f32prof && cut <= 0 && !getenv("ODR_NO_FAST_PATH") && build_vmix_desc(c, t, D);
-  if (guarded && (rng_mode == ODR_RNG_HOST || !fast)) return 1;
-  const int vadv = c->fuse_vadv;
   c->fuse_vadv = -1;
   c->oil_owner = nullptr;
   c->vmix_levels = 0;
   c->guarded_vmix = nullptr;
   p->status_epoch++;
   p->epoch++;
+}
+
+int odr_vmix(odr_ctx *c, odr_particles *p, double t, double dt, double dt_mix, int mix_at_surface, int rng_mode,
+             const double *huni, uint64_t step) {
+  VMixPlan P;
+  odr_i_vmix_plan(c, p, t, dt, dt_mix, mix_at_surface, rng_mode, c->fuse_vadv, step, P);
+  const bool guarded = P.guarded, oil = P.oil, f32prof = P.f32prof, fast = P.fast;
+  const int cut = P.cut, vadv = P.args.vadv;
+  VMixDesc D = P.args.D;
+  c->guard_next_vmix = 0;
+  if (guarded && (rng_mode == ODR_RNG_HOST || !fast)) return 1;
+  odr_i_vmix_take(c, p);
   REQUIRE(dt_mix > 0 && dt != 0, "bad time steps");
   if (!p->env[VAR_DEPTH]) return fail(ODR_ERR_STATE, "sea_floor_depth_below_sea_level has not been sampled");
   int rc = ensure_env(c, p, VAR_SSH);
   if (rc) return rc;
   if ((rc = flush_world(c))) return rc;
   if (p->n == 0) return 0;
-  int nzp = 1;
-  for (int k = 0; k < c->hw.nlist[VAR_KZ]; ++k) {
-    const DevSource &s = c->hw.src[c->hw.list[VAR_KZ][k]];
-    if (s.kind == SRC_GRID) { nzp = s.nz > 1 ? s.nz : 1; break; }
-  }
+  int nzp = P.nzp;
   double *du = nullptr;
   if (rng_mode == ODR_RNG_HOST) {
     REQUIRE(huni, "host uniforms required in ODR_RNG_HOST mode");
@@ -69,13 +97,8 @@
   const int sfl_cut = c->seafloor | ((cut > 0 ? nzp : 0) << 16);
   if (fast) {
     if (guarded) { D.guard = c->counter + 4; c->guarded_vmix = p; c->guarded_vadv = vadv; }
-    const int nq = (nzp + 3) / 4;
-    const bool tl = D.ka != nullptr;
-    const char *wenv = getenv("ODR_VMIX_WINDOW");
-    const bool win = nzp >= 3 && nzp <= BLOCK && (wenv ? atoi(wenv) != 0 : nzp > 12);
-    const bool spec = !win && (nq == 2 || nq == 3) &&
-                      vmix_layout_matches<VMixC3>(c->hw.src[D.sid], D, nq, dt, dt_mix, mix_at_surface, rng_mode, c->seafloor, vadv) &&
-                      !getenv("ODR_NO_VMIX_SPEC");
+    const int nq = P.nq;
+    const bool tl = P.tl, win = P.win, spec = P.spec;
     p->vmix_launches[win ? 2 : spec ? 1 : 0]++;
 #define VMIX_COL(NQ, VM)                                                                                          \
   do {                                                                                                            \
diff --git a/opendrift_amd/csrc/odr_step.hip b/opendrift_amd/csrc/odr_step.hip
--- a/opendrift_amd/csrc/odr_step.hip
+++ b/opendrift_amd/csrc/odr_step.hip
@@ -226,11 +226,22 @@
     }
   }
   if (count_in_launch) { S.wcount = p->wcount; S.sflags = c->counter + 2; }
+  VMixPlan mix;
+  const bool try_mix = want_mix && !(N.on && (scheme > 0 || main_noise)) && N.sm == ODR_STAGE_FAST && scheme == 2 &&
+                       !getenv("ODR_NO_STEP_MIX");
+  if (try_mix) odr_i_vmix_plan(c, p, t, dt, extras->vmix_dt_mix, extras->vmix_at_surface, ODR_RNG_DEVICE, extras->vmix_vadv,
+                               extras->vmix_step, mix);
+  const bool mix_ok = try_mix && mix.fast && mix.spec && !mix.guarded && p->env[VAR_DEPTH] && p->env[VAR_W];
+  if (mix_ok) {
+    if ((rc = ensure_env(c, p, VAR_SSH))) return rc;
+    if ((rc = flush_world(c))) return rc;
+  }
+  bool mixed = false;
   if (N.on && (scheme > 0 || main_noise)) {
     if (scheme > 0 && N.rng_mode == ODR_RNG_HOST && !N.stage) return fail(ODR_ERR_INVALID, "no host draws for the Runge-Kutta stage calls");
     if (N.sm == ODR_STAGE_FAST && scheme > 0) odr_i_step_fast_noise(c, p, G, S, scheme, t, dt, factor, N);
     else odr_i_step_noise(c, p, G, S, scheme, t, dt, factor, N);
-  } else if (N.sm == ODR_STAGE_FAST && scheme > 0) odr_i_step_fast(c, p, G, S, scheme, t, dt, factor, N);
+  } else if (N.sm == ODR_STAGE_FAST && scheme > 0) mixed = odr_i_step_fast(c, p, G, S, scheme, t, dt, factor, N, mix_ok ? &mix : nullptr);
   else step_dispatch<false>(c, p, G, S, scheme, t, dt, factor, N);
   HIPCHK(hipGetLastError());
   if (red_in_launch) {
@@ -241,6 +252,12 @@
   mark(3);
   if (count_in_launch) { p->wcount_epoch = p->status_epoch; p->wcount_n = p->n; }
   if ((rc = coast_action ? read_counter(c, n_on_land) : 0)) return rc;
+  if (mixed) {
+    odr_i_vmix_take(c, p);
+    p->vmix_launches[1]++;
+    p->step_mix_launches++;
+    return 0;
+  }
   return want_mix ? mix_after(c, p, t, dt, extras) : 0;
 }
 
@@ -255,3 +272,9 @@
   out1[0] = p->step_launches[2];
   return 0;
 }
+
+int odr_particles_step_mix_stats(odr_ctx *c, odr_particles *p, uint64_t *out1) {
+  REQUIRE(c && p && out1, "NULL argument");
+  out1[0] = p->step_mix_launches;
+  return 0;
+}
diff --git a/opendrift_amd/csrc/odr_step_fast.hip b/opendrift_amd/csrc/odr_step_fast.hip
--- a/opendrift_amd/csrc/odr_step_fast.hip
+++ b/opendrift_amd/csrc/odr_step_fast.hip
@@ -4,8 +4,8 @@
 bool odr_i_advect_fast(odr_ctx *c, odr_particles *p, int scheme, double t, double dt, double factor, const StageNoise &N) {
   return advect_dispatch<false, 1>(c, p, scheme, t, dt, factor, N);
 }
-void odr_i_step_fast(odr_ctx *c, odr_particles *p, const EnvGroupDesc &G, const StepDesc &S, int scheme, double t, double dt,
-                     double factor, const StageNoise &N) {
-  step_dispatch<false, 1>(c, p, G, S, scheme, t, dt, factor, N);
+bool odr_i_step_fast(odr_ctx *c, odr_particles *p, const EnvGroupDesc &G, const StepDesc &S, int scheme, double t, double dt,
+                     double factor, const StageNoise &N, const VMixPlan *mix) {
+  return step_dispatch<false, 1>(c, p, G, S, scheme, t, dt, factor, N, mix);
 }
 ODR_DEFINE_PHASE_DUMP(odr_i_phase_dump_fast, "fast stage math")
diff --git a/opendrift_amd/csrc/odr_step_launch.h b/opendrift_amd/csrc/odr_step_launch.h
--- a/opendrift_amd/csrc/odr_step_launch.h
+++ b/opendrift_amd/csrc/odr_step_launch.h
@@ -71,8 +71,8 @@
 }
 
 template <int SCHEME, bool NOISE, int SM = 0>
-static void launch_step_grid(odr_ctx *c, odr_particles *p, const EnvGroupDesc &G0, StepDesc S, double t, double dt,
-                             double factor, const StageNoise &N) {
+static bool launch_step_grid(odr_ctx *c, odr_particles *p, const EnvGroupDesc &G0, StepDesc S, double t, double dt,
+                             double factor, const StageNoise &N, const VMixPlan *mix) {
   const EnvGroupDesc G = env_bind_out(G0, view(p));
   const DevSource &s = c->hw.src[G.sid];
   UVTime th = uv_time(s, t + dt / 2), tf = uv_time(s, t + dt);
@@ -83,23 +83,34 @@
   float f = (float)factor;
   if constexpr (SCHEME == 2 && !NOISE && SM == 1) {
     if (odr_proj_template(s.proj) == PROJ_LATLONG && is3d && !getenv("ODR_NO_LAYOUT_SPEC")) {
+#define ODR_LAUNCH_C3(LY, M, ...) hipLaunchKernelGGL((k_step_grid<SCHEME, PROJ_LATLONG, true, NOISE, SM, LY, __VA_ARGS__>), g, b, 0, c->stream, \
+                                                   c->dw, v, G, S, dt, f, th, tf, c->counter, N, M)
       if (layout_matches<LayoutC3>(G, S)) {
-        hipLaunchKernelGGL((k_step_grid<SCHEME, PROJ_LATLONG, true, NOISE, SM, LayoutC3>), g, b, 0, c->stream, c->dw, v, G, S,
-                           dt, f, th, tf, c->counter, N);
         p->step_launches[1]++;
-        return;
+        if (mix && mix->tl) {
+          if (mix->nq == 2) ODR_LAUNCH_C3(LayoutC3, mix->args, StepMixC3<2, true>);
+          else ODR_LAUNCH_C3(LayoutC3, mix->args, StepMixC3<3, true>);
+          return true;
+        }
+        ODR_LAUNCH_C3(LayoutC3, StepMixNone::Args(), StepMixNone);
+        return false;
       }
       if (layout_matches_onlevel(s, G, S, t, dt, th)) {
-        hipLaunchKernelGGL((k_step_grid<SCHEME, PROJ_LATLONG, true, NOISE, SM, LayoutC3L1>), g, b, 0, c->stream, c->dw, v, G, S,
-                           dt, f, th, tf, c->counter, N);
         p->step_launches[0]++;
         p->step_launches[2]++;
-        return;
+        if (mix && !mix->tl) {
+          if (mix->nq == 2) ODR_LAUNCH_C3(LayoutC3L1, mix->args, StepMixC3<2, false>);
+          else ODR_LAUNCH_C3(LayoutC3L1, mix->args, StepMixC3<3, false>);
+          return true;
+        }
+        ODR_LAUNCH_C3(LayoutC3L1, StepMixNone::Args(), StepMixNone);
+        return false;
       }
+#undef ODR_LAUNCH_C3
     }
   }
   p->step_launches[0]++;
-#define ODR_LAUNCH(PROJ, D3) hipLaunchKernelGGL((k_step_grid<SCHEME, PROJ, D3, NOISE, SM>), g, b, 0, c->stream, c->dw, v, G, S, dt, f, th, tf, c->counter, N)
+#define ODR_LAUNCH(PROJ, D3) hipLaunchKernelGGL((k_step_grid<SCHEME, PROJ, D3, NOISE, SM>), g, b, 0, c->stream, c->dw, v, G, S, dt, f, th, tf, c->counter, N, StepMixNone::Args())
   switch (odr_proj_template(s.proj)) {
     case PROJ_LATLONG: if (is3d) ODR_LAUNCH(PROJ_LATLONG, true); else ODR_LAUNCH(PROJ_LATLONG, false); break;
     case PROJ_STERE_POLAR: if (is3d) ODR_LAUNCH(PROJ_STERE_POLAR, true); else ODR_LAUNCH(PROJ_STERE_POLAR, false); break;
@@ -108,14 +119,15 @@
     default: if (is3d) ODR_LAUNCH(PROJ_STERE_EQUIT_SPHERE, true); else ODR_LAUNCH(PROJ_STERE_EQUIT_SPHERE, false); break;
   }
 #undef ODR_LAUNCH
+  return false;
 }
 
 template <bool NOISE, int SM = 0>
-static void step_dispatch(odr_ctx *c, odr_particles *p, const EnvGroupDesc &G, const StepDesc &S, int scheme, double t, double dt,
-                          double factor, const StageNoise &N) {
-  if constexpr (SM == 0) { if (scheme == 0) { launch_step_grid<0, NOISE, 0>(c, p, G, S, t, dt, factor, N); return; } }
-  if (scheme == 1) launch_step_grid<1, NOISE, SM>(c, p, G, S, t, dt, factor, N);
-  else launch_step_grid<2, NOISE, SM>(c, p, G, S, t, dt, factor, N);
+static bool step_dispatch(odr_ctx *c, odr_particles *p, const EnvGroupDesc &G, const StepDesc &S, int scheme, double t, double dt,
+                          double factor, const StageNoise &N, const VMixPlan *mix = nullptr) {
+  if constexpr (SM == 0) { if (scheme == 0) return launch_step_grid<0, NOISE, 0>(c, p, G, S, t, dt, factor, N, mix); }
+  if (scheme == 1) return launch_step_grid<1, NOISE, SM>(c, p, G, S, t, dt, factor, N, mix);
+  return launch_step_grid<2, NOISE, SM>(c, p, G, S, t, dt, factor, N, mix);
 }
 
 bool odr_i_step_tile(odr_ctx *c, odr_particles *p, const EnvGroupDesc &G, StepDesc S, int scheme, double t, double dt,
@@ -140,8 +152,8 @@
 #endif
 void odr_i_phase_dump_fast();
 bool odr_i_advect_fast(odr_ctx *c, odr_particles *p, int scheme, double t, double dt, double factor, const StageNoise &N);
-void odr_i_step_fast(odr_ctx *c, odr_particles *p, const EnvGroupDesc &G, const StepDesc &S, int scheme, double t, double dt,
-                     double factor, const StageNoise &N);
+bool odr_i_step_fast(odr_ctx *c, odr_particles *p, const EnvGroupDesc &G, const StepDesc &S, int scheme, double t, double dt,
+                     double factor, const StageNoise &N, const VMixPlan *mix);
 bool odr_i_advect_fast_noise(odr_ctx *c, odr_particles *p, int scheme, double t, double dt, double factor, const StageNoise &N);
 void odr_i_step_fast_noise(odr_ctx *c, odr_particles *p, const EnvGroupDesc &G, const StepDesc &S, int scheme, double t, double dt,
                            double factor, const StageNoise &N);
diff --git a/opendrift_amd/device.py b/opendrift_amd/device.py
--- a/opendrift_amd/device.py
+++ b/opendrift_amd/device.py
@@ -799,6 +799,12 @@
         check(self.lib.odr_particles_step_onlevel_stats(self.ctx.h, self.h, out))
         return int(out[0])
 
+    def step_mix_stats(self):
+        import ctypes as C
+        out = (C.c_uint64 * 1)()
+        check(self.lib.odr_particles_step_mix_stats(self.ctx.h, self.h, out))
+        return int(out[0])
+
     def vmix_layout_stats(self):
         import ctypes as C
         out = (C.c_uint64 * 3)()
```

Measured after the change: 10.89 billion particle-steps/s (median of 2 runs). -1.7%, worse.
